# li-kunyi/dns-slam

Hardware: AMD Instinct MI355X
Metric: ray-samples/s (higher is better)
Workload: dtype f32 (MLP products as 3 x f16 split-operand MFMA / 6 x bf16 for weight gradients, f32 accumulate: error <= fp32 fma chain)

## Files before the change

dns_slam_amd/_lib.py:

```python
from __future__ import annotations

import ctypes as C
import os

_HERE = os.path.dirname(os.path.abspath(__file__))
LIB_PATH = os.environ.get("DNS_HIP_LIB") or os.path.join(_HERE, "libdns_hip.so")
DNS_MAX_LEVELS = 32
ABI_VERSION = 13


class DnsGridMeta(C.Structure):
    _fields_ = [
        ("n_levels", C.c_uint32), ("n_features", C.c_uint32), ("log2_hashmap_size", C.c_uint32),
        ("base_resolution", C.c_uint32), ("total_rows", C.c_uint32), ("per_level_scale", C.c_float),
        ("scale", C.c_float * DNS_MAX_LEVELS), ("resolution", C.c_uint32 * DNS_MAX_LEVELS),
        ("size", C.c_uint32 * DNS_MAX_LEVELS), ("offset", C.c_uint32 * DNS_MAX_LEVELS),
        ("hashed", C.c_uint32 * DNS_MAX_LEVELS),
    ]


class DnsSplitRows(C.Structure):
    _fields_ = [("rows", C.c_void_p), ("exps", C.c_void_p), ("ld", C.c_uint32), ("lo_off", C.c_uint32)]


class DnsAdamTensor(C.Structure):
    _fields_ = [("p", C.c_void_p), ("g", C.c_void_p), ("m", C.c_void_p), ("v", C.c_void_p), ("n", C.c_uint64),
                ("lr", C.c_float)]


_P = C.c_void_p
_U = C.c_uint32
_I = C.c_int


class DnsTrackFused(C.Structure):
    _fields_ = [("color", _P), ("depth", _P), ("label", _P),
                ("H", C.c_int32), ("W", C.c_int32), ("H0", C.c_int32), ("H1", C.c_int32), ("W0", C.c_int32), ("W1", C.c_int32),
                ("cam", _P), ("bound", _P),
                ("pix", _P), ("t_uniform", _P), ("t_surf", _P), ("t_zero", _P), ("dmax", _P), ("iter", _P), ("n_iters", _U),
                ("n_uniform", _U), ("n_surface", _U), ("n_rays", _U),
                ("quat", _P), ("trans", _P),
                ("table", _P), ("meta", C.POINTER(DnsGridMeta)), ("n_bins", _U),
                ("w_coarse", _P), ("w_color", _P), ("w_logit", _P),
                ("n_neurons", _U), ("n_hidden_layers", _U), ("hidden", _U), ("n_feat", _U), ("n_class", _U),
                ("code", _P), ("code_dim", _U),
                ("lambda_p", C.c_float), ("lambda_d", C.c_float), ("lambda_l", C.c_float),
                ("ws", _P), ("adam_m", _P), ("adam_v", _P), ("adam_state", _P),
                ("lr_quat", C.c_float), ("lr_trans", C.c_float), ("beta1", C.c_float), ("beta2", C.c_float), ("eps", C.c_float),
                ("best_loss", _P), ("best_cam", _P), ("out", _P), ("g_quat", _P), ("g_trans", _P)]

SIGNATURES = {
    "dns_abi_version": (C.c_int, []),
    "dns_last_error": (C.c_char_p, []),
    "dns_init": (C.c_int, []),
    "dns_kernel_timing": (C.c_int, [C.c_int]),
    "dns_kernel_timing_count": (C.c_int, []),
    "dns_kernel_timing_get": (C.c_int, [C.c_int, C.c_char_p, C.c_int, C.POINTER(C.c_float)]),
    "dns_grid_meta_init": (C.c_int, [C.POINTER(DnsGridMeta), _U, _U, _U, _U, C.c_double]),
    "dns_raygen_sample": (C.c_int, [_P, _P, _P, _P, _P, _P, _P, _P, _I, _I, _I, _I, _I, _I, _I, _I, _P, _P, _P, _I, _I, _I,
                                    _P, _I, _P, _P, _P, _P, _P, _P, _P, _P, _P]),
    "dns_rays_from_pixels": (C.c_int, [_P, _P, _I, _P, _P, _P, _I, _I, _I, _I, _I, _I, _I, _P, _P, _P, _P, _P]),
    "dns_sample_along_rays": (C.c_int, [_P, _P, _I, _P, _P, _P, _I, _I, _P, _P, _P]),
    "dns_raygen_bwd": (C.c_int, [_P, _P, _P, _I, _I, _I, _I, _I, _I, _I, _P, _P, _P, _P, _P, _P, _P, _P]),
    "dns_raygen_bwd_ws_floats": (C.c_uint64, [_I, _I]),
    "dns_encode_fwd": (C.c_int, [_P, _P, _U, _U, _P, C.POINTER(DnsGridMeta), _P, _P, _U, _P, _U, _P, _P]),
    "dns_encode_bwd": (C.c_int, [_P, _P, _U, _U, _P, C.POINTER(DnsGridMeta), _P, _U, _P, _U, _P, _P, _P, _P, _U, _U, _P]),
    "dns_encode_bwd_ws_floats": (C.c_uint64, [_U, C.POINTER(DnsGridMeta), _U, _U]),
    "dns_hashgrid_indices": (C.c_int, [_P, _U, C.POINTER(DnsGridMeta), _P, _P]),
    "dns_mlp_fwd": (C.c_int, [_P, _U, _P, _U, _U, _P, _U, _U, _U, _U, _P, _U, _U, _P, _P, _U, _P, _U, _P]),
    "dns_mlp_bwd": (C.c_int, [_P, _U, _P, _U, _U, _P, _U, _P, _U, _U, _U, _U, _P, _U, _P, _U, _P, _P, _U, _P, _P, _U, _P, _I, _P]),
    "dns_mlp_bwd_ws_floats": (C.c_uint64, [_U, _U, _U]),
    "dns_mlp_dwin": (C.c_int, [_P, _U, _P, _U, _U, _U, _U, _U, _P, _P, _U, _P, _P, _U, _U, _P]),
    "dns_mlp_prepared_floats": (C.c_uint64, [_U, _U, _U, _U]),
    "dns_mlp_prepare": (C.c_int, [_P, _U, _U, _U, _U, _U, _U, _P, _U, _P]),
    "dns_encode_fwd_split": (C.c_int, [_P, _P, _U, _U, _P, C.POINTER(DnsGridMeta), _P, _P, _U, _P, _U, _P, _U, _P, _P]),
    "dns_mlp_fwd_split": (C.c_int, [C.POINTER(DnsSplitRows), C.POINTER(DnsSplitRows), _U, _P, _U, _U, _U, _U, _P, _U, _U, _P, _P, _U,
                                    _U, _P]),
    "dns_mlp_bwd_split": (C.c_int, [C.POINTER(DnsSplitRows), C.POINTER(DnsSplitRows), _U, _P, _U, _P, _U, _U, _U, _U, _P, _U, _P, _U,
                                    _P, _P, _U, _P, _P, _U, _I, _P]),
    "dns_mlp_fwd_half": (C.c_int, [_P, _U, _P, _U, _U, _P, _U, _U, _U, _U, _P, _U, _U, _P, _P, _U, _U, _P]),
    "dns_mlp_bwd_half": (C.c_int, [_P, _U, _P, _U, _U, _P, _U, _P, _U, _U, _U, _U, _P, _U, _P, _U, _P, _U, _P, _P, _U, _I, C.c_float, _P]),
    "dns_feature_block_split": (C.c_int, [_P, _U, _U, _P, _U, _U, _U, _P, _P, _U, _U, _P, _U, _P, _U, _P, _U, _P, _P]),
    "dns_loss_sums": (C.c_int, [_P, _U, _U, _U, _U, _I, _P, _P, _P, _P, _P, _P, _P, _P, _P, _P, _P, _P, _P]),
    "dns_loss_rays": (C.c_int, [_P, _U, _U, _U, _U, _I] + [_P] * 19),
    "dns_loss_finalize_bwd": (C.c_int, [_P, _U, _U, _U, _U, _I] + [_P] * 16),
    "dns_loss_finalize": (C.c_int, [_P, _U, _U, _U, _U, _I, _P, _P, _P]),
    "dns_loss_bwd": (C.c_int, [_P, _U, _U, _U, _U, _I, _P, _P, _P, _P, _P, _P, _P, _P, _P, _P, _P, _P, _P, _P, _P, _P, _P,
                                _P, _P, _U, _P]),
    "dns_loss_bwd_points": (C.c_int, [_P, _U, _U, _U, _U, _P, _P, _P, _P, _P, _P, _P, _P, _P, _U, _P, _U, _P]),
    "dns_composite_fwd_ex": (C.c_int, [_P, _P, _P, _U, _U, _U, _P, _P, _P, _P, _P, _U, _P]),
    "dns_composite_bwd_ex": (C.c_int, [_P, _P, _P, _U, _U, _U, _P, _P, _P, _P, _P, _P, _P, _U, _P]),
    "dns_class_slots": (C.c_int, [_P, _U, _U, _I, _P, _U, _P, _P]),
    "dns_feature_block": (C.c_int, [_P, _U, _U, _P, _U, _P, _P, _U, _U, _P, _U, _P, _P]),
    "dns_rgb_sigmoid": (C.c_int, [_P, _U, _P]),
    "dns_raw_bwd": (C.c_int, [_P, _P, _U, _P, _P, _U, _I, _P]),
    "dns_lattice_points": (C.c_int, [_P, _P, _U, _P, _U, _P, _P]),
    "dns_draw_finish": (C.c_int, [_P, _P, _P, _P, _P, _P, _P, _P, _U, _U, _U, _U, _P, _P, _P, _P]),
    "dns_track_mask": (C.c_int, [_P, _P, _U, C.c_float, _P, _P]),
    "dns_keep_best": (C.c_int, [_P, _P, _P, _P, _P, _P]),
    "dns_force_half": (C.c_int, [_P, _U, _U, _P]),
    "dns_track_fused_ws_floats": (C.c_uint64, [C.POINTER(DnsTrackFused)]),
    "dns_track_fused_begin": (C.c_int, [_P, _U, _U, _P, _I, _I, _I, _I, _P, _U, _P, _P]),
    "dns_track_fused_iter": (C.c_int, [C.POINTER(DnsTrackFused), _P]),
    "dns_feature_gather": (C.c_int, [_P, _P, _P, _P, _U, _U, _U, _I, _I, _I, _I, _P, _P, _P]),
    "dns_feature_gather_frames": (C.c_int, [_P, _P, _P, _P, _P, _U, _U, _U, _U, _I, _I, _I, _I, _P, _U, _P, _P]),
    "dns_refer_poses": (C.c_int, [_P, _P, _P, _P, _U, _P, _P, _P]),
    "dns_merge_dy": (C.c_int, [_P, _U, _U, _U, _U, _P, _P, _U, _U, _P, _P]),
    "dns_add_ref_sum": (C.c_int, [_P, _U, _U, _U, _P, _P]),
    "dns_tv_fwd": (C.c_int, [_P, _U, _U, _U, _I, _U, _P, _P]),
    "dns_tv_bwd": (C.c_int, [_P, _U, _U, _U, _I, _U, _P, _P, _P]),
    "dns_group_slots": (C.c_int, [_P, _U, _U, _U, _U, _P, _P, _P, _P]),
    "dns_group_scatter": (C.c_int, [_P, _U, _U, _P, _U, _P, _P]),
    "dns_device_error": (C.c_int, [C.c_int]),
    "dns_adam_step": (C.c_int, [C.POINTER(DnsAdamTensor), _U, C.c_float, C.c_float, C.c_float, _P, _P]),
    "dns_composite_fwd": (C.c_int, [_P, _P, _P, _U, _U, _U, _P, _P, _P, _P, _P, _P]),
    "dns_composite_bwd": (C.c_int, [_P, _P, _P, _U, _U, _U, _P, _P, _P, _P, _P, _P, _P, _P]),
    "dns_mc_ws_bytes": (C.c_uint64, [_U, _U, _U]),
    "dns_mc_count": (C.c_int, [_P, _U, _U, _U, C.c_float, _P, _P, _P]),
    "dns_mc_emit": (C.c_int, [_P, _U, _U, _U, C.c_float, C.POINTER(C.c_double), C.POINTER(C.c_double), _P, _P, C.c_uint64, _P,
                              C.c_uint64, _P]),
    "dns_keyframe_project": (C.c_int, [_P, _U, _P, _U, _P, _P, _I, _I, C.POINTER(C.c_float), _P, _P, _P]),
}


def _load():
    if not os.path.exists(LIB_PATH):
        raise ImportError(
            f"{LIB_PATH} is missing: the HIP hot-path library has not been built. Run "
            "`python -c 'import __graft_entry__ as g; g.build()'` (or `make -C dns_slam_amd/csrc`). "
            "dns_slam_amd has no CPU fallback.")
    import torch
    lib = C.CDLL(LIB_PATH)
    for name, (res, args) in SIGNATURES.items():
        fn = getattr(lib, name)
        fn.restype = res
        fn.argtypes = args
    v = lib.dns_abi_version()
    if v != ABI_VERSION:
        raise ImportError(f"libdns_hip.so ABI version {v} != expected {ABI_VERSION}; rebuild it")
    return lib


lib = _load()


_ready_devices = set()


def ensure_init() -> None:
    import torch
    d = torch.cuda.current_device()
    if d not in _ready_devices:
        if torch.cuda.is_current_stream_capturing():
            raise RuntimeError("dns_slam_amd: first use on this device inside a hipGraph capture; run one op (or "
                               "dns_slam_amd._lib.ensure_init()) before capturing")
        check(lib.dns_init(), "dns_init")
        _ready_devices.add(d)


def check(rc: int, what: str = "") -> None:
    if rc == 0:
        return
    msg = lib.dns_last_error().decode("utf-8", "replace")
    if rc == -1:
        raise ValueError(f"{what}: {msg}")
    if rc == -2:
        word = lib.dns_device_error(1)
        if word:
            raise RuntimeError(f"{what}: {msg} (code {rc}; device error word {word:#x} was set by an EARLIER kernel -- bit 0: "
                               f"dns_group_slots / dns_group_scatter cursor past n_slots -- and has been cleared)")
    raise RuntimeError(f"{what}: {msg} (code {rc})")


def ptr(t):
    return None if t is None else C.c_void_p(t.data_ptr())


def stream_ptr():
    import torch
    ensure_init()
    return C.c_void_p(torch.cuda.current_stream().cuda_stream)


def require_cuda(*tensors):
    import torch
    for t in tensors:
        if t is None:
            continue
        if not isinstance(t, torch.Tensor) or not t.is_cuda:
            raise ValueError("dns_slam_amd ops run on the GPU only (got a non-CUDA tensor); there is no CPU fallback")
        if not t.is_contiguous():
            raise ValueError("dns_slam_amd ops need contiguous tensors")
```

dns_slam_amd/csrc/composite.hip:

```cpp
#include "common.hpp"
#include "dev_composite.hpp"

namespace dns {

template <int E>
__global__ __launch_bounds__(256) void composite_fwd_kernel(const float* __restrict__ raw, const float* __restrict__ zv,
                                                            const float* __restrict__ logits, uint32_t N, uint32_t S,
                                                            uint32_t C, float* __restrict__ depth, float* __restrict__ var,
                                                            float* __restrict__ rgb, float* __restrict__ weights,
                                                            float* __restrict__ sem, uint32_t rgbl) {
  extern __shared__ float lds[];
  const uint32_t lane = threadIdx.x & 63u, wave = threadIdx.x >> 6;
  const uint32_t n = blockIdx.x * 4 + wave;
  if (n >= N) return;
  float* wl = lds + wave * (64 * E);
  RayState<E> st;
  ray_forward<E>(raw, zv, n, S, lane, st);
  float sv = 0.f, sc[3] = {0.f, 0.f, 0.f};
#pragma unroll
  for (int e = 0; e < E; ++e) {
    const uint32_t s = lane * E + e;
    const float t = st.z[e] - st.depth;
    sv += st.w[e] * t * t;
    if (s < S) {
      const float* r = raw + ((size_t)n * S + s) * 4;
      const float c0 = rgbl ? sigmoid1c(r[0]) : r[0], c1 = rgbl ? sigmoid1c(r[1]) : r[1], c2 = rgbl ? sigmoid1c(r[2]) : r[2];
      sc[0] += st.w[e] * c0;
      sc[1] += st.w[e] * c1;
      sc[2] += st.w[e] * c2;
      if (weights) weights[(size_t)n * S + s] = st.w[e];
    }
    wl[s] = st.w[e];
  }
  sv = wave_sum(sv);
  sc[0] = wave_sum(sc[0]);
  sc[1] = wave_sum(sc[1]);
  sc[2] = wave_sum(sc[2]);
  if (lane == 0) {
    depth[n] = st.depth;
    var[n] = sv;
    rgb[(size_t)n * 3 + 0] = sc[0];
    rgb[(size_t)n * 3 + 1] = sc[1];
    rgb[(size_t)n * 3 + 2] = sc[2];
  }
  if (C) {
    for (uint32_t c = lane; c < C; c += 64) {
      float acc = 0.f;
      const float* lp = logits + (size_t)n * S * C + c;
      for (uint32_t s = 0; s < S; ++s) acc += wl[s] * lp[(size_t)s * C];
      sem[(size_t)n * C + c] = acc;
    }
  }
}

template <int E>
__global__ __launch_bounds__(256) void composite_bwd_kernel(const float* __restrict__ raw, const float* __restrict__ zv,
                                                            const float* __restrict__ logits, uint32_t N, uint32_t S,
                                                            uint32_t C, const float* __restrict__ d_depth,
                                                            const float* __restrict__ d_var, const float* __restrict__ d_rgb,
                                                            const float* __restrict__ d_weights,
                                                            const float* __restrict__ d_sem, float* __restrict__ d_raw,
                                                            float* __restrict__ d_logits, uint32_t rgbl) {
  extern __shared__ float lds[];
  const uint32_t lane = threadIdx.x & 63u, wave = threadIdx.x >> 6;
  const uint32_t n = blockIdx.x * 4 + wave;
  if (n >= N) return;
  float* wl = lds + wave * (64 * E);
  RayState<E> st;
  ray_forward<E>(raw, zv, n, S, lane, st);
  const float gD = d_depth ? d_depth[n] : 0.f;
  const float gV = d_var ? d_var[n] : 0.f;
  float gc[3] = {0.f, 0.f, 0.f};
  if (d_rgb) {
    gc[0] = d_rgb[(size_t)n * 3];
    gc[1] = d_rgb[(size_t)n * 3 + 1];
    gc[2] = d_rgb[(size_t)n * 3 + 2];
  }
  float g[E];
  float col[E][3];
  float gbar = 0.f;
#pragma unroll
  for (int e = 0; e < E; ++e) {
    const uint32_t s = lane * E + e;
    g[e] = 0.f;
    col[e][0] = col[e][1] = col[e][2] = 0.f;
    if (s < S) {
      const float* r = raw + ((size_t)n * S + s) * 4;
      const float t = st.z[e] - st.depth;
      col[e][0] = rgbl ? sigmoid1c(r[0]) : r[0];
      col[e][1] = rgbl ? sigmoid1c(r[1]) : r[1];
      col[e][2] = rgbl ? sigmoid1c(r[2]) : r[2];
      float v = gc[0] * col[e][0] + gc[1] * col[e][1] + gc[2] * col[e][2] + gD * st.z[e] + gV * t * t;
      if (d_weights) v += d_weights[(size_t)n * S + s];
      if (C && d_sem) {
        const float* lp = logits + ((size_t)n * S + s) * C;
        const float* gs = d_sem + (size_t)n * C;
        float dot = 0.f;
        for (uint32_t c = 0; c < C; ++c) dot += gs[c] * lp[c];
        v += dot;
      }
      g[e] = v;
    }
    gbar += st.w[e] * g[e];
    wl[s] = st.w[e];
  }
  gbar = wave_sum(gbar);
  float du[E], lsum = 0.f;
#pragma unroll
  for (int e = 0; e < E; ++e) {
    du[e] = (g[e] - gbar) / st.sumu;
    lsum += du[e] * st.u[e];
  }
  const float after = wave_suffix_excl_sum(lsum, lane);
  float tail = after;
#pragma unroll
  for (int e = E - 1; e >= 0; --e) {
    const uint32_t s = lane * E + e;
    const float dalpha = du[e] * st.T[e] - tail / st.om[e];
    tail += du[e] * st.u[e];
    if (s < S) {
      float* o = d_raw + ((size_t)n * S + s) * 4;
      float o0 = st.w[e] * gc[0], o1 = st.w[e] * gc[1], o2 = st.w[e] * gc[2];
      if (rgbl) {
        o0 = o0 * (1.f - col[e][0]) * col[e][0];
        o1 = o1 * (1.f - col[e][1]) * col[e][1];
        o2 = o2 * (1.f - col[e][2]) * col[e][2];
      }
      o[0] = o0;
      o[1] = o1;
      o[2] = o2;
      o[3] = 10.0f * st.alpha[e] * (1.0f - st.alpha[e]) * dalpha;
    }
  }
  if (C && d_logits) {
    for (uint32_t c = lane; c < C; c += 64) {
      const float gs = d_sem ? d_sem[(size_t)n * C + c] : 0.f;
      float* lp = d_logits + (size_t)n * S * C + c;
      for (uint32_t s = 0; s < S; ++s) lp[(size_t)s * C] = wl[s] * gs;
    }
  }
}

}

using namespace dns;

static int composite_fwd_impl(const char* who, const float* raw, const float* z, const float* logits, uint32_t N, uint32_t S,
                              uint32_t C, float* depth, float* var, float* rgb, float* weights, float* sem, uint32_t rgbl,
                              void* stream) {
  if (N == 0) return DNS_OK;
  DNS_REQUIRE(raw && z && depth && var && rgb, "%s: NULL argument", who);
  DNS_REQUIRE(S >= 1 && S <= 256, "%s: S=%u out of range [1,256]", who, S);
  DNS_REQUIRE(C == 0 || (logits && sem), "%s: C>0 needs logits and sem", who);
  const uint32_t blocks = (N + 3) / 4;
  hipStream_t st = (hipStream_t)stream;
  const uint32_t E = S <= 64 ? 1 : (S <= 128 ? 2 : 4);
  const size_t ldsb = 4 * 64 * E * sizeof(float);
  if (E == 1) DNS_LAUNCH(composite_fwd_kernel<1>, dim3(blocks), dim3(256), ldsb, st, raw, z, logits, N, S, C, depth, var, rgb, weights, sem, rgbl);
  else if (E == 2) DNS_LAUNCH(composite_fwd_kernel<2>, dim3(blocks), dim3(256), ldsb, st, raw, z, logits, N, S, C, depth, var, rgb, weights, sem, rgbl);
  else DNS_LAUNCH(composite_fwd_kernel<4>, dim3(blocks), dim3(256), ldsb, st, raw, z, logits, N, S, C, depth, var, rgb, weights, sem, rgbl);
  return check_launch(who);
}

static int composite_bwd_impl(const char* who, const float* raw, const float* z, const float* logits, uint32_t N, uint32_t S,
                              uint32_t C, const float* d_depth, const float* d_var, const float* d_rgb, const float* d_weights,
                              const float* d_sem, float* d_raw, float* d_logits, uint32_t rgbl, void* stream) {
  if (N == 0) return DNS_OK;
  DNS_REQUIRE(raw && z && d_raw, "%s: NULL argument", who);
  DNS_REQUIRE(S >= 1 && S <= 256, "%s: S=%u out of range [1,256]", who, S);
  DNS_REQUIRE(C == 0 || logits, "%s: C>0 needs logits", who);
  const uint32_t blocks = (N + 3) / 4;
  hipStream_t st = (hipStream_t)stream;
  const uint32_t E = S <= 64 ? 1 : (S <= 128 ? 2 : 4);
  const size_t ldsb = 4 * 64 * E * sizeof(float);
  if (E == 1) DNS_LAUNCH(composite_bwd_kernel<1>, dim3(blocks), dim3(256), ldsb, st, raw, z, logits, N, S, C, d_depth, d_var, d_rgb, d_weights, d_sem, d_raw, d_logits, rgbl);
  else if (E == 2) DNS_LAUNCH(composite_bwd_kernel<2>, dim3(blocks), dim3(256), ldsb, st, raw, z, logits, N, S, C, d_depth, d_var, d_rgb, d_weights, d_sem, d_raw, d_logits, rgbl);
  else DNS_LAUNCH(composite_bwd_kernel<4>, dim3(blocks), dim3(256), ldsb, st, raw, z, logits, N, S, C, d_depth, d_var, d_rgb, d_weights, d_sem, d_raw, d_logits, rgbl);
  return check_launch(who);
}

extern "C" int dns_composite_fwd(const float* raw, const float* z, const float* logits, uint32_t N, uint32_t S,
                                 uint32_t C, float* depth, float* var, float* rgb, float* weights, float* sem,
                                 void* stream) {
  return composite_fwd_impl("dns_composite_fwd", raw, z, logits, N, S, C, depth, var, rgb, weights, sem, 0u, stream);
}

extern "C" int dns_composite_bwd(const float* raw, const float* z, const float* logits, uint32_t N, uint32_t S,
                                 uint32_t C, const float* d_depth, const float* d_var, const float* d_rgb,
                                 const float* d_weights, const float* d_sem, float* d_raw, float* d_logits,
                                 void* stream) {
  return composite_bwd_impl("dns_composite_bwd", raw, z, logits, N, S, C, d_depth, d_var, d_rgb, d_weights, d_sem, d_raw, d_logits, 0u,
                            stream);
}

extern "C" int dns_composite_fwd_ex(const float* raw, const float* z, const float* logits, uint32_t N, uint32_t S, uint32_t C,
                                    float* depth, float* var, float* rgb, float* weights, float* sem, uint32_t flags, void* stream) {
  DNS_REQUIRE((flags & ~DNS_COMPOSITE_RGB_LOGITS) == 0, "dns_composite_fwd_ex: unknown flags 0x%x", flags);
  return composite_fwd_impl("dns_composite_fwd_ex", raw, z, logits, N, S, C, depth, var, rgb, weights, sem, flags & DNS_COMPOSITE_RGB_LOGITS,
                            stream);
}

extern "C" int dns_composite_bwd_ex(const float* raw, const float* z, const float* logits, uint32_t N, uint32_t S, uint32_t C,
                                    const float* d_depth, const float* d_var, const float* d_rgb, const float* d_weights,
                                    const float* d_sem, float* d_raw, float* d_logits, uint32_t flags, void* stream) {
  DNS_REQUIRE((flags & ~DNS_COMPOSITE_RGB_LOGITS) == 0, "dns_composite_bwd_ex: unknown flags 0x%x", flags);
  return composite_bwd_impl("dns_composite_bwd_ex", raw, z, logits, N, S, C, d_depth, d_var, d_rgb, d_weights, d_sem, d_raw, d_logits,
                            flags & DNS_COMPOSITE_RGB_LOGITS, stream);
}
```

dns_slam_amd/csrc/dev_composite.hpp:

```cpp
#pragma once
#include "common.hpp"

namespace dns {

__device__ __forceinline__ float wave_sum(float v) {
#pragma unroll
  for (int o = 32; o >= 1; o >>= 1) v += __shfl_xor(v, o);
  return v;
}

__device__ __forceinline__ float wave_excl_prod(float v, uint32_t lane) {
  float inc = v;
#pragma unroll
  for (int o = 1; o < 64; o <<= 1) {
    const float t = __shfl_up(inc, o);
    if (lane >= (uint32_t)o) inc *= t;
  }
  const float ex = __shfl_up(inc, 1);
  return lane == 0 ? 1.0f : ex;
}

__device__ __forceinline__ float wave_suffix_excl_sum(float v, uint32_t lane) {
  float inc = v;
#pragma unroll
  for (int o = 1; o < 64; o <<= 1) {
    const float t = __shfl_down(inc, o);
    if (lane + o < 64u) inc += t;
  }
  const float ex = __shfl_down(inc, 1);
  return lane == 63 ? 0.0f : ex;
}

__device__ __forceinline__ float sigmoid10(float occ) { return 1.0f / (1.0f + expf(-10.0f * occ)); }
__device__ __forceinline__ float sigmoid1c(float x) { return 1.0f / (1.0f + expf(-x)); }

template <int E>
struct RayState {
  float alpha[E], om[E], T[E], u[E], w[E], z[E];
  float sumu, depth;
};

template <int E>
__device__ __forceinline__ void ray_forward(const float* __restrict__ raw, const float* __restrict__ zv, uint32_t n,
                                            uint32_t S, uint32_t lane, RayState<E>& st) {
  float lp = 1.0f;
#pragma unroll
  for (int e = 0; e < E; ++e) {
    const uint32_t s = lane * E + e;
    const bool ok = s < S;
    const float occ = ok ? raw[((size_t)n * S + s) * 4 + 3] : 0.f;
    st.z[e] = ok ? zv[(size_t)n * S + s] : 0.f;
    st.alpha[e] = ok ? sigmoid10(occ) : 0.f;
    st.om[e] = ok ? (1.0f - st.alpha[e]) + 1e-10f : 1.0f;
    st.T[e] = lp;
    lp *= st.om[e];
  }
  const float pre = wave_excl_prod(lp, lane);
  float su = 0.f;
#pragma unroll
  for (int e = 0; e < E; ++e) {
    st.T[e] *= pre;
    st.u[e] = st.alpha[e] * st.T[e];
    su += st.u[e];
  }
  st.sumu = wave_sum(su);
  float sd = 0.f;
#pragma unroll
  for (int e = 0; e < E; ++e) {
    st.w[e] = st.u[e] / st.sumu;
    sd += st.w[e] * st.z[e];
  }
  st.depth = wave_sum(sd);
}

}
```

dns_slam_amd/csrc/losses.hip:

```cpp
#include <stdlib.h>
#include "common.hpp"

namespace dns {

enum { S_P = 0, S_D, S_L, S_LT, S_FS, S_OP, S_NV, S_ND, S_NFRONT, S_NOMASK, S_COUNT = 16,
       S_PARTIALS = 32, S_MAX_BLOCKS = 1024 };
constexpr uint32_t LOSS_POINT_BLOCKS = 1024;
enum { O_P = 0, O_D, O_L, O_LT, O_FS, O_OP, O_TOTAL, O_CP = 8, O_CD, O_CL, O_CLT, O_CFS, O_COP };

struct LossCfg {
  float lambda_p, lambda_d, lambda_l, lambda_lt, lambda_fs, lambda_op;
  float truncation, sigma;
  uint32_t N, S, C, L;
  int tracker;
};

__device__ __forceinline__ float block_sum(float v, float* sh) {
#pragma unroll
  for (int o = 32; o >= 1; o >>= 1) v += __shfl_xor(v, o);
  const uint32_t lane = threadIdx.x & 63u, wave = threadIdx.x >> 6;
  __syncthreads();
  if (lane == 0) sh[wave] = v;
  __syncthreads();
  float t = 0.f;
  if (threadIdx.x == 0)
    for (uint32_t w = 0; w < (blockDim.x >> 6); ++w) t += sh[w];
  return t;
}

__device__ __forceinline__ bool ray_valid(const uint8_t* valid, uint32_t n) { return valid ? valid[n] != 0 : true; }

struct RayTerms {
  float sp, sd, sl, nv, nd;
};
__device__ __forceinline__ RayTerms ray_terms(const LossCfg& c, uint32_t n, const float* __restrict__ pred_color,
                                              const float* __restrict__ pred_depth, const float* __restrict__ pred_var,
                                              const float* __restrict__ logits, const float* __restrict__ gt_color,
                                              const float* __restrict__ gt_depth, const int64_t* __restrict__ gt_label,
                                              const uint8_t* __restrict__ valid) {
  RayTerms r = {0.f, 0.f, 0.f, 0.f, 0.f};
  if (n < c.N && ray_valid(valid, n)) {
    r.nv = 1.f;
#pragma unroll
    for (int k = 0; k < 3; ++k) {
      const float e = gt_color[(size_t)n * 3 + k] - pred_color[(size_t)n * 3 + k];
      r.sp += e * e;
    }
    const float gd = gt_depth[n];
    if (c.tracker) {
      r.sd = fabsf(gd - pred_depth[n]) / sqrtf(pred_var[n] + 1e-10f);
      r.nd = 1.f;
    } else if (gd > 0.f) {
      r.sd = fabsf(gd - pred_depth[n]);
      r.nd = 1.f;
    }
    if (c.C) {
      const float* lg = logits + (size_t)n * c.C;
      float mx = -INFINITY;
      for (uint32_t k = 0; k < c.C; ++k) mx = fmaxf(mx, lg[k]);
      float se = 0.f;
      for (uint32_t k = 0; k < c.C; ++k) se += expf(lg[k] - mx);
      const int64_t lab = gt_label[n];
      const float ll = (lab >= 0 && lab < (int64_t)c.C) ? lg[lab] : 0.f;
      r.sl = (mx + logf(se)) - ll;
    }
  }
  return r;
}

__global__ __launch_bounds__(256) void loss_ray_sums_kernel(LossCfg c, const float* __restrict__ pred_color,
                                                            const float* __restrict__ pred_depth,
                                                            const float* __restrict__ pred_var,
                                                            const float* __restrict__ logits,
                                                            const float* __restrict__ gt_color,
                                                            const float* __restrict__ gt_depth,
                                                            const int64_t* __restrict__ gt_label,
                                                            const uint8_t* __restrict__ valid, float* __restrict__ sums,
                                                            uint32_t n_partials) {
  __shared__ float sh[16];
  const uint32_t n = blockIdx.x * blockDim.x + threadIdx.x;
  const RayTerms rt = ray_terms(c, n, pred_color, pred_depth, pred_var, logits, gt_color, gt_depth, gt_label, valid);
  const float sp = rt.sp, sd = rt.sd, sl = rt.sl, nv = rt.nv, nd = rt.nd;
  float t;
  t = block_sum(sp, sh); if (threadIdx.x == 0 && t != 0.f) atomicAdd(sums + S_P, t);
  t = block_sum(sd, sh); if (threadIdx.x == 0 && t != 0.f) atomicAdd(sums + S_D, t);
  t = block_sum(sl, sh); if (threadIdx.x == 0 && t != 0.f) atomicAdd(sums + S_L, t);
  t = block_sum(nv, sh); if (threadIdx.x == 0 && t != 0.f) atomicAdd(sums + S_NV, t);
  t = block_sum(nd, sh); if (threadIdx.x == 0 && t != 0.f) atomicAdd(sums + S_ND, t);
  if (blockIdx.x == 0 && n_partials) {
    const float* partial = sums + S_PARTIALS;
    const int dst[5] = {S_LT, S_FS, S_OP, S_NFRONT, S_NOMASK};
#pragma unroll
    for (int i = 0; i < 5; ++i) {
      float v = 0.f;
      for (uint32_t b = threadIdx.x; b < n_partials; b += blockDim.x) v += partial[b * 5u + i];
      const float tt = block_sum(v, sh);
      if (threadIdx.x == 0) sums[dst[i]] = tt;
    }
  }
}

__device__ __forceinline__ float sigmoid10f(float x) { return 1.0f / (1.0f + expf(-10.0f * x)); }

struct PointAcc {
  float slt, sfs, sop, nfr, nom;
};

__device__ __forceinline__ void loss_point_elem(const LossCfg& c, float f, float co, uint32_t p, uint32_t k, uint32_t n,
                                                const float* __restrict__ z, const float* __restrict__ gt_depth,
                                                const uint8_t* __restrict__ valid, PointAcc& a) {
  if (!ray_valid(valid, n)) return;
  const float d0 = co - f;
  a.slt += d0 * d0;
  if (k + 1 == c.L) {
    const float d = gt_depth[n], zz = z[p];
    const float occ = sigmoid10f(f);
    const float front = zz < (d - c.truncation) ? 1.f : 0.f;
    const float back = zz > (d + c.truncation) ? 1.f : 0.f;
    const float dm = d > 0.f ? 1.f : 0.f;
    const float om = (1.f - front) * (1.f - back) * dm;
    const float a1 = occ * front * dm;
    a.sfs += a1 * a1;
    const float r = (zz - d) / c.sigma;
    const float pseudo = 0.5f * expf(-0.5f * r * r);
    const float a2 = occ * om - pseudo * om;
    a.sop += a2 * a2;
    a.nfr += front;
    a.nom += om;
  }
}

__device__ __forceinline__ void loss_point_quad(const LossCfg& c, uint32_t e0, const float4& f4, const float4& c4,
                                                const float* __restrict__ z, const float* __restrict__ gt_depth,
                                                const uint8_t* __restrict__ valid, PointAcc& a) {
  const uint32_t p0 = e0 / c.L, k0 = e0 - p0 * c.L;
  const uint32_t n0 = p0 / c.S;
  const uint32_t p1 = p0 + (k0 + 3u >= c.L ? 1u : 0u);
  const uint32_t n1 = (p1 != p0 && p1 - n0 * c.S == c.S) ? n0 + 1u : n0;
  const bool v0 = ray_valid(valid, n0), v1 = ray_valid(valid, n1);
  const uint32_t jl = c.L - 1u - k0;
  const bool has_last = jl < 4u;
  const float zz = z[p0], d = gt_depth[n0];
  const float fv[4] = {f4.x, f4.y, f4.z, f4.w}, cv[4] = {c4.x, c4.y, c4.z, c4.w};
#pragma unroll
  for (int j = 0; j < 4; ++j) {
    const bool second = k0 + (uint32_t)j >= c.L;
    const bool ok = second ? v1 : v0;
    const float d0 = cv[j] - fv[j];
    a.slt += ok ? d0 * d0 : 0.f;
  }
  if (has_last && v0) {
    const float f = jl == 0 ? fv[0] : jl == 1 ? fv[1] : jl == 2 ? fv[2] : fv[3];
    const float occ = sigmoid10f(f);
    const float front = zz < (d - c.truncation) ? 1.f : 0.f;
    const float back = zz > (d + c.truncation) ? 1.f : 0.f;
    const float dm = d > 0.f ? 1.f : 0.f;
    const float om = (1.f - front) * (1.f - back) * dm;
    const float a1 = occ * front * dm;
    a.sfs += a1 * a1;
    const float r = (zz - d) / c.sigma;
    const float pseudo = 0.5f * expf(-0.5f * r * r);
    const float a2 = occ * om - pseudo * om;
    a.sop += a2 * a2;
    a.nfr += front;
    a.nom += om;
  }
}

__global__ __launch_bounds__(256) void loss_point_sums_kernel(LossCfg c, const float* __restrict__ fine,
                                                              const float* __restrict__ coarse,
                                                              const float* __restrict__ z,
                                                              const float* __restrict__ gt_depth,
                                                              const uint8_t* __restrict__ valid,
                                                              float* __restrict__ sums) {
  __shared__ float sh[4];
  if (blockIdx.x == 0 && threadIdx.x < S_COUNT) sums[threadIdx.x] = 0.f;
  const uint32_t E = c.N * c.S * c.L;
  PointAcc a = {0.f, 0.f, 0.f, 0.f, 0.f};
  const uint32_t gtid = blockIdx.x * blockDim.x + threadIdx.x, gstride = gridDim.x * blockDim.x;
  const bool vec = ((((uintptr_t)fine) | ((uintptr_t)coarse)) & 15u) == 0;
  const uint32_t Q = vec ? E / 4u : 0u;
  const float4* __restrict__ f4p = reinterpret_cast<const float4*>(fine);
  const float4* __restrict__ c4p = reinterpret_cast<const float4*>(coarse);
  for (uint32_t q = gtid; q < Q; q += 4u * gstride) {
    uint32_t qq[4];
    float4 fv[4], cv[4];
#pragma unroll
    for (int u = 0; u < 4; ++u) {
      qq[u] = q + (uint32_t)u * gstride;
      const uint32_t qc = qq[u] < Q ? qq[u] : q;
      fv[u] = f4p[qc];
      cv[u] = c4p[qc];
    }
#pragma unroll
    for (int u = 0; u < 4; ++u)
      if (qq[u] < Q) loss_point_quad(c, 4u * qq[u], fv[u], cv[u], z, gt_depth, valid, a);
  }
  for (uint32_t e = 4u * Q + gtid; e < E; e += gstride) {
    const uint32_t p = e / c.L, k = e - p * c.L;
    loss_point_elem(c, fine[e], coarse[e], p, k, p / c.S, z, gt_depth, valid, a);
  }
  float* partial = sums + S_PARTIALS;
  const float vals[5] = {a.slt, a.sfs, a.sop, a.nfr, a.nom};
#pragma unroll
  for (int i = 0; i < 5; ++i) {
    const float t = block_sum(vals[i], sh);
    if (threadIdx.x == 0) partial[blockIdx.x * 5u + i] = t;
  }
}

__device__ __forceinline__ void finalize_terms(const LossCfg& c, const float* sums, float* out) {
  const float nv = sums[S_NV], nd = sums[S_ND];
  const float np = nv * (float)c.S;
  const float p = sums[S_P] / (3.f * nv);
  const float d = sums[S_D] / nd;
  const float l = c.C ? sums[S_L] / nv : 0.f;
  float lt = 0.f, fs = 0.f, op = 0.f, flag = 0.f;
  if (!c.tracker) {
    lt = sums[S_LT] / (np * (float)c.L);
    flag = (sums[S_NFRONT] > 0.f && sums[S_NOMASK] > 0.f) ? 1.f : 0.f;
    fs = flag * sums[S_FS] / np;
    op = flag * sums[S_OP] / np;
  }
  out[O_P] = p; out[O_D] = d; out[O_L] = l; out[O_LT] = lt; out[O_FS] = fs; out[O_OP] = op;
  out[O_TOTAL] = c.lambda_p * p + c.lambda_d * d + c.lambda_l * l + c.lambda_lt * lt + c.lambda_fs * fs + c.lambda_op * op;
  out[O_CP] = c.lambda_p * 2.f / (3.f * nv);
  out[O_CD] = c.lambda_d / nd;
  out[O_CL] = c.lambda_l / nv;
  out[O_CLT] = c.tracker ? 0.f : c.lambda_lt * 2.f / (np * (float)c.L);
  out[O_CFS] = c.tracker ? 0.f : flag * c.lambda_fs * 2.f / np;
  out[O_COP] = c.tracker ? 0.f : flag * c.lambda_op * 2.f / np;
}

__global__ void loss_finalize_kernel(LossCfg c, const float* __restrict__ sums, float* __restrict__ out) {
  if (threadIdx.x != 0 || blockIdx.x != 0) return;
  finalize_terms(c, sums, out);
}

__device__ __forceinline__ void ray_bwd_one(const LossCfg& c, const float* out, float g, uint32_t n,
                                            const float* __restrict__ pred_color, const float* __restrict__ pred_depth,
                                            const float* __restrict__ pred_var, const float* __restrict__ logits,
                                            const float* __restrict__ gt_color, const float* __restrict__ gt_depth,
                                            const int64_t* __restrict__ gt_label, const uint8_t* __restrict__ valid,
                                            float* __restrict__ d_color, float* __restrict__ d_depth, float* __restrict__ d_var,
                                            float* __restrict__ d_logits) {
  const bool ok = ray_valid(valid, n);
#pragma unroll
  for (int k = 0; k < 3; ++k)
    d_color[(size_t)n * 3 + k] = ok ? -g * out[O_CP] * (gt_color[(size_t)n * 3 + k] - pred_color[(size_t)n * 3 + k]) : 0.f;
  const float gd = gt_depth[n];
  float dd = 0.f, dv = 0.f;
  if (ok) {
    const float e = gd - pred_depth[n];
    const float sg = e > 0.f ? -1.f : (e < 0.f ? 1.f : 0.f);
    if (c.tracker) {
      const float sv = sqrtf(pred_var[n] + 1e-10f);
      dd = g * out[O_CD] * sg / sv;
      dv = g * out[O_CD] * fabsf(e) * (-0.5f) / (sv * sv * sv);
    } else if (gd > 0.f) {
      dd = g * out[O_CD] * sg;
    }
  }
  d_depth[n] = dd;
  if (d_var) d_var[n] = dv;
  if (c.C) {
    const float* lg = logits + (size_t)n * c.C;
    float* dl = d_logits + (size_t)n * c.C;
    if (!ok) {
      for (uint32_t k = 0; k < c.C; ++k) dl[k] = 0.f;
    } else {
      float mx = -INFINITY;
      for (uint32_t k = 0; k < c.C; ++k) mx = fmaxf(mx, lg[k]);
      float se = 0.f;
      for (uint32_t k = 0; k < c.C; ++k) se += expf(lg[k] - mx);
      const int64_t lab = gt_label[n];
      const float cl = g * out[O_CL];
      for (uint32_t k = 0; k < c.C; ++k) dl[k] = cl * (expf(lg[k] - mx) / se - ((int64_t)k == lab ? 1.f : 0.f));
    }
  }
}

__global__ __launch_bounds__(256) void loss_ray_bwd_kernel(LossCfg c, const float* __restrict__ out,
                                                           const float* __restrict__ g_total,
                                                           const float* __restrict__ pred_color,
                                                           const float* __restrict__ pred_depth,
                                                           const float* __restrict__ pred_var,
                                                           const float* __restrict__ logits,
                                                           const float* __restrict__ gt_color,
                                                           const float* __restrict__ gt_depth,
                                                           const int64_t* __restrict__ gt_label,
                                                           const uint8_t* __restrict__ valid, float* __restrict__ d_color,
                                                           float* __restrict__ d_depth, float* __restrict__ d_var,
                                                           float* __restrict__ d_logits, const float* __restrict__ sums,
                                                           float* __restrict__ out_w) {
  __shared__ float s_out[16];
  if (sums) {
    if (threadIdx.x == 0) {
      finalize_terms(c, sums, s_out);
      s_out[7] = 0.f; s_out[14] = 0.f; s_out[15] = 0.f;
    }
    __syncthreads();
    if (blockIdx.x == 0 && threadIdx.x < 16) out_w[threadIdx.x] = s_out[threadIdx.x];
    out = s_out;
  }
  const uint32_t n = blockIdx.x * blockDim.x + threadIdx.x;
  if (n >= c.N) return;
  ray_bwd_one(c, out, g_total[0], n, pred_color, pred_depth, pred_var, logits, gt_color, gt_depth, gt_label, valid, d_color, d_depth,
              d_var, d_logits);
}

__global__ __launch_bounds__(1024) void loss_rays_fused_kernel(LossCfg c, const float* __restrict__ pred_color,
                                                               const float* __restrict__ pred_depth,
                                                               const float* __restrict__ pred_var,
                                                               const float* __restrict__ logits,
                                                               const float* __restrict__ gt_color,
                                                               const float* __restrict__ gt_depth,
                                                               const int64_t* __restrict__ gt_label,
                                                               const uint8_t* __restrict__ valid, float* __restrict__ sums,
                                                               uint32_t n_partials, float* __restrict__ out,
                                                               const float* __restrict__ g_total, float* __restrict__ d_color,
                                                               float* __restrict__ d_depth, float* __restrict__ d_var,
                                                               float* __restrict__ d_logits) {
  __shared__ float sh[16];
  __shared__ float s_sums[S_COUNT], s_out[16];
  RayTerms a = {0.f, 0.f, 0.f, 0.f, 0.f};
  for (uint32_t n = threadIdx.x; n < c.N; n += blockDim.x) {
    const RayTerms r = ray_terms(c, n, pred_color, pred_depth, pred_var, logits, gt_color, gt_depth, gt_label, valid);
    a.sp += r.sp; a.sd += r.sd; a.sl += r.sl; a.nv += r.nv; a.nd += r.nd;
  }
  if (threadIdx.x < S_COUNT) s_sums[threadIdx.x] = 0.f;
  const float rv[5] = {a.sp, a.sd, a.sl, a.nv, a.nd};
  const int rd[5] = {S_P, S_D, S_L, S_NV, S_ND};
#pragma unroll
  for (int i = 0; i < 5; ++i) {
    const float t = block_sum(rv[i], sh);
    if (threadIdx.x == 0) s_sums[rd[i]] = t;
  }
  if (n_partials) {
    const float* partial = sums + S_PARTIALS;
    const int dst[5] = {S_LT, S_FS, S_OP, S_NFRONT, S_NOMASK};
#pragma unroll
    for (int i = 0; i < 5; ++i) {
      float v = 0.f;
      for (uint32_t b = threadIdx.x; b < n_partials; b += blockDim.x) v += partial[b * 5u + i];
      const float t = block_sum(v, sh);
      if (threadIdx.x == 0) s_sums[dst[i]] = t;
    }
  }
  if (threadIdx.x == 0) {
    finalize_terms(c, s_sums, s_out);
    s_out[7] = 0.f; s_out[14] = 0.f; s_out[15] = 0.f;
  }
  __syncthreads();
  if (threadIdx.x < S_COUNT) {
    sums[threadIdx.x] = s_sums[threadIdx.x];
    out[threadIdx.x] = s_out[threadIdx.x];
  }
  const float g = g_total[0];
  for (uint32_t n = threadIdx.x; n < c.N; n += blockDim.x)
    ray_bwd_one(c, s_out, g, n, pred_color, pred_depth, pred_var, logits, gt_color, gt_depth, gt_label, valid, d_color, d_depth, d_var,
                d_logits);
}

__global__ __launch_bounds__(256) void loss_point_bwd_kernel(LossCfg c, const float* __restrict__ out,
                                                             const float* __restrict__ g_total,
                                                             const float* __restrict__ fine,
                                                             const float* __restrict__ coarse,
                                                             const float* __restrict__ z,
                                                             const float* __restrict__ gt_depth,
                                                             const uint8_t* __restrict__ valid, float* __restrict__ d_fine,
                                                             float* __restrict__ d_coarse, uint32_t ldd_fine,
                                                             const float* __restrict__ d_occ, uint32_t ld_occ) {
  const uint32_t E = c.N * c.S * c.L;
  const float g = g_total[0];
  const float clt = g * out[O_CLT], cfs = g * out[O_CFS], cop = g * out[O_COP];
  auto elem = [&](uint32_t p, uint32_t k, uint32_t n, bool ok, float f, float co, float& df, float& dc) {
    df = (k == 0 && d_occ) ? d_occ[(size_t)p * ld_occ] : 0.f;
    dc = 0.f;
    if (!ok) return;
    const float d0 = co - f;
    dc = clt * d0;
    df -= clt * d0;
    if (k + 1 == c.L) {
      const float d = gt_depth[n], zz = z[p];
      const float occ = sigmoid10f(f);
      const float front = zz < (d - c.truncation) ? 1.f : 0.f;
      const float back = zz > (d + c.truncation) ? 1.f : 0.f;
      const float dm = d > 0.f ? 1.f : 0.f;
      const float om = (1.f - front) * (1.f - back) * dm;
      const float r = (zz - d) / c.sigma;
      const float pseudo = 0.5f * expf(-0.5f * r * r);
      const float docc = cfs * (occ * front * dm) * (front * dm) + cop * (occ * om - pseudo * om) * om;
      df += docc * 10.f * occ * (1.f - occ);
    }
  };
  const uint32_t gtid = blockIdx.x * blockDim.x + threadIdx.x, stride = gridDim.x * blockDim.x;
  const bool vec = ((((uintptr_t)fine) | ((uintptr_t)coarse) | ((uintptr_t)d_coarse)) & 15u) == 0;
  const uint32_t Q = vec ? E / 4u : 0u;
  const float4* __restrict__ f4p = reinterpret_cast<const float4*>(fine);
  const float4* __restrict__ c4p = reinterpret_cast<const float4*>(coarse);
  for (uint32_t q0 = gtid; q0 < Q; q0 += 2u * stride) {
    const uint32_t q1 = q0 + stride;
    const bool two = q1 < Q;
    const uint32_t qq[2] = {q0, two ? q1 : q0};
    const float4 fa[2] = {f4p[qq[0]], f4p[qq[1]]}, ca[2] = {c4p[qq[0]], c4p[qq[1]]};
#pragma unroll
    for (int u = 0; u < 2; ++u) {
      if (u == 1 && !two) break;
      const uint32_t e0 = 4u * qq[u];
      uint32_t p = e0 / c.L, k = e0 - p * c.L;
      uint32_t n = p / c.S, sidx = p - n * c.S;
      bool ok = ray_valid(valid, n);
      const float fv[4] = {fa[u].x, fa[u].y, fa[u].z, fa[u].w}, cv[4] = {ca[u].x, ca[u].y, ca[u].z, ca[u].w};
      float dcv[4];
#pragma unroll
      for (int j = 0; j < 4; ++j) {
        float df;
        elem(p, k, n, ok, fv[j], cv[j], df, dcv[j]);
        d_fine[(size_t)p * ldd_fine + k] = df;
        if (++k == c.L) {
          k = 0;
          ++p;
          if (++sidx == c.S) {
            sidx = 0;
            ++n;
            ok = n < c.N ? ray_valid(valid, n) : false;
          }
        }
      }
      *reinterpret_cast<float4*>(d_coarse + e0) = make_float4(dcv[0], dcv[1], dcv[2], dcv[3]);
    }
  }
  for (uint32_t e = 4u * Q + gtid; e < E; e += stride) {
    const uint32_t p = e / c.L, k = e - p * c.L;
    const uint32_t n = p / c.S;
    float df, dc;
    elem(p, k, n, ray_valid(valid, n), fine[e], coarse[e], df, dc);
    d_fine[(size_t)p * ldd_fine + k] = df;
    d_coarse[e] = dc;
  }
}

}

using namespace dns;

static LossCfg make_cfg(const float* lambdas, uint32_t N, uint32_t S, uint32_t C, uint32_t L, int tracker) {
  LossCfg c;
  c.lambda_p = lambdas[0]; c.lambda_d = lambdas[1]; c.lambda_l = lambdas[2];
  c.lambda_lt = lambdas[3]; c.lambda_fs = lambdas[4]; c.lambda_op = lambdas[5];
  c.truncation = lambdas[6]; c.sigma = lambdas[7];
  c.N = N; c.S = S; c.C = C; c.L = L; c.tracker = tracker;
  return c;
}

extern "C" int dns_loss_sums(const float* lambdas, uint32_t N, uint32_t S, uint32_t C, uint32_t L, int tracker,
                             const float* pred_color, const float* pred_depth, const float* pred_var,
                             const float* pred_logits, const float* gt_color, const float* gt_depth,
                             const int64_t* gt_label, const uint8_t* valid, const float* fine, const float* coarse,
                             const float* z, float* sums, void* stream) {
  DNS_REQUIRE(lambdas && sums, "dns_loss_sums: NULL argument");
  hipStream_t st = (hipStream_t)stream;
  if (tracker || N == 0) {
    const int rc = fill_words(sums, 0u, S_COUNT, st, "dns_loss_sums");
    if (rc != DNS_OK) return rc;
  }
  if (N == 0) return DNS_OK;
  DNS_REQUIRE(pred_color && pred_depth && gt_color && gt_depth, "dns_loss_sums: NULL ray tensor");
  DNS_REQUIRE(C == 0 || (pred_logits && gt_label), "dns_loss_sums: C > 0 needs logits and labels");
  DNS_REQUIRE(!tracker || pred_var, "dns_loss_sums: tracker mode needs pred_var");
  DNS_REQUIRE(tracker || (fine && coarse && z && L >= 1 && S >= 1), "dns_loss_sums: mapper mode needs fine, coarse, z");
  DNS_REQUIRE(tracker || (uint64_t)N * S * L < (1ull << 32) - (1ull << 22), "dns_loss_sums: N*S*L must stay below 2^32");
  const LossCfg c = make_cfg(lambdas, N, S, C, L, tracker);
  uint32_t blocks = 0;
  if (!tracker) {
    const uint64_t E = (uint64_t)N * S * L;
    static const uint32_t cap_env = [] { const char* e = getenv("DNS_LOSS_BLOCKS"); const long n = e ? atol(e) : 0; return (uint32_t)(n >= 1 && n <= (long)S_MAX_BLOCKS ? n : 0); }();
    const uint32_t cap = cap_env ? cap_env : LOSS_POINT_BLOCKS;
    blocks = (uint32_t)((E + 255) / 256 < cap ? (E + 255) / 256 : cap);
    DNS_LAUNCH(loss_point_sums_kernel, dim3(blocks), dim3(256), 0, st, c, fine, coarse, z, gt_depth, valid, sums);
  }
  DNS_LAUNCH(loss_ray_sums_kernel, dim3((N + 255) / 256), dim3(256), 0, st, c, pred_color, pred_depth, pred_var,
                     pred_logits, gt_color, gt_depth, gt_label, valid, sums, blocks);
  return check_launch("dns_loss_sums");
}

extern "C" int dns_loss_rays(const float* lambdas, uint32_t N, uint32_t S, uint32_t C, uint32_t L, int tracker,
                             const float* pred_color, const float* pred_depth, const float* pred_var, const float* pred_logits,
                             const float* gt_color, const float* gt_depth, const int64_t* gt_label, const uint8_t* valid,
                             const float* fine, const float* coarse, const float* z, float* sums, float* out, const float* g_total,
                             float* d_color, float* d_depth, float* d_var, float* d_logits, void* stream) {
  DNS_REQUIRE(lambdas && sums && out && g_total, "dns_loss_rays: NULL argument");
  DNS_REQUIRE(N >= 1 && N <= (1u << 20), "dns_loss_rays: N %u outside [1, 2^20] (use dns_loss_sums / _finalize / _bwd)", N);
  DNS_REQUIRE(pred_color && pred_depth && gt_color && gt_depth && d_color && d_depth, "dns_loss_rays: NULL ray tensor");
  DNS_REQUIRE(C == 0 || (pred_logits && gt_label && d_logits), "dns_loss_rays: C > 0 needs logits, labels and d_logits");
  DNS_REQUIRE(!tracker || pred_var, "dns_loss_rays: tracker mode needs pred_var");
  DNS_REQUIRE(tracker || (fine && coarse && z && L >= 1 && S >= 1), "dns_loss_rays: mapper mode needs fine, coarse, z");
  DNS_REQUIRE(tracker || (uint64_t)N * S * L < (1ull << 32) - (1ull << 22), "dns_loss_rays: N*S*L must stay below 2^32");
  const LossCfg c = make_cfg(lambdas, N, S, C, L, tracker);
  hipStream_t st = (hipStream_t)stream;
  uint32_t blocks = 0;
  if (!tracker) {
    const uint64_t E = (uint64_t)N * S * L;
    const uint32_t cap = LOSS_POINT_BLOCKS;
    blocks = (uint32_t)((E + 255) / 256 < cap ? (E + 255) / 256 : cap);
    DNS_LAUNCH(loss_point_sums_kernel, dim3(blocks), dim3(256), 0, st, c, fine, coarse, z, gt_depth, valid, sums);
  }
  DNS_LAUNCH(loss_rays_fused_kernel, dim3(1), dim3(1024), 0, st, c, pred_color, pred_depth, pred_var, pred_logits, gt_color, gt_depth,
             gt_label, valid, sums, blocks, out, g_total, d_color, d_depth, d_var, d_logits);
  return check_launch("dns_loss_rays");
}

extern "C" int dns_loss_finalize(const float* lambdas, uint32_t N, uint32_t S, uint32_t C, uint32_t L, int tracker,
                                 const float* sums, float* out, void* stream) {
  DNS_REQUIRE(lambdas && sums && out, "dns_loss_finalize: NULL argument");
  const LossCfg c = make_cfg(lambdas, N, S, C, L, tracker);
  DNS_LAUNCH(loss_finalize_kernel, dim3(1), dim3(64), 0, (hipStream_t)stream, c, sums, out);
  return check_launch("dns_loss_finalize");
}

extern "C" int dns_loss_bwd(const float* lambdas, uint32_t N, uint32_t S, uint32_t C, uint32_t L, int tracker,
                            const float* out, const float* g_total, const float* pred_color, const float* pred_depth,
                            const float* pred_var, const float* pred_logits, const float* gt_color,
                            const float* gt_depth, const int64_t* gt_label, const uint8_t* valid, const float* fine,
                            const float* coarse, const float* z, float* d_color, float* d_depth, float* d_var,
                            float* d_logits, float* d_fine, float* d_coarse, uint32_t ldd_fine, void* stream) {
  if (N == 0) return DNS_OK;
  DNS_REQUIRE(ldd_fine == 0 || ldd_fine >= L, "dns_loss_bwd: ldd_fine %u < L %u", ldd_fine, L);
  DNS_REQUIRE(lambdas && out && g_total && d_color && d_depth, "dns_loss_bwd: NULL argument");
  DNS_REQUIRE(C == 0 || d_logits, "dns_loss_bwd: C > 0 needs d_logits");
  DNS_REQUIRE(tracker || (d_fine != nullptr) == (d_coarse != nullptr), "dns_loss_bwd: d_fine and d_coarse come together (both NULL: "
              "the ray part only, the point part follows with dns_loss_bwd_points)");
  const LossCfg c = make_cfg(lambdas, N, S, C, L, tracker);
  hipStream_t st = (hipStream_t)stream;
  DNS_LAUNCH(loss_ray_bwd_kernel, dim3((N + 255) / 256), dim3(256), 0, st, c, out, g_total, pred_color, pred_depth,
                     pred_var, pred_logits, gt_color, gt_depth, gt_label, valid, d_color, d_depth, d_var, d_logits, (const float*)nullptr,
                     (float*)nullptr);
  if (!tracker && d_fine) {
    const uint64_t E = (uint64_t)N * S * L;
    const uint32_t blocks = (uint32_t)((E + 255) / 256 < 4096 ? (E + 255) / 256 : 4096);
    DNS_LAUNCH(loss_point_bwd_kernel, dim3(blocks), dim3(256), 0, st, c, out, g_total, fine, coarse, z, gt_depth,
                       valid, d_fine, d_coarse, ldd_fine ? ldd_fine : L, nullptr, 0u);
  }
  return check_launch("dns_loss_bwd");
}

extern "C" int dns_loss_finalize_bwd(const float* lambdas, uint32_t N, uint32_t S, uint32_t C, uint32_t L, int tracker,
                                     const float* sums, float* out, const float* g_total, const float* pred_color,
                                     const float* pred_depth, const float* pred_var, const float* pred_logits, const float* gt_color,
                                     const float* gt_depth, const int64_t* gt_label, const uint8_t* valid, float* d_color,
                                     float* d_depth, float* d_var, float* d_logits, void* stream) {
  DNS_REQUIRE(N >= 1, "dns_loss_finalize_bwd: N must be >= 1 (dns_loss_finalize handles the empty batch)");
  DNS_REQUIRE(lambdas && sums && out && g_total && d_color && d_depth, "dns_loss_finalize_bwd: NULL argument");
  DNS_REQUIRE(C == 0 || d_logits, "dns_loss_finalize_bwd: C > 0 needs d_logits");
  const LossCfg c = make_cfg(lambdas, N, S, C, L, tracker);
  DNS_LAUNCH(loss_ray_bwd_kernel, dim3((N + 255) / 256), dim3(256), 0, (hipStream_t)stream, c, (const float*)nullptr, g_total,
             pred_color, pred_depth, pred_var, pred_logits, gt_color, gt_depth, gt_label, valid, d_color, d_depth, d_var, d_logits, sums,
             out);
  return check_launch("dns_loss_finalize_bwd");
}

extern "C" int dns_loss_bwd_points(const float* lambdas, uint32_t N, uint32_t S, uint32_t C, uint32_t L, const float* out,
                                   const float* g_total, const float* gt_depth, const uint8_t* valid, const float* fine,
                                   const float* coarse, const float* z, float* d_fine, float* d_coarse, uint32_t ldd_fine,
                                   const float* d_occ, uint32_t ld_occ, void* stream) {
  if (N == 0) return DNS_OK;
  DNS_REQUIRE(lambdas && out && g_total && gt_depth && fine && coarse && z && d_fine && d_coarse, "dns_loss_bwd_points: NULL argument");
  DNS_REQUIRE(ldd_fine == 0 || ldd_fine >= L, "dns_loss_bwd_points: ldd_fine %u < L %u", ldd_fine, L);
  DNS_REQUIRE(!d_occ || ld_occ >= 1, "dns_loss_bwd_points: ld_occ");
  DNS_REQUIRE((uint64_t)N * S * L < (1ull << 32) - (1ull << 22), "dns_loss_bwd_points: N*S*L must stay below 2^32");
  const LossCfg c = make_cfg(lambdas, N, S, C, L, 0);
  const uint64_t E = (uint64_t)N * S * L;
  const uint32_t blocks = (uint32_t)((E + 255) / 256 < 4096 ? (E + 255) / 256 : 4096);
  DNS_LAUNCH(loss_point_bwd_kernel, dim3(blocks), dim3(256), 0, (hipStream_t)stream, c, out, g_total, fine, coarse, z, gt_depth, valid,
             d_fine, d_coarse, ldd_fine ? ldd_fine : L, d_occ, ld_occ);
  return check_launch("dns_loss_bwd_points");
}
```

dns_slam_amd/fused_step.py:

```python
from __future__ import annotations

import ctypes as C
import os

import torch

from . import ops
from ._lib import DnsAdamTensor, DnsSplitRows, DnsTrackFused, check, ptr
from .common import get_quad_from_c2w, get_rotation_from_quad

_V = C.c_void_p


def _morton2(row, col):
    def spread(v):
        v = v & 0xffff
        v = (v | (v << 8)) & 0x00ff00ff
        v = (v | (v << 4)) & 0x0f0f0f0f
        v = (v | (v << 2)) & 0x33333333
        return (v | (v << 1)) & 0x55555555
    return spread(col) | (spread(row) << 1)


class _Set:
    pass


class MapStep:
    def __init__(self, mapper, target_frames, quad_list=None, T_list=None, prep=None, features=None, lambda_lt=10.0,
                 smooth=True, betas=(0.9, 0.999), eps=1e-8, keep_hidden=False, split_rows=None, refer_frames=None):
        m = self.m = mapper
        dev = self.dev = torch.device(m.device)
        if dev.type != "cuda":
            raise ValueError("dns_slam_amd ops run on the GPU only; there is no CPU fallback")
        if not (m.static_shapes and m.fused_losses):
            raise ValueError("MapStep needs mapper.static_shapes and mapper.fused_losses (the sync-free iteration)")
        self.stem = features is not None and features.dim() == 5
        if features is not None and features.dim() not in (3, 5):
            raise ValueError("MapStep: features is the per-sample code [N, S, C] or the stem feature maps [K, R, C, h, w]")
        if self.stem and refer_frames is None:
            raise ValueError("MapStep: stem feature maps need refer_frames (kf_idx, est_c2w)")
        self.dist_on = m.dist is not None and m.dist.enabled
        self.world = m.dist.world_size if self.dist_on else 1
        self.union = self.dist_on and m.dist.union
        self.frames = target_frames
        self.prep = prep if prep is not None else m.prepare_frames(target_frames)
        self.npf_g = self.prep["n1"] + self.prep["n2"]
        self.ray_a, self.ray_b = m.dist.shard(self.npf_g) if self.union else (0, self.npf_g)
        self.features = None if (features is None or self.stem) else features.to(dev).float().contiguous()
        if self.features is not None and self.union:
            K_ = m.n_target_frame
            fs = self.features
            self.features = fs.reshape(K_, self.npf_g, *fs.shape[1:])[:, self.ray_a:self.ray_b].reshape(-1, *fs.shape[1:]).contiguous()
        self.lambda_lt, self.smooth = float(lambda_lt), bool(smooth)
        self.morton = (bool(getattr(m, "morton_draws", os.environ.get("DNS_MORTON_DRAWS", "0") == "1")) and m.label_layout == "per_ray")
        self.betas, self.eps = betas, eps
        K = self.K = m.n_target_frame
        dec, pool = m.decoder, m.fine_decoders
        self.pe_dim, self.grid_dim, self.hid = m.pe_dim, m.grid_dim, m.hidden_dim
        nets = (dec.coarse_fn.decoder, dec.out_fn.color_decoder, dec.out_fn.logit_decoder)
        if any(getattr(n, "fp16", False) != getattr(nets[0], "fp16", False) for n in nets):
            raise ValueError("MapStep: the networks must share one operand precision")
        self.fp16 = ops.MLP_FP16_FLAG if getattr(nets[0], "fp16", False) else 0
        shp = lambda n: (n.n_input_dims, n.n_output_dims, n.n_neurons, n.n_hidden_layers)
        self.shp_c, self.shp_col, self.shp_log = (shp(n) for n in nets)
        self.shp_f = (self.pe_dim + self.grid_dim, self.hid + 1, pool.nn_, pool.nl)
        code_dim = self.hid if self.stem else (0 if features is None else self.features.shape[-1])
        n_feat_full = self.shp_col[0] - self.pe_dim
        self.n_feat = self.hid + code_dim
        if not (self.pe_dim % 4 == 0 and self.pe_dim <= 64 and n_feat_full <= 64 and self.n_feat % 4 == 0
                and (self.n_feat == n_feat_full or code_dim == 0) and self.shp_log[0] == self.shp_col[0]):
            raise ValueError("MapStep: network shapes outside the two-segment input form (ops.render_nets has the same limits)")
        self.live = ops.MLP_LIVE_IN(self.pe_dim + self.n_feat) if self.n_feat < n_feat_full else 0
        if self.live and keep_hidden:
            self.n_feat, self.live = n_feat_full, 0
        self.n_class = self.shp_log[1]

        if quad_list is None:
            quad_list = [get_quad_from_c2w(target_frames["est_c2w"][k]).to(dev) for k in range(K)]
            T_list = [target_frames["est_c2w"][k][:3, 3].detach().clone().to(dev) for k in range(K)]
        self.quad_list, self.T_list = quad_list, T_list
        self.Q = torch.stack([q.detach().float() for q in quad_list]).contiguous()
        self.T = torch.stack([t.detach().float() for t in T_list]).contiguous()
        self.is_BA = bool(m.is_BA)
        self.pose_row0 = 0 if K == 1 else 1

        self.p_table = dec.pe_fn.grid_fn.params
        self.meta = dec.pe_fn.grid_fn.meta
        self.n_bins = dec.pe_fn.pe_fn.n_bins
        self.p_coarse, self.p_color, self.p_logit = (n.params for n in nets)
        self.p_pool = pool.pool
        names = ["color", "logit", "pool"] + (["merge"] if self.stem else []) + ["table", "coarse", "quat", "trans"]
        if self.stem:
            mg = dec.merge.decoder
            self.shp_m = shp(mg)
            self.p_merge = mg.params
        byname = {"color": self.p_color, "logit": self.p_logit, "pool": self.p_pool, "table": self.p_table, "coarse": self.p_coarse,
                  "quat": self.Q, "trans": self.T}
        if self.stem:
            byname["merge"] = self.p_merge
        plist = [byname[n] for n in names]
        for p in plist:
            if not (p.is_cuda and p.is_contiguous() and p.dtype == torch.float32):
                raise ValueError("MapStep: parameters must be contiguous fp32 CUDA tensors")
        sizes = [(p.numel() + 3) // 4 * 4 for p in plist]
        offs = [sum(sizes[:i]) for i in range(len(sizes))]
        off_of = dict(zip(names, offs))
        n_G = sum(sizes)
        self.M, self.V = torch.zeros(n_G, device=dev), torch.zeros(n_G, device=dev)
        self.adam_state = torch.zeros(3, device=dev)
        lr_pose = float(m.BA_cam_lr) * float(self.is_BA)
        items = [(byname[n], off_of[n], byname[n].numel(), float(m.lr)) for n in names if n not in ("quat", "trans")]
        if self.is_BA:
            a4, a3 = 4 * self.pose_row0, 3 * self.pose_row0
            items.append((self.Q.view(-1)[a4:], off_of["quat"] + a4, self.Q.numel() - a4, lr_pose))
            items.append((self.T.view(-1)[a3:], off_of["trans"] + a3, self.T.numel() - a3, lr_pose))
        items = [it for it in items if it[2] > 0]
        self.n_adam = len(items)

        def adam_items(G):
            arr = (DnsAdamTensor * len(items))()
            for k, (p, o, n, lr) in enumerate(items):
                it = arr[k]
                it.p, it.g = p.data_ptr(), G.data_ptr() + 4 * o
                it.m, it.v = self.M.data_ptr() + 4 * o, self.V.data_ptr() + 4 * o
                it.n, it.lr = n, lr
            return arr

        npf = self.npf = self.ray_b - self.ray_a
        nu = 0 if m.t_uniform is None else m.t_uniform.numel()
        ns = m.n_surface_ray
        N, S = K * npf, nu + ns
        P = N * S
        self.N, self.S, self.P, self.nu, self.ns = N, S, P, nu, ns
        f = lambda *s: torch.empty(*s, device=dev, dtype=torch.float32)
        self.rays_o, self.rays_d, self.gt_color, self.gt_depth = f(N, 3), f(N, 3), f(N, 3), f(N)
        self.gt_label = torch.empty(N, device=dev, dtype=torch.int64)
        self.inside = torch.empty(N, device=dev, dtype=torch.uint8)
        self.z, self.pts = f(N, S), f(N, S, 3)
        ld = self.ld = self.pe_dim + self.grid_dim
        self.x3, self.buf = f(P, 3), f(P, ld)
        self.dydx = f(self.meta.n_levels * 3 * P * 2) if self.is_BA else None
        if split_rows is None:
            split_rows = os.environ.get("DNS_SPLIT_ROWS", "0") == "1"
        self.sr = bool(split_rows) and ld % 16 == 0 and self.pe_dim % 16 == 0 and self.n_feat % 16 == 0 and not keep_hidden
        if self.sr and self.live:
            self.n_feat, self.live = self.shp_col[0] - self.pe_dim, 0
        self.half = (bool(self.fp16) and bool(getattr(m, "half_rows", os.environ.get("DNS_HALF_ROWS", "1") != "0")) and not self.stem
                     and not keep_hidden and not self.sr and ld % 16 == 0 and self.pe_dim % 8 == 0 and self.n_feat % 8 == 0
                     and (self.pe_dim + self.n_feat) % 16 == 0)
        self.loss_scale = float(getattr(m, "loss_scale", ops.HALF_LOSS_SCALE))
        if self.half:
            self.xh = torch.empty(P, ld, device=dev, dtype=torch.float16)
            self.feath = torch.empty(P, self.n_feat, device=dev, dtype=torch.float16)
        self.use_prep = (bool(getattr(m, "prepared_images", os.environ.get("DNS_PREPARED_IMAGES", "1") != "0")) and not self.sr
                         and not self.half)
        self._blobs, self._prep_jobs = {}, []
        if self.use_prep:
            raw_lib = ops.lib._raw
            G = int(self.p_pool.shape[0]) if self.p_pool.dim() == 2 else 1
            live_n = (self.live >> 16) & 0xff
            jobs = [(self.p_coarse, self.shp_c, self.shp_c[1], 1, 0, 0),
                    (self.p_coarse, self.shp_c, 1, 1, 0, 0),
                    (self.p_pool, self.shp_f, self.shp_f[1], G, int(self.p_pool.shape[-1]), 0),
                    (self.p_color, self.shp_col, self.shp_col[1], 1, 0, self.live),
                    (self.p_logit, self.shp_log, self.shp_log[1], 1, 0, self.live)]
            for prm, shp_, n_out, n_sets, stride, lv in jobs:
                n_in_eff = live_n if lv else shp_[0]
                nfl = int(raw_lib.dns_mlp_prepared_floats(n_in_eff, n_out, shp_[2], shp_[3]))
                blob = torch.empty(nfl * n_sets + 64, device=dev)
                off = (-blob.data_ptr() // 4) % 4
                view = blob[off:off + nfl * n_sets]
                self._blobs[(prm.data_ptr(), n_out)] = view
                self._prep_jobs.append((prm, shp_[0], n_out, shp_[2], shp_[3], n_sets, stride, view, lv, blob))
        self.sr_planes = 1 if self.fp16 else 2
        self.sr_flags = 1 if self.fp16 else 0
        if self.sr:
            np_ = self.sr_planes
            h16 = lambda *s_: torch.empty(*s_, device=dev, dtype=torch.float16)
            i32 = lambda n_: torch.empty(n_, device=dev, dtype=torch.int32)
            self.xs, self.xexp = h16(P, np_ * ld), i32(P)
            self.fxs, self.fexp = h16(P, np_ * self.n_feat), i32(P)
            self.rows_x = DnsSplitRows(self.xs.data_ptr(), self.xexp.data_ptr(), np_ * ld, ld if np_ == 2 else 0)
            self.rows_f = DnsSplitRows(self.fxs.data_ptr(), self.fexp.data_ptr(), np_ * self.n_feat, self.n_feat if np_ == 2 else 0)
        nf = self.hid + 1
        self.coarse = f(P, nf)
        n_groups = self.n_groups = max(len(pool), 1)
        self.n_slots = (P + 127) // 128 * 128 + 128 * n_groups
        self.group_ws = torch.empty(512, device=dev, dtype=torch.int32)
        self.feat = f(P, self.n_feat)
        self.slot = torch.empty(P, device=dev, dtype=torch.int64)
        self.sets = []
        for _ in range(2):
            st_ = _Set()
            o_G = (P * nf + 3) // 4 * 4
            st_.zb = torch.zeros(o_G + n_G, device=dev)
            st_.fine, st_.G = st_.zb[:P * nf].view(P, nf), st_.zb[o_G:]
            for n_ in names:
                setattr(st_, "g_" + n_, st_.G[off_of[n_]:off_of[n_] + byname[n_].numel()])
            st_.G_early, st_.G_late = st_.G[:off_of["table"]], st_.G[off_of["table"]:]
            st_.adam_items = adam_items(st_.G)
            st_.row_index = torch.empty(self.n_slots, device=dev, dtype=torch.int32)
            st_.tile_group = torch.empty(self.n_slots // 128, device=dev, dtype=torch.int32)
            st_.ev, st_.draws, st_.dmax = None, None, None
            self.sets.append(st_)
        self.cur = self.sets[0]
        self.raw, self.logit = f(P, 4), f(P, self.n_class)
        self.depth, self.var, self.rgb, self.weights, self.sem = f(N), f(N), f(N, 3), f(N, S), f(N, self.n_class)
        self.sums_ws, self.out = f(ops.LOSS_SUMS_FLOATS), f(16)
        self.one = torch.ones(1, device=dev)
        self.d_color, self.d_depth, self.d_sem = f(N, 3), f(N), f(N, self.n_class)
        self.d_coarse = f(P, nf)
        self.d_raw, self.d_logit, self.d_col = f(P, 4), f(P, self.n_class), f(P, 4)
        self.d_buf = f(P, ld)
        self.d_featx = torch.zeros(P, 4 + self.n_feat, device=dev)
        self.d_x3 = f(P, 3)
        raw_lib = ops.lib._raw
        if self.stem:
            Kf, R, Cs, fh, fw = features.shape
            if Kf != K:
                raise ValueError("MapStep: stem feature maps must have one set of reference views per target frame")
            self.R, self.Cs, self.fh, self.fw = int(R), int(Cs), int(fh), int(fw)
            self.feat_maps = features.detach().to(dev).float().permute(0, 1, 3, 4, 2).contiguous().reshape(K * R, fh, fw, Cs)
            mrg = dec.merge
            self.n_bins_m = mrg.pe_fn.n_bins
            self.pe_m = 3 * self.n_bins_m
            n_in_m, n_out_m = self.shp_m[0], self.shp_m[1]
            if not (n_in_m == self.pe_m + Cs and n_out_m == self.hid and self.pe_m % 4 == 0):
                raise ValueError("MapStep: Decoder.merge's network does not match the stem features / hidden width")
            self.b6m = ops._bound6(mrg.bound)
            target_idx = list(target_frames["kf_idx"])
            src, fixed = [], []
            for i in range(K):
                ridx = list(refer_frames["kf_idx"][i])
                if len(ridx) != R:
                    raise ValueError("MapStep: refer_frames['kf_idx'] must list n_refer views per target frame")
                for r, rid in enumerate(ridx):
                    k = i if rid == -1 else (target_idx.index(rid) if rid in target_idx else -1)
                    src.append(k)
                    fixed.append(refer_frames["est_c2w"][i][ridx.index(rid)].detach().to(dev).float().reshape(16))
            self.ref_src = torch.tensor(src, dtype=torch.int32, device=dev)
            self.ref_fixed = torch.stack(fixed).contiguous()
            self.w2c, self.origin = f(K * R, 16), f(K * R, 3)
            Mr = self.Mr = R * P
            self.Pf = npf * S
            self.mbuf, self.rel, self.xm = f(Mr, n_in_m), f(Mr, 3), f(Mr, 3)
            self.mlat, self.mdy = f(Mr, n_out_m), f(Mr, n_out_m)
            self.d_mpe, self.d_rel = (f(Mr, self.pe_m), f(Mr, 3)) if self.is_BA else (None, None)
            self.ws_m = f(max(int(raw_lib.dns_mlp_bwd_ws_floats(Mr, self.shp_m[2], self.shp_m[3])), 4))
            self.K9 = (C.c_float * 9)(float(m.fx), 0.0, float(m.cx), 0.0, float(m.fy), float(m.cy), 0.0, 0.0, 1.0)
        self.ray_ws = f(max(int(raw_lib.dns_raygen_bwd_ws_floats(K, npf)), 1))
        mlp_ws = lambda n_slots, s: f(max(int(raw_lib.dns_mlp_bwd_ws_floats(n_slots, s[2], s[3])), 4))
        self.ws_mlp = max((mlp_ws(self.n_slots, s) for s in (self.shp_f, self.shp_c, self.shp_col, self.shp_log)),
                          key=lambda t: t.numel())
        self.ws_mlp4 = [self.ws_mlp] + [torch.empty_like(self.ws_mlp) for _ in range(3)]
        self.keep_h = self.keep_h_lat = bool(keep_hidden)
        hbuf = lambda n_slots, s: f(s[3] * n_slots * s[2]) if self.keep_h else None
        self.h_c, self.h_f, self.h_col, self.h_log = hbuf(P, self.shp_c), hbuf(self.n_slots, self.shp_f), hbuf(P, self.shp_col), hbuf(P, self.shp_log)
        self.scatter_form, self.scatter_cap = ops.SCATTER_FORM
        enc_ws = lambda n: f(max(int(raw_lib.dns_encode_bwd_ws_floats(n, C.byref(self.meta.c), self.scatter_form, self.scatter_cap)), 4))
        self.ws_enc = enc_ws(P)
        tr = m.cfg["training"]
        self.lam = (C.c_float * 8)(m.lambda_p, m.lambda_d, m.lambda_l, self.lambda_lt, m.lambda_fs, m.lambda_opacity,
                                   tr["opacity_sigma"], 0.05)
        self.camv = (C.c_double * 4)(float(m.fx), float(m.fy), float(m.cx), float(m.cy))
        self.b6 = ops._bound6(m.bound)

        if self.smooth:
            sp = self.sp = tr["smooth_pts"]
            m._ensure_lattice(sp, 0.1, 0.05)
            n = self.n_lat = sp - 1
            la, lb = m.dist.shard(n) if self.union else (0, n)
            lhi = min(lb + 1, n)
            self.lat_nx, self.lat_halo = lhi - la, 1 if lhi > lb else 0
            Pl = self.Pl = self.lat_nx * n * n
            self.bufl, self.occ, self.d_occ, self.d_bufl = f(Pl, ld), f(Pl, 1), f(Pl, 1), f(Pl, ld)
            if self.half:
                self.xhl = torch.empty(Pl, ld, device=dev, dtype=torch.float16)
            if self.sr:
                np_ = self.sr_planes
                self.xsl, self.xexpl = torch.empty(Pl, np_ * ld, device=dev, dtype=torch.float16), torch.empty(Pl, device=dev, dtype=torch.int32)
                self.rows_l = DnsSplitRows(self.xsl.data_ptr(), self.xexpl.data_ptr(), np_ * ld, ld if np_ == 2 else 0)
            self.pts_l = f(Pl, 3)
            ar = torch.arange(n, device=dev)
            ii, jj, kk = torch.meshgrid(ar[la:lhi], ar, ar, indexing="ij")
            elem = (ii * (n * n) + jj * n + kk).reshape(-1)

            def spread(v):
                v = v & 0x3ff
                v = (v | (v << 16)) & 0x30000ff
                v = (v | (v << 8)) & 0x300f00f
                v = (v | (v << 4)) & 0x30c30c3
                return (v | (v << 2)) & 0x9249249

            code = spread(ii.reshape(-1)) | (spread(jj.reshape(-1)) << 1) | (spread(kk.reshape(-1)) << 2)
            self.lat_order_l = torch.argsort(code).contiguous()
            self.lat_order = elem[self.lat_order_l].to(torch.int32).contiguous()
            self.lat_slot = torch.empty_like(self.lat_order_l)
            self.lat_slot[self.lat_order_l] = torch.arange(Pl, device=dev)
            self.occ_x, self.d_occ_x = f(Pl, 1), f(Pl, 1)
            _, c_vox, c_off, c_mar = m._lattice_consts
            self.lat_consts = (C.c_double * 9)(*[float(v) for t in (c_vox, c_off, c_mar) for v in t.cpu().tolist()])
            self.tv = f(1)
            self.w_sm = torch.full((1,), m.lambda_sm if self.union else m.lambda_sm / self.world, device=dev)
            self.ws_mlp_l = mlp_ws(Pl, self.shp_c)
            self.h_l = f(self.shp_c[3] * Pl * self.shp_c[2]) if self.keep_h_lat else None
            self.ws_enc_l = enc_ws(Pl)
        if getattr(m, "_side_stream", None) is None:
            m._side_stream = torch.cuda.Stream(device=dev)
        self.side = m._side_stream
        self.steps = 0

    def _prepare_weights(self, st):
        for prm, n_in, n_out, nn, nl, n_sets, stride, view, lv, _ in self._prep_jobs:
            check(ops.lib.dns_mlp_prepare(ptr(prm), n_in, n_out, nn, nl, n_sets, stride, ptr(view), lv, st), "dns_mlp_prepare")

    def _w(self, params, n_out):
        blob = self._blobs.get((params.data_ptr(), n_out)) if self.use_prep else None
        if blob is None:
            return ptr(params), 0
        return ptr(blob), ops.MLP_PREPARED_FLAG

    def _lattice_branch(self, cur, st):
        lib = ops.lib
        Pl, ld, pe = self.Pl, self.ld, self.pe_dim
        pts = self.pts_l
        check(lib.dns_lattice_points(ptr(cur.draws["r6"]), self.lat_consts, self.n_lat, ptr(self.lat_order), Pl, ptr(pts), st),
              "dns_lattice_points")
        meta = C.byref(self.meta.c)
        grid_l = _V(self.bufl.data_ptr() + 4 * pe)
        n_in, _, nn, nl = self.shp_c
        if self.half:
            check(lib.dns_encode_fwd_split(ptr(pts), None, Pl, self.n_bins, ptr(self.p_table), meta, None, None, 0, ptr(self.xhl), ld,
                                           None, ops.SPLIT_PLAIN, None, st), "dns_encode_fwd_split")
            check(lib.dns_mlp_fwd_half(ptr(self.xhl), ld, None, 0, 0, ptr(self.p_coarse), n_in, 1, nn, nl, ptr(self.occ), 1, Pl,
                                       None, None, 0, 0, st), "dns_mlp_fwd_half")
        elif self.sr:
            check(lib.dns_encode_fwd_split(ptr(pts), None, Pl, self.n_bins, ptr(self.p_table), meta, None, ptr(self.bufl), ld,
                                           ptr(self.xsl), self.sr_planes * ld, ptr(self.xexpl), self.sr_flags, None, st), "dns_encode_fwd_split")
            check(lib.dns_mlp_fwd_split(C.byref(self.rows_l), None, 0, ptr(self.p_coarse), n_in, 1, nn, nl, ptr(self.occ), 1, Pl,
                                        None, None, 0, self.fp16, st), "dns_mlp_fwd_split")
        else:
            check(lib.dns_encode_fwd(ptr(pts), None, Pl, self.n_bins, ptr(self.p_table), meta, None, ptr(self.bufl), ld,
                                     grid_l, ld, None, st), "dns_encode_fwd")
            wl, wflag = self._w(self.p_coarse, 1)
            check(lib.dns_mlp_fwd(ptr(self.bufl), ld, None, 0, 0, wl, n_in, 1, nn, nl, ptr(self.occ), 1, Pl,
                                  None, None, 0, ptr(self.h_l), self.fp16 | wflag, st), "dns_mlp_fwd")
        torch.index_select(self.occ, 0, self.lat_slot, out=self.occ_x)
        check(lib.dns_tv_fwd(ptr(self.occ_x), 1, self.lat_nx, self.n_lat, self.lat_halo, self.sp, ptr(self.tv), st), "dns_tv_fwd")
        check(lib.dns_tv_bwd(ptr(self.occ_x), 1, self.lat_nx, self.n_lat, self.lat_halo, self.sp, ptr(self.w_sm), ptr(self.d_occ_x), st),
              "dns_tv_bwd")
        torch.index_select(self.d_occ_x, 0, self.lat_order_l, out=self.d_occ)
        if self.half:
            check(lib.dns_mlp_bwd_half(ptr(self.xhl), ld, None, 0, 0, ptr(self.d_occ), 1, ptr(self.p_coarse), n_in, 1, nn, nl,
                                       ptr(self.d_bufl), ld, None, 0, ptr(cur.g_coarse), Pl, None, None, 0, ops.MLP_DX_FROM(pe),
                                       self.loss_scale, st), "dns_mlp_bwd_half")
        elif self.sr:
            check(lib.dns_mlp_bwd_split(C.byref(self.rows_l), None, 0, ptr(self.d_occ), 1, ptr(self.p_coarse), n_in, 1, nn, nl,
                                        ptr(self.d_bufl), ld, None, 0, ptr(cur.g_coarse), ptr(self.ws_mlp_l), Pl, None, None, 0,
                                        self.fp16, st), "dns_mlp_bwd_split")
            check(lib.dns_mlp_dwin(ptr(self.bufl), ld, None, 0, 0, n_in, nn, nl, ptr(cur.g_coarse), ptr(self.ws_mlp_l), Pl, None, None,
                                   0, self.fp16, st), "dns_mlp_dwin")
        else:
            wl, wflag = self._w(self.p_coarse, 1)
            check(lib.dns_mlp_bwd(ptr(self.bufl), ld, None, 0, 0, ptr(self.d_occ), 1, wl, n_in, 1, nn, nl,
                                  ptr(self.d_bufl), ld, None, 0, ptr(cur.g_coarse), ptr(self.ws_mlp_l), Pl, None, None, 0, ptr(self.h_l),
                                  self.fp16 | wflag | (0 if self.h_l is not None else ops.MLP_DX_FROM(pe)), st), "dns_mlp_bwd")
        d_grid_l = _V(self.d_bufl.data_ptr() + 4 * pe)
        check(lib.dns_encode_bwd(ptr(pts), None, Pl, self.n_bins, ptr(self.p_table), meta, None, ld, d_grid_l, ld,
                                 ptr(cur.g_table), None, None, ptr(self.ws_enc_l), self.scatter_form, self.scatter_cap, st),
              "dns_encode_bwd")

    def _prepare(self, st_, stream, draws):
        m, lib = self.m, ops.lib
        K, npf, N, S, P = self.K, self.npf, self.N, self.S, self.P
        npf_g = self.npf_g
        prep = self.prep
        if draws is None:
            n1, n2 = prep["n1"], prep["n2"]
            i1 = torch.randint(prep["HW"], (K, n1), device=self.dev)
            u = torch.rand(K, n2, device=self.dev, dtype=torch.float64)
            pix = torch.empty(K * npf_g, device=self.dev, dtype=torch.int64)
            labels = torch.empty(K * npf_g, device=self.dev, dtype=torch.int64)
            dmax = torch.empty(K, device=self.dev, dtype=torch.int32)
            check(lib.dns_draw_finish(ptr(i1), ptr(u), ptr(prep["counts_f64"]), ptr(prep["counts_m1"]), ptr(prep["starts_flat"]),
                                      ptr(prep["sorted_flat"]), ptr(prep["depth"]), ptr(prep["label"]), K, n1, n2, prep["HW"],
                                      ptr(pix), ptr(labels), ptr(dmax), stream), "dns_draw_finish")
            if self.morton:
                p2 = pix.view(K, npf_g)
                code = _morton2(torch.div(p2, m.W, rounding_mode="floor"), p2 % m.W)
                order = torch.argsort(code, dim=1)
                pix = torch.gather(p2, 1, order).reshape(-1).contiguous()
                labels = torch.gather(labels.view(K, npf_g), 1, order).reshape(-1).contiguous()
            d = {"pix": pix, "jitter": m.draw_jitter(), "r6": torch.rand(6, device=self.dev) if self.smooth else None}
        else:
            d = dict(draws)
            pix2 = d["pix"].reshape(K, npf_g)
            dmax = torch.gather(prep["depth"].reshape(K, -1), 1, pix2).amax(dim=1).clamp_min(0.0).float().contiguous().view(torch.int32)
            labels = torch.gather(prep["label"].reshape(K, -1), 1, pix2).reshape(-1).long()
        tiled = m.label_layout == "reference_tiled"
        n_lab, s_lab = N, S
        if self.union:
            m._check_same_draws(d["pix"].reshape(K, npf_g))
            a, b = self.ray_a, self.ray_b
            d["pix"] = d["pix"].reshape(K, npf_g)[:, a:b].reshape(-1).contiguous()
            if tiled:
                from .dist import union_point_labels
                labels, n_lab, s_lab, tiled = union_point_labels(labels, K, npf_g, a, b, S).contiguous(), P, 1, False
            else:
                labels = labels.reshape(K, npf_g)[:, a:b].reshape(-1).contiguous()
        st_.draws = d
        if self.dist_on and not self.union:
            fmax = dmax.view(torch.float32)
            m.dist.allreduce_max(fmax)
        st_.dmax = dmax
        lut = m.fine_decoders.lut(0)
        check(lib.dns_class_slots(ptr(labels), n_lab, s_lab, 1 if tiled else 0, ptr(lut), lut.numel(),
                                  ptr(self.slot), stream), "dns_class_slots")
        check(lib.dns_group_slots(ptr(self.slot), P, self.n_groups, 2, self.n_slots, ptr(self.group_ws), ptr(st_.row_index),
                                  ptr(st_.tile_group), stream), "dns_group_slots")
        st_.zb.zero_()

    @torch.no_grad()
    def step(self, draws=None, last=False):
        m, lib = self.m, ops.lib
        if torch.cuda.is_current_stream_capturing():
            self._captured = True
        main = torch.cuda.current_stream()
        st = _V(main.cuda_stream)
        K, npf, N, S, P, ld, pe = self.K, self.npf, self.N, self.S, self.P, self.ld, self.pe_dim
        prefetch = getattr(m, "prefetch_draws", False) and draws is None
        cur = self.sets[self.steps % 2]
        if not prefetch or cur.ev is None:
            self._prepare(cur, st, draws)
        else:
            main.wait_event(cur.ev)
        cur.ev = None
        self.cur = cur
        pix, (t_surf, t_zero) = cur.draws["pix"], cur.draws["jitter"]
        on_side = self.smooth and getattr(m, "overlap_smooth", False)
        if on_side or prefetch:
            self.side.wait_stream(main)
        prep_ev = None
        if self.use_prep:
            if on_side or prefetch:
                with torch.cuda.stream(self.side):
                    self._prepare_weights(_V(self.side.cuda_stream))
                    prep_ev = torch.cuda.Event()
                    prep_ev.record(self.side)
            else:
                self._prepare_weights(st)
        if on_side:
            with torch.cuda.stream(self.side):
                self._lattice_branch(cur, _V(self.side.cuda_stream))
        elif self.smooth:
            self._lattice_branch(cur, st)
        if prefetch and not last:
            nxt = self.sets[(self.steps + 1) % 2]
            with torch.cuda.stream(self.side):
                self._prepare(nxt, _V(self.side.cuda_stream), None)
                nxt.ev = torch.cuda.Event()
                nxt.ev.record(self.side)
            for t in (nxt.draws["pix"], nxt.draws["jitter"][0], nxt.draws["jitter"][1], nxt.dmax):
                t.record_stream(main)

        jstride = self.ns if t_surf.dim() == 2 else 0
        prep = self.prep
        H, W = m.H, m.W
        check(lib.dns_raygen_sample(ptr(pix), ptr(prep["color"]), ptr(prep["depth"]), ptr(prep["label"]), ptr(self.Q),
                                    ptr(self.T), self.camv, self.b6, H, W, 0, H, 0, W, K, npf, ptr(m.t_uniform), ptr(t_surf),
                                    ptr(t_zero), self.nu, self.ns, jstride, ptr(cur.dmax), 1, ptr(self.rays_o), ptr(self.rays_d),
                                    ptr(self.gt_color), ptr(self.gt_depth), ptr(self.gt_label), ptr(self.inside), ptr(self.z),
                                    ptr(self.pts), st), "dns_raygen_sample")
        meta = C.byref(self.meta.c)
        grid = _V(self.buf.data_ptr() + 4 * pe)
        sr = self.sr
        half = self.half
        if half:
            check(lib.dns_encode_fwd_split(ptr(self.pts), self.b6, P, self.n_bins, ptr(self.p_table), meta, ptr(self.x3), None, 0,
                                           ptr(self.xh), ld, None, ops.SPLIT_PLAIN, ptr(self.dydx), st), "dns_encode_fwd_split")
        elif sr:
            check(lib.dns_encode_fwd_split(ptr(self.pts), self.b6, P, self.n_bins, ptr(self.p_table), meta, ptr(self.x3), ptr(self.buf),
                                           ld, ptr(self.xs), self.sr_planes * ld, ptr(self.xexp), self.sr_flags, ptr(self.dydx), st),
                  "dns_encode_fwd_split")
        else:
            check(lib.dns_encode_fwd(ptr(self.pts), self.b6, P, self.n_bins, ptr(self.p_table), meta, ptr(self.x3), ptr(self.buf),
                                     ld, grid, ld, ptr(self.dydx), st), "dns_encode_fwd")
        if self.stem:
            R, Pf = self.R, self.Pf
            n_in_m, n_out_m, nn_m, nl_m = self.shp_m
            check(lib.dns_refer_poses(ptr(self.Q), ptr(self.T), ptr(self.ref_src), ptr(self.ref_fixed), K * R, ptr(self.w2c),
                                      ptr(self.origin), st), "dns_refer_poses")
            check(lib.dns_feature_gather_frames(ptr(self.pts), ptr(self.w2c), ptr(self.origin), self.K9, ptr(self.feat_maps), K, R, Pf,
                                                self.Cs, self.fh, self.fw, H, W, _V(self.mbuf.data_ptr() + 4 * self.pe_m), n_in_m,
                                                ptr(self.rel), st), "dns_feature_gather_frames")
            check(lib.dns_encode_fwd(ptr(self.rel), self.b6m, self.Mr, self.n_bins_m, None, None, ptr(self.xm), ptr(self.mbuf), n_in_m,
                                     None, 0, None, st), "dns_encode_fwd")
            check(lib.dns_mlp_fwd(ptr(self.mbuf), n_in_m, None, 0, 0, ptr(self.p_merge), n_in_m, n_out_m, nn_m, nl_m, ptr(self.mlat),
                                  n_out_m, self.Mr, None, None, 0, None, self.fp16, st), "dns_mlp_fwd")
        fp16 = self.fp16
        rows_x = C.byref(self.rows_x) if sr else None
        rows_f = C.byref(self.rows_f) if sr else None

        def fwd(x2, n_in1, params, shape, y, ri, tg, n_slots, stride, hs):
            n_in, n_out, nn, nl = shape
            if half:
                check(lib.dns_mlp_fwd_half(ptr(self.xh), ld, None if x2 is None else ptr(self.feath), self.n_feat, n_in1, ptr(params),
                                           n_in, n_out, nn, nl, ptr(y), y.stride(0), n_slots, ptr(ri), ptr(tg), stride,
                                           0 if x2 is None else self.live, st), "dns_mlp_fwd_half")
                return
            if sr:
                check(lib.dns_mlp_fwd_split(rows_x, None if x2 is None else rows_f, n_in1, ptr(params), n_in, n_out, nn, nl, ptr(y),
                                            y.stride(0), n_slots, ptr(ri), ptr(tg), stride, fp16, st), "dns_mlp_fwd_split")
                return
            wp, wflag = self._w(params, n_out)
            check(lib.dns_mlp_fwd(ptr(self.buf), ld, ptr(x2), 0 if x2 is None else x2.stride(0), n_in1, wp, n_in, n_out,
                                  nn, nl, ptr(y), y.stride(0), n_slots, ptr(ri), ptr(tg), stride, ptr(hs),
                                  fp16 | wflag | (0 if x2 is None else self.live), st), "dns_mlp_fwd")

        if prep_ev is not None:
            main.wait_event(prep_ev)
        fwd(None, 0, self.p_coarse, self.shp_c, self.coarse, None, None, P, 0, self.h_c)
        fine, row_index, tile_group = cur.fine, cur.row_index, cur.tile_group
        fwd(None, 0, self.p_pool, self.shp_f, fine, row_index, tile_group, self.n_slots, self.p_pool.shape[-1], self.h_f)
        if half:
            check(lib.dns_feature_block_split(ptr(fine), self.hid + 1, self.hid, ptr(self.features), self.n_feat - self.hid, 1, 0,
                                              ptr(self.z), ptr(self.gt_depth), N, S, None, 0, ptr(self.feath), self.n_feat, None,
                                              ops.SPLIT_PLAIN, ptr(self.raw), st), "dns_feature_block_split")
        elif sr or self.stem:
            code, n_ref, Pf_ = (self.mlat, self.R, self.Pf) if self.stem else (self.features, 1, 0)
            check(lib.dns_feature_block_split(ptr(fine), self.hid + 1, self.hid, ptr(code), self.n_feat - self.hid, n_ref, Pf_,
                                              ptr(self.z), ptr(self.gt_depth), N, S, ptr(self.feat), self.n_feat,
                                              ptr(self.fxs) if sr else None, self.sr_planes * self.n_feat,
                                              ptr(self.fexp) if sr else None, self.sr_flags, ptr(self.raw), st),
                  "dns_feature_block_split")
        else:
            check(lib.dns_feature_block(ptr(fine), self.hid + 1, self.hid, ptr(self.features), self.n_feat - self.hid, ptr(self.z),
                                        ptr(self.gt_depth), N, S, ptr(self.feat), self.n_feat, ptr(self.raw), st), "dns_feature_block")
        fwd(self.feat, pe, self.p_color, self.shp_col, self.raw, None, None, P, 0, self.h_col)
        fwd(self.feat, pe, self.p_logit, self.shp_log, self.logit, None, None, P, 0, self.h_log)
        Cn, L = self.n_class, self.hid + 1
        check(lib.dns_composite_fwd_ex(ptr(self.raw), ptr(self.z), ptr(self.logit), N, S, Cn, ptr(self.depth), ptr(self.var),
                                       ptr(self.rgb), ptr(self.weights), ptr(self.sem), 1, st), "dns_composite_fwd_ex")
        lam = self.lam
        check(lib.dns_loss_sums(lam, N, S, Cn, L, 0, ptr(self.rgb), ptr(self.depth), None, ptr(self.sem), ptr(self.gt_color),
                                ptr(self.gt_depth), ptr(self.gt_label), ptr(self.inside), ptr(fine), ptr(self.coarse),
                                ptr(self.z), ptr(self.sums_ws), st), "dns_loss_sums")
        if self.dist_on:
            m.dist.allreduce_sums(self.sums_ws[:16])

        ldf = 4 + self.n_feat
        d_fine_dst = _V(self.d_featx.data_ptr() + 4 * 3)
        check(lib.dns_loss_finalize_bwd(lam, N, S, Cn, L, 0, ptr(self.sums_ws), ptr(self.out), ptr(self.one), ptr(self.rgb),
                                        ptr(self.depth), None, ptr(self.sem), ptr(self.gt_color), ptr(self.gt_depth),
                                        ptr(self.gt_label), ptr(self.inside), ptr(self.d_color), ptr(self.d_depth), None,
                                        ptr(self.d_sem), st), "dns_loss_finalize_bwd")
        check(lib.dns_composite_bwd_ex(ptr(self.raw), ptr(self.z), ptr(self.logit), N, S, Cn, ptr(self.d_depth), None,
                                       ptr(self.d_color), None, ptr(self.d_sem), ptr(self.d_raw), ptr(self.d_logit), 1, st),
              "dns_composite_bwd_ex")
        check(lib.dns_loss_bwd_points(lam, N, S, Cn, L, ptr(self.out), ptr(self.one), ptr(self.gt_depth), ptr(self.inside), ptr(fine),
                                      ptr(self.coarse), ptr(self.z), d_fine_dst, ptr(self.d_coarse), ldf,
                                      _V(self.d_raw.data_ptr() + 12), 4, st), "dns_loss_bwd_points")

        fork_dwin = on_side and not half
        side_st = _V(self.side.cuda_stream)
        nws = [0]

        def bwd(x2, n_in1, dy, params, shape, d_x2, d_p, ri, tg, n_slots, stride, acc, hs):
            n_in, n_out, nn, nl = shape
            live = 0 if x2 is None else self.live
            ws = self.ws_mlp4[nws[0]] if fork_dwin else self.ws_mlp
            nws[0] += 1
            if half:
                check(lib.dns_mlp_bwd_half(ptr(self.xh), ld, None if x2 is None else ptr(self.feath), self.n_feat, n_in1, ptr(dy),
                                           dy.stride(0), ptr(params), n_in, n_out, nn, nl, ptr(self.d_buf), ld, ptr(d_x2),
                                           0 if d_x2 is None else d_x2.stride(0), ptr(d_p), n_slots, ptr(ri), ptr(tg), stride,
                                           acc | live, self.loss_scale, st), "dns_mlp_bwd_half")
                return
            if sr:
                check(lib.dns_mlp_bwd_split(rows_x, None if x2 is None else rows_f, n_in1, ptr(dy), dy.stride(0), ptr(params), n_in,
                                            n_out, nn, nl, ptr(self.d_buf), ld, ptr(d_x2), 0 if d_x2 is None else d_x2.stride(0),
                                            ptr(d_p), ptr(ws), n_slots, ptr(ri), ptr(tg), stride, acc | fp16, st), "dns_mlp_bwd_split")
                if not fork_dwin:
                    check(lib.dns_mlp_dwin(ptr(self.buf), ld, ptr(x2), 0 if x2 is None else x2.stride(0), n_in1, n_in, nn, nl, ptr(d_p),
                                           ptr(ws), n_slots, ptr(ri), ptr(tg), stride, fp16 | live, st), "dns_mlp_dwin")
            else:
                wp, wflag = self._w(params, n_out)
                check(lib.dns_mlp_bwd(ptr(self.buf), ld, ptr(x2), 0 if x2 is None else x2.stride(0), n_in1, ptr(dy), dy.stride(0),
                                      wp, n_in, n_out, nn, nl, ptr(self.d_buf), ld, ptr(d_x2),
                                      0 if d_x2 is None else d_x2.stride(0), ptr(d_p), ptr(ws), n_slots, ptr(ri), ptr(tg),
                                      stride, ptr(hs), acc | fp16 | wflag | live | (ops.MLP_NO_DWIN_FLAG if fork_dwin else 0), st), "dns_mlp_bwd")
            if fork_dwin:
                ev = torch.cuda.Event()
                ev.record(main)
                self.side.wait_event(ev)
                with torch.cuda.stream(self.side):
                    check(lib.dns_mlp_dwin(ptr(self.buf), ld, ptr(x2), 0 if x2 is None else x2.stride(0), n_in1, n_in, nn, nl, ptr(d_p),
                                           ptr(ws), n_slots, ptr(ri), ptr(tg), stride, fp16 | live, side_st), "dns_mlp_dwin")

        d_feat = self.d_featx[:, 4:]
        bwd(None, 0, self.d_coarse, self.p_coarse, self.shp_c, None, cur.g_coarse, None, None, P, 0, 0, self.h_c)
        bwd(self.feat, pe, self.d_raw, self.p_color, self.shp_col, d_feat, cur.g_color, None, None, P, 0, 3, self.h_col)
        bwd(self.feat, pe, self.d_logit, self.p_logit, self.shp_log, d_feat, cur.g_logit, None, None, P, 0, 3, self.h_log)
        if self.stem:
            n_in_m, n_out_m, nn_m, nl_m = self.shp_m
            pe_m = self.pe_m
            check(lib.dns_merge_dy(_V(self.d_featx.data_ptr() + 4 * (4 + self.hid)), ldf, n_out_m, self.R, self.Pf, ptr(self.z),
                                   ptr(self.gt_depth), N, S, ptr(self.mdy), st), "dns_merge_dy")
            check(lib.dns_mlp_bwd(ptr(self.mbuf), n_in_m, _V(self.mbuf.data_ptr() + 4 * pe_m), n_in_m, pe_m, ptr(self.mdy), n_out_m,
                                  ptr(self.p_merge), n_in_m, n_out_m, nn_m, nl_m, ptr(self.d_mpe), pe_m, None, 0, ptr(cur.g_merge),
                                  ptr(self.ws_m), self.Mr, None, None, 0, None,
                                  ops.MLP_DX_FIRST_FLAG | fp16 | (ops.MLP_NO_DWIN_FLAG if fork_dwin else 0), st), "dns_mlp_bwd")
            if fork_dwin:
                ev = torch.cuda.Event()
                ev.record(main)
                self.side.wait_event(ev)
                with torch.cuda.stream(self.side):
                    check(lib.dns_mlp_dwin(ptr(self.mbuf), n_in_m, None, 0, 0, n_in_m, nn_m, nl_m, ptr(cur.g_merge), ptr(self.ws_m),
                                           self.Mr, None, None, 0, fp16, side_st), "dns_mlp_dwin")
            if self.is_BA:
                check(lib.dns_encode_bwd(ptr(self.xm), self.b6m, self.Mr, self.n_bins_m, None, None, ptr(self.d_mpe), pe_m, None, 0,
                                         None, ptr(self.d_rel), None, None, 0, 0, st), "dns_encode_bwd")
        bwd(None, 0, self.d_featx[:, 3:3 + L], self.p_pool, self.shp_f, None, cur.g_pool, row_index, tile_group,
            self.n_slots, self.p_pool.shape[-1], 1, self.h_f)
        work = None
        if self.dist_on:
            import torch.distributed as dist
            if fork_dwin:
                with torch.cuda.stream(self.side):
                    work = dist.all_reduce(cur.G_early, op=dist.ReduceOp.SUM, group=m.dist.group, async_op=True)
            else:
                work = dist.all_reduce(cur.G_early, op=dist.ReduceOp.SUM, group=m.dist.group, async_op=True)
        d_grid = _V(self.d_buf.data_ptr() + 4 * pe)
        fork_pose = self.is_BA and on_side
        if fork_pose:
            self.side.wait_stream(main)
            with torch.cuda.stream(self.side):
                st2 = _V(self.side.cuda_stream)
                check(lib.dns_encode_bwd(ptr(self.x3), self.b6, P, self.n_bins, ptr(self.p_table), meta, ptr(self.d_buf), ld, d_grid,
                                         ld, None, ptr(self.d_x3), ptr(self.dydx), None, 0, 0, st2), "dns_encode_bwd")
                if self.stem:
                    check(lib.dns_add_ref_sum(ptr(self.d_rel), self.R, self.Pf, P, ptr(self.d_x3), st2), "dns_add_ref_sum")
                check(lib.dns_raygen_bwd(ptr(pix), ptr(self.Q), self.camv, 0, H, 0, W, K, npf, S, ptr(self.z), ptr(self.d_x3), None,
                                         None, ptr(self.ray_ws), ptr(cur.g_quat), ptr(cur.g_trans), st2), "dns_raygen_bwd")
        check(lib.dns_encode_bwd(ptr(self.x3), self.b6, P, self.n_bins, ptr(self.p_table), meta, ptr(self.d_buf), ld, d_grid, ld,
                                 ptr(cur.g_table), ptr(self.d_x3) if (self.is_BA and not fork_pose) else None, ptr(self.dydx),
                                 ptr(self.ws_enc), self.scatter_form, self.scatter_cap, st), "dns_encode_bwd")
        if self.is_BA and not fork_pose:
            if self.stem:
                check(lib.dns_add_ref_sum(ptr(self.d_rel), self.R, self.Pf, P, ptr(self.d_x3), st), "dns_add_ref_sum")
            check(lib.dns_raygen_bwd(ptr(pix), ptr(self.Q), self.camv, 0, H, 0, W, K, npf, S, ptr(self.z), ptr(self.d_x3), None,
                                     None, ptr(self.ray_ws), ptr(cur.g_quat), ptr(cur.g_trans), st), "dns_raygen_bwd")
        if on_side:
            main.wait_stream(self.side)
        if self.dist_on:
            import torch.distributed as dist
            work2 = dist.all_reduce(cur.G_late, op=dist.ReduceOp.SUM, group=m.dist.group, async_op=True)
            work.wait()
            work2.wait()
        check(lib.dns_adam_step(cur.adam_items, self.n_adam, self.betas[0], self.betas[1], self.eps, ptr(self.adam_state), st),
              "dns_adam_step")
        self.steps += 1

    def set_lambda_lt(self, value):
        if getattr(self, "_captured", False) and float(value) != float(self.lam[3]):
            raise RuntimeError("MapStep.set_lambda_lt: the step has been captured into a hipGraph -- the loss weights are kernel "
                               "arguments frozen at capture time; capture one graph per weight schedule phase")
        self.lam[3] = float(value)

    g_table = property(lambda self: self.cur.g_table)
    g_coarse = property(lambda self: self.cur.g_coarse)
    g_color = property(lambda self: self.cur.g_color)
    g_logit = property(lambda self: self.cur.g_logit)
    g_pool = property(lambda self: self.cur.g_pool)
    g_merge = property(lambda self: self.cur.g_merge)
    g_quat = property(lambda self: self.cur.g_quat)
    g_trans = property(lambda self: self.cur.g_trans)

    def losses(self):
        t = self.out
        terms = {"p_loss": t[0], "d_loss": t[1], "l_loss": t[2], "lt_loss": t[3], "fs_loss": t[4], "opacity_loss": t[5]}
        total = t[6]
        if self.smooth:
            terms["smooth_loss"] = self.tv[0]
            total = total + self.w_sm[0] * self.tv[0]
        return total, terms

    @torch.no_grad()
    def write_back(self):
        for k in range(self.K):
            self.quad_list[k].data.copy_(self.Q[k])
            self.T_list[k].data.copy_(self.T[k])

    def pose(self, k):
        bottom = torch.tensor([[0.0, 0.0, 0.0, 1.0]], device=self.dev)
        return torch.cat([torch.cat((get_rotation_from_quad(self.Q[k]), self.T[k][:, None]), -1), bottom], dim=0)


class TrackStep:

    def __init__(self, tracker, cur_frames, est_c2w, features=None, betas=(0.9, 0.999), eps=1e-8, refer_frames=None):
        t = self.t = tracker
        dev = self.dev = torch.device(t.device)
        if dev.type != "cuda":
            raise ValueError("dns_slam_amd ops run on the GPU only; there is no CPU fallback")
        self.stem = features is not None and features.dim() == 5
        if features is not None and features.dim() not in (3, 5):
            raise ValueError("TrackStep: features is the per-sample code [N, S, C] or the stem feature maps [1, R, C, h, w]")
        if self.stem and refer_frames is None:
            raise ValueError("TrackStep: stem feature maps need refer_frames['est_w2c']")
        dec = t.decoder
        self.prep = t.prepare_frame(cur_frames)
        self.features = None if (features is None or self.stem) else features.to(dev).float().contiguous()
        self.betas, self.eps = betas, eps
        self.pe_dim, self.grid_dim, self.hid = dec.pe_dim, dec.grid_dim, dec.hidden_dim
        nets = (dec.coarse_fn.decoder, dec.out_fn.color_decoder, dec.out_fn.logit_decoder)
        self.fp16 = ops.MLP_FP16_FLAG if getattr(nets[0], "fp16", False) else 0
        shp = lambda n: (n.n_input_dims, n.n_output_dims, n.n_neurons, n.n_hidden_layers)
        self.shp_c, self.shp_col, self.shp_log = (shp(n) for n in nets)
        self.p_coarse, self.p_color, self.p_logit = (n.params for n in nets)
        self.p_table, self.meta, self.n_bins = dec.pe_fn.grid_fn.params, dec.pe_fn.grid_fn.meta, dec.pe_fn.pe_fn.n_bins
        self.n_feat = self.hid + (self.hid if (features is None or self.stem) else self.features.shape[-1])
        if not (self.pe_dim % 4 == 0 and self.pe_dim <= 64 and self.n_feat <= 64 and self.n_feat % 4 == 0
                and self.shp_col[0] == self.pe_dim + self.n_feat and self.shp_c[1] == self.hid + 1):
            raise ValueError("TrackStep: network shapes outside the two-segment input form")
        self.n_class = self.shp_log[1]
        N = self.N = int(t.n_pixels)
        nu = self.nu = 0 if t.t_uniform is None else t.t_uniform.numel()
        ns = self.ns = t.n_surface_ray
        S = self.S = nu + ns
        P = self.P = N * S
        ld = self.ld = self.pe_dim + self.grid_dim
        f = lambda *s: torch.empty(*s, device=dev, dtype=torch.float32)
        self.Q = get_quad_from_c2w(est_c2w).detach().to(dev).float().reshape(1, 4).contiguous()
        self.T = est_c2w[:3, 3].detach().clone().to(dev).float().reshape(1, 3).contiguous()
        self.zbuf = torch.zeros(P * ld + 8, device=dev)
        self.d_buf = self.zbuf[:P * ld].view(P, ld)
        self.g_quat, self.g_trans = self.zbuf[P * ld:P * ld + 4], self.zbuf[P * ld + 4:P * ld + 7]
        self.M, self.V, self.adam_state = torch.zeros(8, device=dev), torch.zeros(8, device=dev), torch.zeros(3, device=dev)
        lr = float(t.cam_lr)
        lrT = lr * 0.2 if t.seperate_LR else lr
        self.adam_items = (DnsAdamTensor * 2)()
        for k, (p, g, o, n, l) in enumerate(((self.T, self.g_trans, 4, 3, lrT), (self.Q, self.g_quat, 0, 4, lr))):
            it = self.adam_items[k]
            it.p, it.g, it.m, it.v, it.n, it.lr = p.data_ptr(), g.data_ptr(), self.M.data_ptr() + 4 * o, self.V.data_ptr() + 4 * o, n, l
        self.best_loss = torch.full((1,), float("inf"), device=dev)
        self.best_cam = torch.cat((self.Q.reshape(-1), self.T.reshape(-1))).clone()
        self.rays_o, self.rays_d, self.gt_color, self.gt_depth = f(N, 3), f(N, 3), f(N, 3), f(N)
        self.gt_label = torch.empty(N, device=dev, dtype=torch.int64)
        self.inside, self.valid = torch.empty(N, device=dev, dtype=torch.uint8), torch.empty(N, device=dev, dtype=torch.uint8)
        self.z, self.pts = f(N, S), f(N, S, 3)
        self.dmax_ws = torch.empty(1, device=dev, dtype=torch.int32)
        self.x3, self.buf = f(P, 3), f(P, ld)
        self.dydx = f(self.meta.n_levels * 3 * P * 2)
        nf = self.hid + 1
        self.lat, self.feat = f(P, nf), f(P, self.n_feat)
        self.raw, self.logit = f(P, 4), f(P, self.n_class)
        self.depth, self.var, self.rgb, self.weights, self.sem = f(N), f(N), f(N, 3), f(N, S), f(N, self.n_class)
        self.sums_ws, self.out, self.one = f(ops.LOSS_SUMS_FLOATS), f(16), torch.ones(1, device=dev)
        self.d_color, self.d_depth, self.d_var, self.d_sem = f(N, 3), f(N), f(N), f(N, self.n_class)
        self.d_raw, self.d_logit, self.d_col = f(P, 4), f(P, self.n_class), f(P, 4)
        self.d_featx = torch.zeros(P, 4 + self.n_feat, device=dev)
        self.d_x3 = f(P, 3)
        raw_lib = ops.lib._raw
        if self.stem:
            _, R, Cs, fh, fw = features.shape
            self.R, self.Cs, self.fh, self.fw = int(R), int(Cs), int(fh), int(fw)
            self.feat_maps = features.detach().to(dev).float()[0].permute(0, 2, 3, 1).contiguous()
            mg = dec.merge.decoder
            self.shp_m, self.p_merge = shp(mg), mg.params
            self.n_bins_m = dec.merge.pe_fn.n_bins
            self.pe_m = 3 * self.n_bins_m
            if not (self.shp_m[0] == self.pe_m + Cs and self.shp_m[1] == self.hid and self.pe_m % 4 == 0):
                raise ValueError("TrackStep: Decoder.merge's network does not match the stem features / hidden width")
            self.b6m = ops._bound6(dec.merge.bound)
            w2c = refer_frames["est_w2c"].clone().detach().to(dev).float()
            self.w2c = w2c.reshape(R, 16).contiguous()
            self.origin = torch.inverse(w2c)[:, :3, 3].contiguous()
            Mr = self.Mr = R * P
            self.mbuf, self.rel, self.xm = f(Mr, self.shp_m[0]), f(Mr, 3), f(Mr, 3)
            self.mlat, self.mdy = f(Mr, self.hid), f(Mr, self.hid)
            self.d_mpe, self.d_rel = f(Mr, self.pe_m), f(Mr, 3)
            self.K9 = (C.c_float * 9)(float(t.fx), 0.0, float(t.cx), 0.0, float(t.fy), float(t.cy), 0.0, 0.0, 1.0)
        self.ray_ws = f(max(int(raw_lib.dns_raygen_bwd_ws_floats(1, N)), 1))
        self.PREP = ops.MLP_PREPARED_FLAG
        nets_w = [(self.p_coarse, self.shp_c), (self.p_color, self.shp_col), (self.p_logit, self.shp_log)]
        if self.stem:
            nets_w.append((self.p_merge, self.shp_m))
        self._nets_w = nets_w
        self.w = [f(int(raw_lib.dns_mlp_prepared_floats(*shp_))) for _, shp_ in nets_w]
        self._prepare_weights()
        self.g = None
        self.w_coarse, self.w_color, self.w_logit = self.w[:3]
        self.w_merge = self.w[3] if self.stem else None
        self.lam = (C.c_float * 8)(t.lambda_p, t.lambda_d, t.lambda_l, 0.0, 0.0, 0.0, 0.0, 1.0)
        self.camv = (C.c_double * 4)(float(t.fx), float(t.fy), float(t.cx), float(t.cy))
        self.b6 = ops._bound6(t.bound)
        self.steps = 0

    @torch.no_grad()
    def step(self, draws=None):
        t, lib = self.t, ops.lib
        st = _V(torch.cuda.current_stream().cuda_stream)
        N, S, P, ld, pe, b = self.N, self.S, self.P, self.ld, self.pe_dim, t.border
        H, W = t.H, t.W
        if draws is None:
            pix = torch.randint((H - 2 * b) * (W - 2 * b), (N,), device=self.dev)
            t_surf = torch.rand(self.ns, device=self.dev)
            check(lib.dns_force_half(ptr(t_surf), self.ns, self.ns // 2 + 1, st), "dns_force_half")
            t_zero = torch.rand(self.ns, device=self.dev)
        else:
            pix, t_surf, t_zero = draws
        self._keep = (pix, t_surf, t_zero)
        self.zbuf.zero_()
        prep = self.prep
        check(lib.dns_raygen_sample(ptr(pix), ptr(prep["color"]), ptr(prep["depth"]), ptr(prep["label"]), ptr(self.Q), ptr(self.T),
                                    self.camv, self.b6, H, W, b, H - b, b, W - b, 1, N, ptr(t.t_uniform), ptr(t_surf), ptr(t_zero),
                                    self.nu, self.ns, 0, ptr(self.dmax_ws), 0, ptr(self.rays_o), ptr(self.rays_d),
                                    ptr(self.gt_color), ptr(self.gt_depth), ptr(self.gt_label), ptr(self.inside), ptr(self.z),
                                    ptr(self.pts), st), "dns_raygen_sample")
        check(lib.dns_track_mask(ptr(self.gt_depth), ptr(self.inside), N, 0.01, ptr(self.valid), st), "dns_track_mask")
        meta = C.byref(self.meta.c)
        check(lib.dns_encode_fwd(ptr(self.pts), self.b6, P, self.n_bins, ptr(self.p_table), meta, ptr(self.x3), ptr(self.buf), ld,
                                 _V(self.buf.data_ptr() + 4 * pe), ld, ptr(self.dydx), st), "dns_encode_fwd")
        fp16 = self.fp16 | self.PREP

        def fwd(x2, n_in1, params, shape, y):
            n_in, n_out, nn, nl = shape
            check(lib.dns_mlp_fwd(ptr(self.buf), ld, ptr(x2), 0 if x2 is None else x2.stride(0), n_in1, ptr(params), n_in, n_out,
                                  nn, nl, ptr(y), y.stride(0), P, None, None, 0, None, fp16, st), "dns_mlp_fwd")

        fwd(None, 0, self.w_coarse, self.shp_c, self.lat)
        if self.stem:
            n_in_m, n_out_m, nn_m, nl_m = self.shp_m
            check(lib.dns_feature_gather_frames(ptr(self.pts), ptr(self.w2c), ptr(self.origin), self.K9, ptr(self.feat_maps), 1, self.R,
                                                P, self.Cs, self.fh, self.fw, H, W, _V(self.mbuf.data_ptr() + 4 * self.pe_m), n_in_m,
                                                ptr(self.rel), st), "dns_feature_gather_frames")
            check(lib.dns_encode_fwd(ptr(self.rel), self.b6m, self.Mr, self.n_bins_m, None, None, ptr(self.xm), ptr(self.mbuf), n_in_m,
                                     None, 0, None, st), "dns_encode_fwd")
            check(lib.dns_mlp_fwd(ptr(self.mbuf), n_in_m, None, 0, 0, ptr(self.w_merge), n_in_m, n_out_m, nn_m, nl_m, ptr(self.mlat),
                                  n_out_m, self.Mr, None, None, 0, None, fp16, st), "dns_mlp_fwd")
            check(lib.dns_feature_block_split(ptr(self.lat), self.hid + 1, self.hid, ptr(self.mlat), self.hid, self.R, P, ptr(self.z),
                                              ptr(self.gt_depth), N, S, ptr(self.feat), self.n_feat, None, 0, None, 0, ptr(self.raw), st),
                  "dns_feature_block_split")
        else:
            check(lib.dns_feature_block(ptr(self.lat), self.hid + 1, self.hid, ptr(self.features), self.n_feat - self.hid, ptr(self.z),
                                        ptr(self.gt_depth), N, S, ptr(self.feat), self.n_feat, ptr(self.raw), st), "dns_feature_block")
        fwd(self.feat, pe, self.w_color, self.shp_col, self.raw)
        fwd(self.feat, pe, self.w_logit, self.shp_log, self.logit)
        check(lib.dns_rgb_sigmoid(ptr(self.raw), P, st), "dns_rgb_sigmoid")
        Cn = self.n_class
        check(lib.dns_composite_fwd(ptr(self.raw), ptr(self.z), ptr(self.logit), N, S, Cn, ptr(self.depth), ptr(self.var),
                                    ptr(self.rgb), ptr(self.weights), ptr(self.sem), st), "dns_composite_fwd")
        lam = self.lam
        check(lib.dns_loss_rays(lam, N, 1, Cn, 1, 1, ptr(self.rgb), ptr(self.depth), ptr(self.var), ptr(self.sem), ptr(self.gt_color),
                                ptr(self.gt_depth), ptr(self.gt_label), ptr(self.valid), None, None, None, ptr(self.sums_ws),
                                ptr(self.out), ptr(self.one), ptr(self.d_color), ptr(self.d_depth), ptr(self.d_var), ptr(self.d_sem),
                                st), "dns_loss_rays")
        check(lib.dns_keep_best(_V(self.out.data_ptr() + 4 * 6), ptr(self.Q), ptr(self.T), ptr(self.best_loss), ptr(self.best_cam),
                                st), "dns_keep_best")
        check(lib.dns_composite_bwd(ptr(self.raw), ptr(self.z), ptr(self.logit), N, S, Cn, ptr(self.d_depth), ptr(self.d_var),
                                    ptr(self.d_color), None, ptr(self.d_sem), ptr(self.d_raw), ptr(self.d_logit), st),
              "dns_composite_bwd")
        ldf = 4 + self.n_feat
        check(lib.dns_raw_bwd(ptr(self.d_raw), ptr(self.raw), P, ptr(self.d_col), _V(self.d_featx.data_ptr() + 12), ldf, 0, st),
              "dns_raw_bwd")

        def bwd(x2, n_in1, dy, params, shape, d_x2, acc):
            n_in, n_out, nn, nl = shape
            check(lib.dns_mlp_bwd(ptr(self.buf), ld, ptr(x2), 0 if x2 is None else x2.stride(0), n_in1, ptr(dy), dy.stride(0),
                                  ptr(params), n_in, n_out, nn, nl, ptr(self.d_buf), ld, ptr(d_x2),
                                  0 if d_x2 is None else d_x2.stride(0), None, None, P, None, None, 0, None, acc | fp16, st),
                  "dns_mlp_bwd")

        d_feat = self.d_featx[:, 4:]
        bwd(self.feat, pe, self.d_col, self.w_color, self.shp_col, d_feat, 1)
        bwd(self.feat, pe, self.d_logit, self.w_logit, self.shp_log, d_feat, 3)
        if self.stem:
            n_in_m, n_out_m, nn_m, nl_m = self.shp_m
            pe_m = self.pe_m
            check(lib.dns_merge_dy(_V(self.d_featx.data_ptr() + 4 * (4 + self.hid)), ldf, n_out_m, self.R, P, ptr(self.z),
                                   ptr(self.gt_depth), N, S, ptr(self.mdy), st), "dns_merge_dy")
            check(lib.dns_mlp_bwd(ptr(self.mbuf), n_in_m, _V(self.mbuf.data_ptr() + 4 * pe_m), n_in_m, pe_m, ptr(self.mdy), n_out_m,
                                  ptr(self.w_merge), n_in_m, n_out_m, nn_m, nl_m, ptr(self.d_mpe), pe_m, None, 0, None, None, self.Mr,
                                  None, None, 0, None, ops.MLP_DX_FIRST_FLAG | fp16, st), "dns_mlp_bwd")
            check(lib.dns_encode_bwd(ptr(self.xm), self.b6m, self.Mr, self.n_bins_m, None, None, ptr(self.d_mpe), pe_m, None, 0, None,
                                     ptr(self.d_rel), None, None, 0, 0, st), "dns_encode_bwd")
        bwd(None, 0, self.d_featx[:, 3:3 + self.hid + 1], self.w_coarse, self.shp_c, None, 1)
        check(lib.dns_encode_bwd(ptr(self.x3), self.b6, P, self.n_bins, ptr(self.p_table), meta, ptr(self.d_buf), ld,
                                 _V(self.d_buf.data_ptr() + 4 * pe), ld, None, ptr(self.d_x3), ptr(self.dydx), None, 0, 0, st),
              "dns_encode_bwd")
        if self.stem:
            check(lib.dns_add_ref_sum(ptr(self.d_rel), self.R, P, P, ptr(self.d_x3), st), "dns_add_ref_sum")
        check(lib.dns_raygen_bwd(ptr(pix), ptr(self.Q), self.camv, b, H - b, b, W - b, 1, N, S, ptr(self.z), ptr(self.d_x3), None,
                                 None, ptr(self.ray_ws), ptr(self.g_quat), ptr(self.g_trans), st), "dns_raygen_bwd")
        check(lib.dns_adam_step(self.adam_items, 2, self.betas[0], self.betas[1], self.eps, ptr(self.adam_state), st),
              "dns_adam_step")
        self.steps += 1

    @staticmethod
    def signature(tracker, features, refer_frames):
        t, dec = tracker, tracker.decoder
        nets = [dec.pe_fn.grid_fn.params, dec.coarse_fn.decoder.params, dec.out_fn.color_decoder.params, dec.out_fn.logit_decoder.params]
        fs = None if features is None else tuple(features.shape)
        if features is not None and features.dim() == 5:
            nets.append(dec.merge.decoder.params)
            fs = fs + (tuple(refer_frames["est_w2c"].shape),)
        grid = dec.pe_fn.grid_fn
        meta = getattr(grid, "meta", None)
        meta_key = None
        meta = getattr(meta, "c", meta)
        if meta is not None:
            n_lv = int(meta.n_levels)
            meta_key = (n_lv,) + tuple((float(meta.scale[l]), int(meta.resolution[l]), int(meta.size[l]), int(meta.offset[l]),
                                        int(meta.hashed[l])) for l in range(n_lv))
        extra = (bool(getattr(dec.coarse_fn.decoder, "fp16", False)), str(torch.device(t.device)), meta_key,
                 int(dec.pe_fn.pe_fn.n_bins), 0 if t.t_uniform is None else t.t_uniform.data_ptr())
        if features is not None and features.dim() == 5:
            mb = getattr(dec.merge, "bound", None)
            extra = extra + (None if mb is None else tuple(float(v) for v in torch.as_tensor(mb).reshape(-1)),
                             int(getattr(getattr(dec.merge, "pe_fn", None), "n_bins", 0) or 0))
        return extra + (int(t.n_pixels), 0 if t.t_uniform is None else t.t_uniform.numel(), t.n_surface_ray, t.H, t.W, t.border, fs,
                float(t.lambda_p), float(t.lambda_d), float(t.lambda_l), float(t.cam_lr), bool(t.seperate_LR),
                float(t.fx), float(t.fy), float(t.cx), float(t.cy), tuple(float(v) for v in torch.as_tensor(t.bound).reshape(-1)),
                tuple((p.data_ptr(), p.numel()) for p in nets))

    @torch.no_grad()
    def reset(self, cur_frames, est_c2w, features=None, refer_frames=None):
        t, dev = self.t, self.dev
        for k, v in (("color", cur_frames["gt_color"]), ("depth", cur_frames["gt_depth"]), ("label", cur_frames["gt_label"])):
            self.prep[k].copy_(v.to(dev).float()[None])
        if self.stem:
            self.feat_maps.copy_(features.detach().to(dev).float()[0].permute(0, 2, 3, 1))
            w2c = refer_frames["est_w2c"].clone().detach().to(dev).float()
            self.w2c.copy_(w2c.reshape(self.R, 16))
            self.origin.copy_(torch.inverse(w2c)[:, :3, 3])
        elif self.features is not None:
            self.features.copy_(features.to(dev).float())
        self.Q.copy_(get_quad_from_c2w(est_c2w).detach().to(dev).float().reshape(1, 4))
        self.T.copy_(est_c2w[:3, 3].detach().to(dev).float().reshape(1, 3))
        self.M.zero_()
        self.V.zero_()
        self.adam_state.zero_()
        self.best_loss.fill_(float("inf"))
        self.best_cam.copy_(torch.cat((self.Q.reshape(-1), self.T.reshape(-1))))
        self._prepare_weights()
        self.steps = 0

    def _prepare_weights(self):
        st = _V(torch.cuda.current_stream().cuda_stream)
        for (p_, shp_), w in zip(self._nets_w, self.w):
            check(ops.lib.dns_mlp_prepare(ptr(p_), shp_[0], shp_[1], shp_[2], shp_[3], 1, 0, ptr(w), 0, st), "dns_mlp_prepare")
        if self.features is None and not self.stem:
            live = ops.MLP_LIVE_IN(self.pe_dim + self.hid)
            if getattr(self, "w_live", None) is None:
# ... 115 lines not shown
```

dns_slam_amd/ops.py:

```python
from __future__ import annotations

import ctypes as C
from typing import Optional

import os

import numpy as np
import torch

from ._lib import DnsGridMeta, check, lib as _rawlib, ptr, require_cuda, stream_ptr


class _TimedLib:

    def __init__(self, raw):
        self._raw = raw
        self.records = None
        self.kernels = False

    def __getattr__(self, name):
        fn = getattr(self._raw, name)
        if self.records is None or name in ("dns_grid_meta_init", "dns_mlp_bwd_ws_floats", "dns_mlp_prepared_floats", "dns_encode_bwd_ws_floats", "dns_raygen_bwd_ws_floats", "dns_last_error",
                                            "dns_abi_version", "dns_init") or name.startswith("dns_kernel_timing"):
            return fn

        ui = self._UNITS_ARG.get(name)
        info_of = self._INFO.get(name)

        def timed(*a):
            k0 = self._raw.dns_kernel_timing_count() if self.kernels else 0
            e0 = torch.cuda.Event(enable_timing=True)
            e1 = torch.cuda.Event(enable_timing=True)
            e0.record()
            rc = fn(*a)
            e1.record()
            k1 = self._raw.dns_kernel_timing_count() if self.kernels else 0
            units = 0 if ui is None else (a[ui] if not isinstance(ui, tuple) else a[ui[0]] * a[ui[1]])
            self.records.append((name, e0, e1, int(units), info_of(a) if info_of else None, (k0, k1)))
            return rc
        return timed

    _live = staticmethod(lambda n_in, flags: ((int(flags) >> 16) & 0xff) or n_in)
    @staticmethod
    def _grid_info(meta_ref):
        m = getattr(meta_ref, "_obj", None)
        if m is None:
            return None
        L = int(m.n_levels)
        in_lists = lambda l: 8192 < m.size[l] <= (1 << 20) and (m.hashed[l] or (m.size[l] + 8191) // 8192 >= 6)
        return {"n_levels": L, "list_levels": sum(1 for l in range(L) if in_lists(l))}

    _INFO = {"dns_encode_bwd": lambda a: _TimedLib._grid_info(a[5]),
             "dns_mlp_fwd": lambda a: {"n_in": _TimedLib._live(a[6], a[17]), "n_out": a[7], "nn": a[8], "nl": a[9]},
             "dns_mlp_dwin": lambda a: {"n_in": _TimedLib._live(a[5], a[14]), "n_out": 0, "nn": a[6], "nl": a[7]},
             "dns_mlp_bwd": lambda a: {"n_in": _TimedLib._live(a[8], a[23]), "n_out": a[9], "nn": a[10], "nl": a[11], "dx": bool(a[12]),
                                       "dw": bool(a[16])},
             "dns_mlp_fwd_half": lambda a: {"n_in": _TimedLib._live(a[6], a[16]), "n_out": a[7], "nn": a[8], "nl": a[9]},
             "dns_mlp_bwd_half": lambda a: {"n_in": _TimedLib._live(a[8], a[21]), "n_out": a[9], "nn": a[10], "nl": a[11], "dx": bool(a[12]),
                                            "dw": bool(a[16]), "dx_from": (int(a[21]) >> 24) & 0x7f, "acc": int(a[21]) & 3},
             "dns_mlp_fwd_split": lambda a: {"n_in": a[4], "n_out": a[5], "nn": a[6], "nl": a[7]},
             "dns_mlp_bwd_split": lambda a: {"n_in": a[6], "n_out": a[7], "nn": a[8], "nl": a[9], "dx": bool(a[10]), "dw": bool(a[14])}}

    _UNITS_ARG = {"dns_encode_fwd": 2, "dns_encode_bwd": 2, "dns_mlp_fwd": 12, "dns_mlp_bwd": 18,
                  "dns_composite_fwd": 3, "dns_composite_bwd": 3, "dns_raygen_sample": (14, 15), "dns_raygen_bwd": (7, 8),
                  "dns_rays_from_pixels": 12, "dns_mlp_dwin": 10, "dns_feature_block": (7, 8), "dns_loss_sums": (1, 2),
                  "dns_loss_bwd": (1, 2), "dns_loss_rays": (1, 2), "dns_loss_finalize_bwd": (1, 2), "dns_raw_bwd": 2, "dns_rgb_sigmoid": 1, "dns_class_slots": (1, 2),
                  "dns_hashgrid_indices": 1, "dns_sample_along_rays": 2, "dns_feature_gather": (4, 5),
                  "dns_encode_fwd_split": 2, "dns_mlp_fwd_half": 12, "dns_mlp_bwd_half": 17, "dns_mlp_fwd_split": 10, "dns_mlp_bwd_split": 16, "dns_feature_block_split": (9, 10),
                  "dns_composite_fwd_ex": 3, "dns_composite_bwd_ex": 3, "dns_loss_bwd_points": (1, 2)}

    def arm(self, kernels=False):
        self.kernels = bool(kernels)
        if self.kernels:
            check(self._raw.dns_kernel_timing(1), "dns_kernel_timing")
        self.records = []

    def disarm(self):
        recs, self.records = self.records or [], None
        out = {}
        spans = []
        if self.kernels:
            check(self._raw.dns_kernel_timing(0), "dns_kernel_timing")
            buf, ms = C.create_string_buffer(160), C.c_float()
        for name, e0, e1, units, info, (k0, k1) in recs:
            c, t, u = out.get(name, (0, 0.0, 0))
            out[name] = (c + 1, t + e0.elapsed_time(e1), u + units)
            for k in range(k0, k1):
                check(self._raw.dns_kernel_timing_get(k, buf, 160, C.byref(ms)), "dns_kernel_timing_get")
                spans.append((name, buf.value.decode().strip("()"), float(ms.value), units, info))
        self.kernel_spans, self.kernels = spans, False
        return out


lib = _TimedLib(_rawlib)
timer = lib


class GridMeta:

    def __init__(self, log2_hashmap_size: int, desired_resolution: int, n_levels: int = 16,
                 n_features: int = 2, base_resolution: int = 16, per_level_scale: Optional[float] = None):
        if per_level_scale is None:
            per_level_scale = float(np.exp2(np.log2(desired_resolution / base_resolution) / (n_levels - 1)))
        self.c = DnsGridMeta()
        check(lib.dns_grid_meta_init(C.byref(self.c), n_levels, n_features, log2_hashmap_size, base_resolution,
                                     per_level_scale), "dns_grid_meta_init")
        self.n_levels = n_levels
        self.n_features = n_features
        self.total_rows = int(self.c.total_rows)
        self.out_dim = n_levels * n_features
        self._args = (log2_hashmap_size, desired_resolution, n_levels, n_features, base_resolution, per_level_scale)

    def levels(self):
        c = self.c
        return [dict(scale=np.float32(c.scale[l]), resolution=int(c.resolution[l]), size=int(c.size[l]),
                     offset=int(c.offset[l]), hashed=bool(c.hashed[l])) for l in range(self.n_levels)]

    def __getstate__(self):
        return {"args": self._args}

    def __setstate__(self, st):
        a = st["args"]
        self.__init__(a[0], a[1], a[2], a[3], a[4], a[5])


def _bound6(bound) -> Optional[C.Array]:
    if bound is None:
        return None
    if isinstance(bound, C.Array):
        return bound
    cached = getattr(bound, "_dns_b6", None) if isinstance(bound, torch.Tensor) else None
    if cached is not None:
        return cached
    b = torch.as_tensor(bound, dtype=torch.float64).detach().cpu().reshape(3, 2)
    b6 = (C.c_double * 6)(*[float(v) for v in b.reshape(-1)])
    if isinstance(bound, torch.Tensor):
        try:
            bound._dns_b6 = b6
        except Exception:
            pass
    return b6


SCATTER_AUTO, SCATTER_ATOMIC, SCATTER_BINNED, SCATTER_QUEUES = 0, 1, 2, 3
SCATTER_REPLAY = 0x10
SCATTER_LISTS = 0x20
SCATTER_FORM = (SCATTER_AUTO | (SCATTER_REPLAY if os.environ.get("DNS_SCATTER_REPLAY", "0") == "1" else 0)
                | (SCATTER_LISTS if os.environ.get("DNS_SCATTER_LISTS", "0") == "1" else 0), 0)
SAVE_DY_DX = True


class _EncodeFn(torch.autograd.Function):
    @staticmethod
    def forward(ctx, pts, table, meta: Optional[GridMeta], bound, n_bins: int, want_pe: bool, want_grid: bool):
        require_cuda(pts, table)
        P = pts.shape[0]
        pts = pts.contiguous().float()
        pe_dim = 3 * n_bins if want_pe else 0
        g_dim = meta.out_dim if want_grid else 0
        ld = pe_dim + g_dim
        out = torch.empty(P, ld, device=pts.device, dtype=torch.float32)
        b6 = _bound6(bound)
        x = torch.empty(P, 3, device=pts.device, dtype=torch.float32) if b6 is not None else pts
        pe_ptr = ptr(out) if want_pe else None
        grid_ptr = C.c_void_p(out.data_ptr() + 4 * pe_dim) if want_grid else None
        dydx = torch.empty(meta.n_levels * 3 * P * 2, device=pts.device, dtype=torch.float32) \
            if (want_grid and pts.requires_grad and SAVE_DY_DX) else None
        check(lib.dns_encode_fwd(ptr(pts), b6, P, n_bins, ptr(table) if want_grid else None,
                                 C.byref(meta.c) if want_grid else None,
                                 ptr(x) if b6 is not None else None, pe_ptr, ld, grid_ptr, ld, ptr(dydx), stream_ptr()),
              "dns_encode_fwd")
        ctx.save_for_backward(x, table if want_grid else None, dydx)
        ctx.meta, ctx.b6, ctx.n_bins, ctx.pe_dim, ctx.g_dim = meta, b6, n_bins, pe_dim, g_dim
        ctx.need_x = pts.requires_grad
        return out

    @staticmethod
    def backward(ctx, d_out):
        x, table, dydx = ctx.saved_tensors
        P = x.shape[0]
        d_out = d_out.contiguous()
        ld = ctx.pe_dim + ctx.g_dim
        need_x = ctx.needs_input_grad[0]
        need_t = ctx.g_dim > 0 and ctx.needs_input_grad[1]
        d_x = torch.empty(P, 3, device=x.device, dtype=torch.float32) if need_x else None
        d_table = torch.zeros_like(table) if need_t else None
        d_pe = ptr(d_out) if ctx.pe_dim else None
        d_grid = C.c_void_p(d_out.data_ptr() + 4 * ctx.pe_dim) if ctx.g_dim else None
        form, cap = SCATTER_FORM
        ws = torch.empty(int(lib.dns_encode_bwd_ws_floats(P, C.byref(ctx.meta.c), form, cap)), device=x.device,
                         dtype=torch.float32) if need_t else None
        check(lib.dns_encode_bwd(ptr(x), ctx.b6, P, ctx.n_bins, ptr(table) if ctx.g_dim else None,
                                 C.byref(ctx.meta.c) if ctx.g_dim else None, d_pe, ld, d_grid, ld,
                                 ptr(d_table), ptr(d_x), ptr(dydx) if need_x else None, ptr(ws), form, cap, stream_ptr()),
              "dns_encode_bwd")
        return d_x, d_table, None, None, None, None, None


def encode(pts: torch.Tensor, table: Optional[torch.Tensor], meta: Optional[GridMeta], bound=None, n_bins: int = 16,
           want_pe: bool = True, want_grid: bool = True) -> torch.Tensor:
    if table is None:
        table = pts.new_zeros(1)
    return _EncodeFn.apply(pts, table, meta, bound, n_bins, want_pe, want_grid)


def hashgrid_rows(x: torch.Tensor, meta: GridMeta) -> torch.Tensor:
    require_cuda(x)
    x = x.contiguous().float()
    rows = torch.empty(x.shape[0], meta.n_levels, 8, device=x.device, dtype=torch.int32)
    check(lib.dns_hashgrid_indices(ptr(x), x.shape[0], C.byref(meta.c), ptr(rows), stream_ptr()), "dns_hashgrid_indices")
    return rows.to(torch.int64) & 0xFFFFFFFF


def mlp_out_padded(n_out: int) -> int:
    return (n_out + 15) // 16 * 16


def mlp_param_count(n_in: int, n_out: int, n_neurons: int, n_hidden_layers: int) -> int:
    return n_neurons * n_in + (n_hidden_layers - 1) * n_neurons * n_neurons + mlp_out_padded(n_out) * n_neurons


def _row_major_2d(x: torch.Tensor) -> torch.Tensor:
    if x.dim() != 2 or x.stride(1) != 1 or x.stride(0) % 4 != 0 or x.data_ptr() % 16 != 0:
        x = x.contiguous()
        if x.data_ptr() % 16 != 0:
            x = x.clone()
    return x


LOSS_SUMS_FLOATS = 32 + 5 * 1024
MLP_SAVE_HIDDEN = False
MLP_FP16_FLAG = 0x100
MLP_PREPARED_FLAG = 0x200
MLP_NO_DWIN_FLAG = 0x400
MLP_DX_FIRST_FLAG = 0x800
MLP_DX_FROM = lambda c: int(c) << 24
MLP_LIVE_IN = lambda n: int(n) << 16


class _MlpFn(torch.autograd.Function):

    @staticmethod
    def forward(ctx, x, params, shape, row_index, tile_group, n_slots):
        n_in, n_out, nn, nl = shape[:4]
        fp16 = MLP_FP16_FLAG if (len(shape) > 4 and shape[4]) else 0
        require_cuda(params, row_index, tile_group)
        if not x.is_cuda:
            raise ValueError("dns_slam_amd ops run on the GPU only (got a non-CUDA tensor); there is no CPU fallback")
        x = _row_major_2d(x.float())
        P = x.shape[0]
        if row_index is None:
            y = torch.empty(P, n_out, device=x.device, dtype=torch.float32)
            n_slots = P
        else:
            y = torch.zeros(P, n_out, device=x.device, dtype=torch.float32)
        stride = params.shape[-1] if params.dim() == 2 else 0
        keep = MLP_SAVE_HIDDEN and (ctx.needs_input_grad[0] or ctx.needs_input_grad[1])
        h_save = torch.empty(nl * n_slots * nn, device=x.device, dtype=torch.float32) if keep else None
        check(lib.dns_mlp_fwd(ptr(x), x.stride(0), None, 0, 0, ptr(params), n_in, n_out, nn, nl, ptr(y), n_out, n_slots,
                              ptr(row_index), ptr(tile_group), stride, ptr(h_save), fp16, stream_ptr()), "dns_mlp_fwd")
        ctx.save_for_backward(x, params, row_index, tile_group, h_save)
        ctx.shape, ctx.n_slots, ctx.stride, ctx.fp16 = shape[:4], n_slots, stride, fp16
        return y

    @staticmethod
    def backward(ctx, dy):
        x, params, row_index, tile_group, h_save = ctx.saved_tensors
        n_in, n_out, nn, nl = ctx.shape
        dy = dy.contiguous()
        P = x.shape[0]
        need_x, need_p = ctx.needs_input_grad[0], ctx.needs_input_grad[1]
        if row_index is None:
            d_x = torch.empty(P, n_in, device=x.device, dtype=torch.float32) if need_x else None
        else:
            d_x = torch.zeros(P, n_in, device=x.device, dtype=torch.float32) if need_x else None
        d_p = torch.zeros_like(params) if need_p else None
        ws = torch.empty(int(lib.dns_mlp_bwd_ws_floats(ctx.n_slots, nn, nl)), device=x.device, dtype=torch.float32)
        check(lib.dns_mlp_bwd(ptr(x), x.stride(0), None, 0, 0, ptr(dy), n_out, ptr(params), n_in, n_out, nn, nl,
                              ptr(d_x), n_in, None, 0, ptr(d_p), ptr(ws), ctx.n_slots, ptr(row_index), ptr(tile_group),
                              ctx.stride, ptr(h_save), ctx.fp16, stream_ptr()), "dns_mlp_bwd")
        return d_x, d_p, None, None, None, None


class _MlpCatFn(torch.autograd.Function):

    @staticmethod
    def forward(ctx, x1, x2, params, shape):
        n_in, n_out, nn, nl = shape[:4]
        fp16 = MLP_FP16_FLAG if (len(shape) > 4 and shape[4]) else 0
        require_cuda(params)
        if not (x1.is_cuda and x2.is_cuda):
            raise ValueError("dns_slam_amd ops run on the GPU only (got a non-CUDA tensor); there is no CPU fallback")
        x1, x2 = _row_major_2d(x1.float()), _row_major_2d(x2.float())
        P, n1 = x1.shape
        y = torch.empty(P, n_out, device=x1.device, dtype=torch.float32)
        h_save = torch.empty(nl * P * nn, device=x1.device, dtype=torch.float32) if MLP_SAVE_HIDDEN else None
        check(lib.dns_mlp_fwd(ptr(x1), x1.stride(0), ptr(x2), x2.stride(0), n1, ptr(params), n_in, n_out, nn, nl, ptr(y),
                              n_out, P, None, None, 0, ptr(h_save), fp16, stream_ptr()), "dns_mlp_fwd")
        ctx.save_for_backward(x1, x2, params, h_save)
        ctx.shape, ctx.fp16 = shape[:4], fp16
        return y

    @staticmethod
    def backward(ctx, dy):
        x1, x2, params, h_save = ctx.saved_tensors
        n_in, n_out, nn, nl = ctx.shape
        dy = dy.contiguous()
        P, n1 = x1.shape
        need_x = ctx.needs_input_grad[0] or ctx.needs_input_grad[1]
        d1 = torch.empty(P, n1, device=x1.device, dtype=torch.float32) if need_x else None
        d2 = torch.empty(P, n_in - n1, device=x1.device, dtype=torch.float32) if need_x else None
        d_p = torch.zeros_like(params) if ctx.needs_input_grad[2] else None
        ws = torch.empty(int(lib.dns_mlp_bwd_ws_floats(P, nn, nl)), device=x1.device, dtype=torch.float32)
        check(lib.dns_mlp_bwd(ptr(x1), x1.stride(0), ptr(x2), x2.stride(0), n1, ptr(dy), n_out, ptr(params), n_in, n_out, nn, nl,
                              ptr(d1), n1, ptr(d2), n_in - n1, ptr(d_p), ptr(ws), P, None, None, 0, ptr(h_save), ctx.fp16,
                              stream_ptr()), "dns_mlp_bwd")
        return (d1 if ctx.needs_input_grad[0] else None), (d2 if ctx.needs_input_grad[1] else None), d_p, None


def mlp_cat(x1: torch.Tensor, x2: torch.Tensor, params: torch.Tensor, n_out: int, n_neurons: int = 32,
            n_hidden_layers: int = 1, fp16: bool = False) -> torch.Tensor:
    n1, n2 = x1.shape[-1], x2.shape[-1]
    ok = (n1 % 4 == 0 and n2 % 4 == 0 and 0 < n1 <= 64 and 0 < n2 <= 64 and x1.dim() == 2 and x2.dim() == 2
          and x1.stride(-1) == 1 and x2.stride(-1) == 1 and x1.stride(0) % 4 == 0 and x2.stride(0) % 4 == 0
          and x1.data_ptr() % 16 == 0 and x2.data_ptr() % 16 == 0 and x1.dtype == torch.float32 and x2.dtype == torch.float32)
    if not ok:
        return mlp(torch.cat((x1, x2), -1), params, n1 + n2, n_out, n_neurons, n_hidden_layers, fp16)
    return _MlpCatFn.apply(x1, x2, params, (n1 + n2, n_out, n_neurons, n_hidden_layers, bool(fp16)))


def mlp(x: torch.Tensor, params: torch.Tensor, n_in: int, n_out: int, n_neurons: int = 32,
        n_hidden_layers: int = 1, fp16: bool = False) -> torch.Tensor:
    return _MlpFn.apply(x, params, (n_in, n_out, n_neurons, n_hidden_layers, bool(fp16)), None, None, 0)


HALF_LOSS_SCALE = 128.0
SPLIT_PLAIN = 2


def _cuda_rows(*tensors):
    for t in tensors:
        if t is None:
            continue
        if not isinstance(t, torch.Tensor) or not t.is_cuda:
            raise ValueError("dns_slam_amd ops run on the GPU only (got a non-CUDA tensor); there is no CPU fallback")
        if t.dim() == 2 and t.stride(1) != 1:
            raise ValueError("dns_slam_amd ops need unit column stride")


def _half_rows_ok(t):
    return t is None or (t.is_cuda and t.dtype == torch.float16 and t.dim() == 2 and t.stride(1) == 1)


def mlp_fwd_half(x, params, n_in, n_out, n_neurons, n_hidden_layers, x2=None, row_index=None, tile_group=None, n_slots=None,
                 param_stride=0, live_in=0, out=None):
    _cuda_rows(x, x2, out)
    require_cuda(params)
    if not (_half_rows_ok(x) and _half_rows_ok(x2)):
        raise ValueError("mlp_fwd_half: x / x2 must be 2-D float16 CUDA tensors with unit column stride")
    rows = x.shape[0]
    n_slots = rows if n_slots is None else n_slots
    y = out if out is not None else torch.zeros(rows, n_out, device=x.device, dtype=torch.float32)
    n_in1 = x.shape[1] if x2 is not None else 0
    check(lib.dns_mlp_fwd_half(ptr(x), x.stride(0), ptr(x2), 0 if x2 is None else x2.stride(0), n_in1, ptr(params), n_in, n_out,
                               n_neurons, n_hidden_layers, ptr(y), y.stride(0), n_slots, ptr(row_index), ptr(tile_group), param_stride,
                               MLP_LIVE_IN(live_in) if live_in else 0, stream_ptr()), "dns_mlp_fwd_half")
    return y


def mlp_bwd_half(x, dy, params, n_in, n_out, n_neurons, n_hidden_layers, x2=None, d_x=None, d_x2=None, d_params=None, row_index=None,
                 tile_group=None, n_slots=None, param_stride=0, accumulate=0, loss_scale=HALF_LOSS_SCALE):
    _cuda_rows(x, x2, dy, d_x, d_x2)
# ... 464 lines not shown
```

include/dns_hip.h:

```cpp
#ifndef DNS_HIP_H
#define DNS_HIP_H

#include <stdint.h>

#ifdef __cplusplus
extern "C" {
#endif

#define DNS_ABI_VERSION 13
#define DNS_MAX_LEVELS 32

#define DNS_OK 0
#define DNS_E_ARG (-1)
#define DNS_E_LAUNCH (-2)
#define DNS_E_STATE (-3)

typedef struct DnsGridMeta {
  uint32_t n_levels;
  uint32_t n_features;
  uint32_t log2_hashmap_size;
  uint32_t base_resolution;
  uint32_t total_rows;
  float per_level_scale;
  float scale[DNS_MAX_LEVELS];
  uint32_t resolution[DNS_MAX_LEVELS];
  uint32_t size[DNS_MAX_LEVELS];
  uint32_t offset[DNS_MAX_LEVELS];
  uint32_t hashed[DNS_MAX_LEVELS];
} DnsGridMeta;

int dns_abi_version(void);
const char* dns_last_error(void);

int dns_init(void);

int dns_kernel_timing(int enable);
int dns_kernel_timing_count(void);
int dns_kernel_timing_get(int i, char* name, int name_cap, float* ms);

int dns_grid_meta_init(DnsGridMeta* meta, uint32_t n_levels, uint32_t n_features,
                       uint32_t log2_hashmap_size, uint32_t base_resolution, double per_level_scale);

int dns_raygen_sample(const int64_t* pix_idx, const float* color, const float* depth, const float* label,
                      const float* quat, const float* trans, const double* cam, const double* bound,
                      int H, int W, int H0, int H1, int W0, int W1, int n_frames, int n_per_frame,
                      const float* t_uniform, const float* t_surf, const float* t_zero,
                      int n_uniform, int n_surface, int jitter_stride, uint32_t* depth_max_ws, int depth_max_given,
                      float* rays_o, float* rays_d, float* gt_color, float* gt_depth, int64_t* gt_label,
                      uint8_t* inside, float* z, float* pts ,
                      void* stream);

int dns_rays_from_pixels(const int64_t* pix_idx, const float* image, int C, const float* R, const float* T,
                         const double* cam, int H, int W, int H0, int H1, int W0, int W1, int n,
                         float* rays_o, float* rays_d, float* sample, float* ij, void* stream);

int dns_sample_along_rays(const float* gt_depth, const double* far_bb, int n_rays, const float* t_uniform,
                          const float* t_surf, const float* t_zero, int n_uniform, int n_surface,
                          uint32_t* depth_max_ws, float* z, void* stream);

int dns_raygen_bwd(const int64_t* pix_idx, const float* quat, const double* cam,
                   int H0, int H1, int W0, int W1, int n_frames, int n_per_frame, int S,
                   const float* z, const float* d_pts, const float* d_rays_o, const float* d_rays_d,
                   float* ws, float* d_quat, float* d_trans, void* stream);
uint64_t dns_raygen_bwd_ws_floats(int n_frames, int n_per_frame);

int dns_encode_fwd(const float* in, const double* bound, uint32_t P, uint32_t n_bins,
                   const float* table, const DnsGridMeta* meta,
                   float* x_out, float* pe_out, uint32_t ld_pe, float* grid_out, uint32_t ld_grid,
                   float* dy_dx, void* stream);

typedef struct DnsSplitRows {
  const void* rows;
  const int32_t* exps;
  uint32_t ld;
  uint32_t lo_off;
} DnsSplitRows;
#define DNS_SPLIT_HI_ONLY 1u
#define DNS_SPLIT_PLAIN 2u
int dns_encode_fwd_split(const float* in, const double* bound, uint32_t P, uint32_t n_bins, const float* table,
                         const DnsGridMeta* meta, float* x_out, float* f32_out, uint32_t ld32, void* xs_out, uint32_t ldxs,
                         int32_t* xexp, uint32_t flags, float* dy_dx, void* stream);

#define DNS_SCATTER_AUTO 0u
#define DNS_SCATTER_ATOMIC 1u
#define DNS_SCATTER_BINNED 2u
#define DNS_SCATTER_QUEUES 3u
#define DNS_SCATTER_MASK 3u
#define DNS_SCATTER_REPLAY 0x10u
#define DNS_SCATTER_LISTS 0x20u
int dns_encode_bwd(const float* x, const double* bound, uint32_t P, uint32_t n_bins,
                   const float* table, const DnsGridMeta* meta,
                   const float* d_pe, uint32_t ld_dpe, const float* d_grid, uint32_t ld_dgrid,
                   float* d_table, float* d_x, const float* dy_dx, float* ws, uint32_t flags, uint32_t queue_cap,
                   void* stream);
uint64_t dns_encode_bwd_ws_floats(uint32_t P, const DnsGridMeta* meta, uint32_t flags, uint32_t queue_cap);

int dns_hashgrid_indices(const float* x, uint32_t P, const DnsGridMeta* meta, uint32_t* rows, void* stream);

#define DNS_MLP_FP16 0x100u
#define DNS_MLP_PREPARED 0x200u
#define DNS_MLP_NO_DWIN 0x400u
#define DNS_MLP_DX_FIRST 0x800u
#define DNS_MLP_LIVE_IN(n) ((uint32_t)(n) << 16)
#define DNS_MLP_DX_FROM(c) ((uint32_t)(c) << 24)
int dns_mlp_dwin(const float* x, uint32_t ldx, const float* x2, uint32_t ldx2, uint32_t n_in1, uint32_t n_in, uint32_t n_neurons,
                 uint32_t n_hidden_layers, float* d_params, const float* ws, uint32_t n_slots, const int32_t* row_index,
                 const int32_t* tile_group, uint32_t param_stride, uint32_t flags, void* stream);
uint64_t dns_mlp_prepared_floats(uint32_t n_in, uint32_t n_out, uint32_t n_neurons, uint32_t n_hidden_layers);
int dns_mlp_prepare(const float* params, uint32_t n_in, uint32_t n_out, uint32_t n_neurons, uint32_t n_hidden_layers,
                    uint32_t n_sets, uint32_t param_stride, float* prepared, uint32_t flags, void* stream);
int dns_mlp_fwd(const float* x, uint32_t ldx, const float* x2, uint32_t ldx2, uint32_t n_in1,
                const float* params, uint32_t n_in, uint32_t n_out,
                uint32_t n_neurons, uint32_t n_hidden_layers, float* y, uint32_t ldy, uint32_t n_slots,
                const int32_t* row_index, const int32_t* tile_group, uint32_t param_stride,
                float* h_save ,
                uint32_t flags , void* stream);

int dns_mlp_bwd(const float* x, uint32_t ldx, const float* x2, uint32_t ldx2, uint32_t n_in1,
                const float* dy, uint32_t lddy, const float* params,
                uint32_t n_in, uint32_t n_out, uint32_t n_neurons, uint32_t n_hidden_layers,
                float* d_x, uint32_t lddx, float* d_x2, uint32_t lddx2, float* d_params, float* ws, uint32_t n_slots,
                const int32_t* row_index, const int32_t* tile_group, uint32_t param_stride, const float* h_saved,
                int accumulate_dx, void* stream);
uint64_t dns_mlp_bwd_ws_floats(uint32_t n_slots, uint32_t n_neurons, uint32_t n_hidden_layers);
int dns_mlp_fwd_split(const DnsSplitRows* x, const DnsSplitRows* x2, uint32_t n_in1, const float* params, uint32_t n_in,
                      uint32_t n_out, uint32_t n_neurons, uint32_t n_hidden_layers, float* y, uint32_t ldy, uint32_t n_slots,
                      const int32_t* row_index, const int32_t* tile_group, uint32_t param_stride, uint32_t flags, void* stream);
int dns_mlp_bwd_split(const DnsSplitRows* x, const DnsSplitRows* x2, uint32_t n_in1, const float* dy, uint32_t lddy,
                      const float* params, uint32_t n_in, uint32_t n_out, uint32_t n_neurons, uint32_t n_hidden_layers,
                      float* d_x, uint32_t lddx, float* d_x2, uint32_t lddx2, float* d_params, float* ws, uint32_t n_slots,
                      const int32_t* row_index, const int32_t* tile_group, uint32_t param_stride, int accumulate_dx,
                      void* stream);

int dns_mlp_fwd_half(const void* x, uint32_t ldx, const void* x2, uint32_t ldx2, uint32_t n_in1, const float* params, uint32_t n_in,
                     uint32_t n_out, uint32_t n_neurons, uint32_t n_hidden_layers, float* y, uint32_t ldy, uint32_t n_slots,
                     const int32_t* row_index, const int32_t* tile_group, uint32_t param_stride, uint32_t flags, void* stream);
int dns_mlp_bwd_half(const void* x, uint32_t ldx, const void* x2, uint32_t ldx2, uint32_t n_in1, const float* dy, uint32_t lddy,
                     const float* params, uint32_t n_in, uint32_t n_out, uint32_t n_neurons, uint32_t n_hidden_layers, float* d_x,
                     uint32_t lddx, float* d_x2, uint32_t lddx2, float* d_params, uint32_t n_slots, const int32_t* row_index,
                     const int32_t* tile_group, uint32_t param_stride, int accumulate_dx, float loss_scale, void* stream);

int dns_composite_fwd(const float* raw, const float* z, const float* logits, uint32_t N, uint32_t S, uint32_t C,
                      float* depth, float* var, float* rgb, float* weights, float* sem, void* stream);
int dns_composite_bwd(const float* raw, const float* z, const float* logits, uint32_t N, uint32_t S, uint32_t C,
                      const float* d_depth, const float* d_var, const float* d_rgb, const float* d_weights,
                      const float* d_sem, float* d_raw, float* d_logits, void* stream);

#define DNS_COMPOSITE_RGB_LOGITS 1u
int dns_composite_fwd_ex(const float* raw, const float* z, const float* logits, uint32_t N, uint32_t S, uint32_t C, float* depth,
                         float* var, float* rgb, float* weights, float* sem, uint32_t flags, void* stream);
int dns_composite_bwd_ex(const float* raw, const float* z, const float* logits, uint32_t N, uint32_t S, uint32_t C,
                         const float* d_depth, const float* d_var, const float* d_rgb, const float* d_weights, const float* d_sem,
                         float* d_raw, float* d_logits, uint32_t flags, void* stream);

#define DNS_LOSS_SUMS_FLOATS (32 + 5 * 1024)
int dns_loss_rays(const float* lambdas, uint32_t N, uint32_t S, uint32_t C, uint32_t L, int tracker,
                  const float* pred_color, const float* pred_depth, const float* pred_var, const float* pred_logits,
                  const float* gt_color, const float* gt_depth, const int64_t* gt_label, const uint8_t* valid,
                  const float* fine, const float* coarse, const float* z, float* sums, float* out, const float* g_total,
                  float* d_color, float* d_depth, float* d_var, float* d_logits, void* stream);
int dns_loss_finalize_bwd(const float* lambdas, uint32_t N, uint32_t S, uint32_t C, uint32_t L, int tracker,
                          const float* sums, float* out, const float* g_total, const float* pred_color,
                          const float* pred_depth, const float* pred_var, const float* pred_logits, const float* gt_color,
                          const float* gt_depth, const int64_t* gt_label, const uint8_t* valid, float* d_color,
                          float* d_depth, float* d_var, float* d_logits, void* stream);
int dns_loss_sums(const float* lambdas, uint32_t N, uint32_t S, uint32_t C, uint32_t L, int tracker,
                  const float* pred_color, const float* pred_depth, const float* pred_var, const float* pred_logits,
                  const float* gt_color, const float* gt_depth, const int64_t* gt_label, const uint8_t* valid,
                  const float* fine, const float* coarse, const float* z, float* sums, void* stream);
int dns_loss_finalize(const float* lambdas, uint32_t N, uint32_t S, uint32_t C, uint32_t L, int tracker,
                      const float* sums, float* out, void* stream);
int dns_loss_bwd(const float* lambdas, uint32_t N, uint32_t S, uint32_t C, uint32_t L, int tracker,
                 const float* out, const float* g_total, const float* pred_color, const float* pred_depth,
                 const float* pred_var, const float* pred_logits, const float* gt_color, const float* gt_depth,
                 const int64_t* gt_label, const uint8_t* valid, const float* fine, const float* coarse, const float* z,
                 float* d_color, float* d_depth, float* d_var, float* d_logits, float* d_fine, float* d_coarse,
                 uint32_t ldd_fine, void* stream);

int dns_loss_bwd_points(const float* lambdas, uint32_t N, uint32_t S, uint32_t C, uint32_t L, const float* out,
                        const float* g_total, const float* gt_depth, const uint8_t* valid, const float* fine, const float* coarse,
                        const float* z, float* d_fine, float* d_coarse, uint32_t ldd_fine, const float* d_occ, uint32_t ld_occ,
                        void* stream);

typedef struct DnsAdamTensor {
  float* p;
  const float* g;
  float* m;
  float* v;
  uint64_t n;
  float lr;
} DnsAdamTensor;
int dns_adam_step(const DnsAdamTensor* tensors, uint32_t n_tensors, float beta1, float beta2, float eps,
                  float* state, void* stream);

typedef struct DnsTrackFused {
  const float* color;
  const float* depth;
  const float* label;
  int32_t H, W, H0, H1, W0, W1;
  const double* cam;
  const double* bound;
  const int64_t* pix;
  const float* t_uniform;
  const float* t_surf;
  const float* t_zero;
  const uint32_t* dmax;
  uint32_t* iter;
  uint32_t n_iters;
  uint32_t n_uniform, n_surface, n_rays;
  float* quat;
  float* trans;
  const float* table;
  const DnsGridMeta* meta;
  uint32_t n_bins;
  const float* w_coarse;
  const float* w_color;
  const float* w_logit;
  uint32_t n_neurons, n_hidden_layers, hidden, n_feat, n_class;
  const float* code;
  uint32_t code_dim;
  float lambda_p, lambda_d, lambda_l;
  float* ws;
  float* adam_m;
  float* adam_v;
  float* adam_state;
  float lr_quat, lr_trans, beta1, beta2, eps;
  float* best_loss;
  float* best_cam;
  float* out;
  float* g_quat;
  float* g_trans;
} DnsTrackFused;
uint64_t dns_track_fused_ws_floats(const DnsTrackFused* a);
int dns_track_fused_begin(const int64_t* pix_all, uint32_t n_rays, uint32_t n_iters, const float* depth, int W, int H0, int W0,
                          int W1, float* t_surf_all, uint32_t n_surface, uint32_t* dmax_all, void* stream);
int dns_track_fused_iter(const DnsTrackFused* a, void* stream);

int dns_tv_fwd(const float* lat, uint32_t ld, uint32_t nx, uint32_t n, int halo, uint32_t sample_points, float* out,
               void* stream);
int dns_tv_bwd(const float* lat, uint32_t ld, uint32_t nx, uint32_t n, int halo, uint32_t sample_points, const float* g,
               float* d_lat, void* stream);

int dns_group_slots(const int64_t* slot_of_point, uint32_t P, uint32_t n_groups, uint32_t min_count, uint32_t n_slots,
                    uint32_t* ws, int32_t* row_index, int32_t* tile_group, void* stream);

int dns_device_error(int clear);
int dns_group_scatter(const int64_t* slot_of_point, uint32_t P, uint32_t n_groups, uint32_t* cursor, uint32_t n_slots,
                      int32_t* row_index, void* stream);

int dns_class_slots(const int64_t* labels, uint32_t N, uint32_t S, int tiled, const int64_t* lut, uint32_t n_lut,
                    int64_t* slot_of_point, void* stream);
int dns_feature_block(const float* fine, uint32_t ld_fine, uint32_t hidden, const float* code, uint32_t C, const float* z,
                      const float* gt_depth, uint32_t N, uint32_t S, float* feat, uint32_t ld_feat, float* raw, void* stream);
int dns_feature_block_split(const float* fine, uint32_t ld_fine, uint32_t hidden, const float* code, uint32_t C, uint32_t n_ref,
                            uint32_t pts_per_frame, const float* z, const float* gt_depth, uint32_t N, uint32_t S, float* feat,
                            uint32_t ld_feat, void* xs_out, uint32_t ldxs, int32_t* xexp, uint32_t flags, float* raw, void* stream);
int dns_rgb_sigmoid(float* raw, uint32_t P, void* stream);
int dns_raw_bwd(const float* d_raw, const float* raw, uint32_t P, float* d_col, float* d_occ, uint32_t ld_occ, int accumulate,
                void* stream);
int dns_lattice_points(const float* r6, const double* consts9, uint32_t n, const int32_t* order, uint32_t count, float* pts,
                       void* stream);
int dns_draw_finish(const int64_t* i1, const double* u, const double* count_f64, const int64_t* count_m1,
                    const int64_t* start_flat, const int64_t* sorted_flat, const float* depth, const float* label,
                    uint32_t n_frames, uint32_t n1, uint32_t n2, uint32_t HW, int64_t* pix, int64_t* labels, uint32_t* dmax,
                    void* stream);
int dns_track_mask(const float* gt_depth, const uint8_t* inside, uint32_t N, float min_depth, uint8_t* valid, void* stream);
int dns_keep_best(const float* loss, const float* quat, const float* trans, float* best_loss, float* best_cam, void* stream);
int dns_force_half(float* t, uint32_t n, uint32_t idx, void* stream);

int dns_feature_gather(const float* pts, const float* w2c, const float* K, const float* feat, uint32_t R, uint32_t P,
                       uint32_t C, int h, int w, int H, int W, float* code, uint8_t* mask, void* stream);

int dns_feature_gather_frames(const float* pts, const float* w2c, const float* origin, const float* K, const float* feat,
                              uint32_t n_frames, uint32_t R, uint32_t pts_per_frame, uint32_t C, int h, int w, int H, int W,
                              float* code, uint32_t ld_code, float* rel_out, void* stream);
int dns_refer_poses(const float* quat, const float* trans, const int32_t* src, const float* fixed_c2w, uint32_t n, float* w2c,
                    float* origin, void* stream);
int dns_merge_dy(float* d_code, uint32_t ld_dcode, uint32_t C, uint32_t R, uint32_t pts_per_frame, const float* z,
                 const float* gt_depth, uint32_t N, uint32_t S, float* d_lat, void* stream);
int dns_add_ref_sum(const float* d_rel, uint32_t R, uint32_t pts_per_frame, uint32_t P, float* d_pts, void* stream);

uint64_t dns_mc_ws_bytes(uint32_t nx, uint32_t ny, uint32_t nz);
int dns_mc_count(const float* vol, uint32_t nx, uint32_t ny, uint32_t nz, float level, void* ws, uint64_t* totals, void* stream);
int dns_mc_emit(const float* vol, uint32_t nx, uint32_t ny, uint32_t nz, float level, const double* origin, const double* spacing,
                const void* ws, float* verts, uint64_t v_cap, int32_t* faces, uint64_t f_cap, void* stream);

int dns_keyframe_project(const float* pts, uint32_t P, const float* w2c, uint32_t K, const float* labels, const float* max_depth,
                         int H, int W, const float* intr, float* label, uint8_t* seen, void* stream);

#ifdef __cplusplus
}
#endif
#endif
```

Measured before the change: 170.1 million.

## Fuse ray compositing, loss forward and backward into one per-ray kernel

```diff
diff --git a/dns_slam_amd/_lib.py b/dns_slam_amd/_lib.py
--- a/dns_slam_amd/_lib.py
+++ b/dns_slam_amd/_lib.py
@@ -6,7 +6,7 @@
 _HERE = os.path.dirname(os.path.abspath(__file__))
 LIB_PATH = os.environ.get("DNS_HIP_LIB") or os.path.join(_HERE, "libdns_hip.so")
 DNS_MAX_LEVELS = 32
-ABI_VERSION = 13
+ABI_VERSION = 14
 
 
 class DnsGridMeta(C.Structure):
@@ -88,6 +88,10 @@
     "dns_loss_bwd": (C.c_int, [_P, _U, _U, _U, _U, _I, _P, _P, _P, _P, _P, _P, _P, _P, _P, _P, _P, _P, _P, _P, _P, _P, _P,
                                 _P, _P, _U, _P]),
     "dns_loss_bwd_points": (C.c_int, [_P, _U, _U, _U, _U, _P, _P, _P, _P, _P, _P, _P, _P, _P, _U, _P, _U, _P]),
+    "dns_ray_losses_ws_floats": (C.c_uint64, [_U]),
+    "dns_loss_mask_counts": (C.c_int, [_P, _U, _U, _P, _P, _P, _P, _P]),
+    "dns_ray_losses": (C.c_int, [_P, _U, _U, _U, _U] + [_P] * 20 + [_U, _U, _P]),
+    "dns_ray_losses_finalize": (C.c_int, [_P, _U, _U, _U, _U, _P, _P, _P]),
     "dns_composite_fwd_ex": (C.c_int, [_P, _P, _P, _U, _U, _U, _P, _P, _P, _P, _P, _U, _P]),
     "dns_composite_bwd_ex": (C.c_int, [_P, _P, _P, _U, _U, _U, _P, _P, _P, _P, _P, _P, _P, _U, _P]),
     "dns_class_slots": (C.c_int, [_P, _U, _U, _I, _P, _U, _P, _P]),
diff --git a/dns_slam_amd/csrc/composite.hip b/dns_slam_amd/csrc/composite.hip
--- a/dns_slam_amd/csrc/composite.hip
+++ b/dns_slam_amd/csrc/composite.hip
@@ -16,26 +16,8 @@
   float* wl = lds + wave * (64 * E);
   RayState<E> st;
   ray_forward<E>(raw, zv, n, S, lane, st);
-  float sv = 0.f, sc[3] = {0.f, 0.f, 0.f};
-#pragma unroll
-  for (int e = 0; e < E; ++e) {
-    const uint32_t s = lane * E + e;
-    const float t = st.z[e] - st.depth;
-    sv += st.w[e] * t * t;
-    if (s < S) {
-      const float* r = raw + ((size_t)n * S + s) * 4;
-      const float c0 = rgbl ? sigmoid1c(r[0]) : r[0], c1 = rgbl ? sigmoid1c(r[1]) : r[1], c2 = rgbl ? sigmoid1c(r[2]) : r[2];
-      sc[0] += st.w[e] * c0;
-      sc[1] += st.w[e] * c1;
-      sc[2] += st.w[e] * c2;
-      if (weights) weights[(size_t)n * S + s] = st.w[e];
-    }
-    wl[s] = st.w[e];
-  }
-  sv = wave_sum(sv);
-  sc[0] = wave_sum(sc[0]);
-  sc[1] = wave_sum(sc[1]);
-  sc[2] = wave_sum(sc[2]);
+  float sv, sc[3];
+  ray_render<E>(st, raw + (size_t)n * S * 4, S, lane, rgbl, weights ? weights + (size_t)n * S : nullptr, wl, sv, sc);
   if (lane == 0) {
     depth[n] = st.depth;
     var[n] = sv;
@@ -43,14 +25,7 @@
     rgb[(size_t)n * 3 + 1] = sc[1];
     rgb[(size_t)n * 3 + 2] = sc[2];
   }
-  if (C) {
-    for (uint32_t c = lane; c < C; c += 64) {
-      float acc = 0.f;
-      const float* lp = logits + (size_t)n * S * C + c;
-      for (uint32_t s = 0; s < S; ++s) acc += wl[s] * lp[(size_t)s * C];
-      sem[(size_t)n * C + c] = acc;
-    }
-  }
+  if (C) ray_sem(logits + (size_t)n * S * C, S, C, lane, wl, sem + (size_t)n * C);
 }
 
 template <int E>
@@ -76,62 +51,9 @@
     gc[1] = d_rgb[(size_t)n * 3 + 1];
     gc[2] = d_rgb[(size_t)n * 3 + 2];
   }
-  float g[E];
-  float col[E][3];
-  float gbar = 0.f;
-#pragma unroll
-  for (int e = 0; e < E; ++e) {
-    const uint32_t s = lane * E + e;
-    g[e] = 0.f;
-    col[e][0] = col[e][1] = col[e][2] = 0.f;
-    if (s < S) {
-      const float* r = raw + ((size_t)n * S + s) * 4;
-      const float t = st.z[e] - st.depth;
-      col[e][0] = rgbl ? sigmoid1c(r[0]) : r[0];
-      col[e][1] = rgbl ? sigmoid1c(r[1]) : r[1];
-      col[e][2] = rgbl ? sigmoid1c(r[2]) : r[2];
-      float v = gc[0] * col[e][0] + gc[1] * col[e][1] + gc[2] * col[e][2] + gD * st.z[e] + gV * t * t;
-      if (d_weights) v += d_weights[(size_t)n * S + s];
-      if (C && d_sem) {
-        const float* lp = logits + ((size_t)n * S + s) * C;
-        const float* gs = d_sem + (size_t)n * C;
-        float dot = 0.f;
-        for (uint32_t c = 0; c < C; ++c) dot += gs[c] * lp[c];
-        v += dot;
-      }
-      g[e] = v;
-    }
-    gbar += st.w[e] * g[e];
-    wl[s] = st.w[e];
-  }
-  gbar = wave_sum(gbar);
-  float du[E], lsum = 0.f;
-#pragma unroll
-  for (int e = 0; e < E; ++e) {
-    du[e] = (g[e] - gbar) / st.sumu;
-    lsum += du[e] * st.u[e];
-  }
-  const float after = wave_suffix_excl_sum(lsum, lane);
-  float tail = after;
-#pragma unroll
-  for (int e = E - 1; e >= 0; --e) {
-    const uint32_t s = lane * E + e;
-    const float dalpha = du[e] * st.T[e] - tail / st.om[e];
-    tail += du[e] * st.u[e];
-    if (s < S) {
-      float* o = d_raw + ((size_t)n * S + s) * 4;
-      float o0 = st.w[e] * gc[0], o1 = st.w[e] * gc[1], o2 = st.w[e] * gc[2];
-      if (rgbl) {
-        o0 = o0 * (1.f - col[e][0]) * col[e][0];
-        o1 = o1 * (1.f - col[e][1]) * col[e][1];
-        o2 = o2 * (1.f - col[e][2]) * col[e][2];
-      }
-      o[0] = o0;
-      o[1] = o1;
-      o[2] = o2;
-      o[3] = 10.0f * st.alpha[e] * (1.0f - st.alpha[e]) * dalpha;
-    }
-  }
+  ray_backward<E>(st, raw + (size_t)n * S * 4, logits + (size_t)n * S * C, S, C, lane, gD, gV, gc,
+                  d_weights ? d_weights + (size_t)n * S : nullptr, d_sem ? d_sem + (size_t)n * C : nullptr, wl,
+                  d_raw + (size_t)n * S * 4, rgbl, nullptr);
   if (C && d_logits) {
     for (uint32_t c = lane; c < C; c += 64) {
       const float gs = d_sem ? d_sem[(size_t)n * C + c] : 0.f;
diff --git a/dns_slam_amd/csrc/dev_composite.hpp b/dns_slam_amd/csrc/dev_composite.hpp
--- a/dns_slam_amd/csrc/dev_composite.hpp
+++ b/dns_slam_amd/csrc/dev_composite.hpp
@@ -73,4 +73,104 @@
   st.depth = wave_sum(sd);
 }
 
+template <int E>
+__device__ __forceinline__ void ray_render(const RayState<E>& st, const float* __restrict__ raw_r, uint32_t S, uint32_t lane,
+                                           uint32_t rgbl, float* __restrict__ weights_r, float* wl, float& sv, float (&sc)[3]) {
+  sv = 0.f;
+  sc[0] = sc[1] = sc[2] = 0.f;
+#pragma unroll
+  for (int e = 0; e < E; ++e) {
+    const uint32_t s = lane * E + e;
+    const float t = st.z[e] - st.depth;
+    sv += st.w[e] * t * t;
+    if (s < S) {
+      const float* r = raw_r + (size_t)s * 4;
+      const float c0 = rgbl ? sigmoid1c(r[0]) : r[0], c1 = rgbl ? sigmoid1c(r[1]) : r[1], c2 = rgbl ? sigmoid1c(r[2]) : r[2];
+      sc[0] += st.w[e] * c0;
+      sc[1] += st.w[e] * c1;
+      sc[2] += st.w[e] * c2;
+      if (weights_r) weights_r[s] = st.w[e];
+    }
+    wl[s] = st.w[e];
+  }
+  sv = wave_sum(sv);
+  sc[0] = wave_sum(sc[0]);
+  sc[1] = wave_sum(sc[1]);
+  sc[2] = wave_sum(sc[2]);
 }
+
+__device__ __forceinline__ void ray_sem(const float* __restrict__ logits_r, uint32_t S, uint32_t C, uint32_t lane, const float* wl,
+                                        float* sem_r) {
+  for (uint32_t c = lane; c < C; c += 64) {
+    float acc = 0.f;
+    const float* lp = logits_r + c;
+    for (uint32_t s = 0; s < S; ++s) acc += wl[s] * lp[(size_t)s * C];
+    sem_r[c] = acc;
+  }
+}
+
+template <int E>
+__device__ __forceinline__ void ray_backward(const RayState<E>& st, const float* __restrict__ raw_r,
+                                             const float* __restrict__ logits_r, uint32_t S, uint32_t C, uint32_t lane, float gD,
+                                             float gV, const float (&gc)[3], const float* __restrict__ d_weights_r, const float* gs,
+                                             float* wl, float* __restrict__ d_raw_r, uint32_t rgbl, float* docc_l) {
+  float g[E];
+  float col[E][3];
+  float gbar = 0.f;
+#pragma unroll
+  for (int e = 0; e < E; ++e) {
+    const uint32_t s = lane * E + e;
+    g[e] = 0.f;
+    col[e][0] = col[e][1] = col[e][2] = 0.f;
+    if (s < S) {
+      const float* r = raw_r + (size_t)s * 4;
+      const float t = st.z[e] - st.depth;
+      col[e][0] = rgbl ? sigmoid1c(r[0]) : r[0];
+      col[e][1] = rgbl ? sigmoid1c(r[1]) : r[1];
+      col[e][2] = rgbl ? sigmoid1c(r[2]) : r[2];
+      float v = gc[0] * col[e][0] + gc[1] * col[e][1] + gc[2] * col[e][2] + gD * st.z[e] + gV * t * t;
+      if (d_weights_r) v += d_weights_r[s];
+      if (C && gs) {
+        const float* lp = logits_r + (size_t)s * C;
+        float dot = 0.f;
+        for (uint32_t c = 0; c < C; ++c) dot += gs[c] * lp[c];
+        v += dot;
+      }
+      g[e] = v;
+    }
+    gbar += st.w[e] * g[e];
+    wl[s] = st.w[e];
+  }
+  gbar = wave_sum(gbar);
+  float du[E], lsum = 0.f;
+#pragma unroll
+  for (int e = 0; e < E; ++e) {
+    du[e] = (g[e] - gbar) / st.sumu;
+    lsum += du[e] * st.u[e];
+  }
+  const float after = wave_suffix_excl_sum(lsum, lane);
+  float tail = after;
+#pragma unroll
+  for (int e = E - 1; e >= 0; --e) {
+    const uint32_t s = lane * E + e;
+    const float dalpha = du[e] * st.T[e] - tail / st.om[e];
+    tail += du[e] * st.u[e];
+    if (s < S) {
+      float* o = d_raw_r + (size_t)s * 4;
+      float o0 = st.w[e] * gc[0], o1 = st.w[e] * gc[1], o2 = st.w[e] * gc[2];
+      if (rgbl) {
+        o0 = o0 * (1.f - col[e][0]) * col[e][0];
+        o1 = o1 * (1.f - col[e][1]) * col[e][1];
+        o2 = o2 * (1.f - col[e][2]) * col[e][2];
+      }
+      const float o3 = 10.0f * st.alpha[e] * (1.0f - st.alpha[e]) * dalpha;
+      o[0] = o0;
+      o[1] = o1;
+      o[2] = o2;
+      o[3] = o3;
+      if (docc_l) docc_l[s] = o3;
+    }
+  }
+}
+
+}
diff --git a/dns_slam_amd/csrc/losses.hip b/dns_slam_amd/csrc/losses.hip
--- a/dns_slam_amd/csrc/losses.hip
+++ b/dns_slam_amd/csrc/losses.hip
@@ -1,5 +1,6 @@
 #include <stdlib.h>
 #include "common.hpp"
+#include "dev_composite.hpp"
 
 namespace dns {
 
@@ -33,39 +34,43 @@
 struct RayTerms {
   float sp, sd, sl, nv, nd;
 };
+__device__ __forceinline__ RayTerms ray_terms_vals(const LossCfg& c, bool ok, const float* pc, float pd, float pv, const float* lg,
+                                                   const float* gc, float gd, int64_t lab) {
+  RayTerms r = {0.f, 0.f, 0.f, 0.f, 0.f};
+  if (ok) {
+    r.nv = 1.f;
+#pragma unroll
+    for (int k = 0; k < 3; ++k) {
+      const float e = gc[k] - pc[k];
+      r.sp += e * e;
+    }
+    if (c.tracker) {
+      r.sd = fabsf(gd - pd) / sqrtf(pv + 1e-10f);
+      r.nd = 1.f;
+    } else if (gd > 0.f) {
+      r.sd = fabsf(gd - pd);
+      r.nd = 1.f;
+    }
+    if (c.C) {
+      float mx = -INFINITY;
+      for (uint32_t k = 0; k < c.C; ++k) mx = fmaxf(mx, lg[k]);
+      float se = 0.f;
+      for (uint32_t k = 0; k < c.C; ++k) se += expf(lg[k] - mx);
+      const float ll = (lab >= 0 && lab < (int64_t)c.C) ? lg[lab] : 0.f;
+      r.sl = (mx + logf(se)) - ll;
+    }
+  }
+  return r;
+}
+
 __device__ __forceinline__ RayTerms ray_terms(const LossCfg& c, uint32_t n, const float* __restrict__ pred_color,
                                               const float* __restrict__ pred_depth, const float* __restrict__ pred_var,
                                               const float* __restrict__ logits, const float* __restrict__ gt_color,
                                               const float* __restrict__ gt_depth, const int64_t* __restrict__ gt_label,
                                               const uint8_t* __restrict__ valid) {
-  RayTerms r = {0.f, 0.f, 0.f, 0.f, 0.f};
-  if (n < c.N && ray_valid(valid, n)) {
-    r.nv = 1.f;
-#pragma unroll
-    for (int k = 0; k < 3; ++k) {
-      const float e = gt_color[(size_t)n * 3 + k] - pred_color[(size_t)n * 3 + k];
-      r.sp += e * e;
-    }
-    const float gd = gt_depth[n];
-    if (c.tracker) {
-      r.sd = fabsf(gd - pred_depth[n]) / sqrtf(pred_var[n] + 1e-10f);
-      r.nd = 1.f;
-    } else if (gd > 0.f) {
-      r.sd = fabsf(gd - pred_depth[n]);
-      r.nd = 1.f;
-    }
-    if (c.C) {
-      const float* lg = logits + (size_t)n * c.C;
-      float mx = -INFINITY;
-      for (uint32_t k = 0; k < c.C; ++k) mx = fmaxf(mx, lg[k]);
-      float se = 0.f;
-      for (uint32_t k = 0; k < c.C; ++k) se += expf(lg[k] - mx);
-      const int64_t lab = gt_label[n];
-      const float ll = (lab >= 0 && lab < (int64_t)c.C) ? lg[lab] : 0.f;
-      r.sl = (mx + logf(se)) - ll;
-    }
-  }
-  return r;
+  if (!(n < c.N && ray_valid(valid, n))) return RayTerms{0.f, 0.f, 0.f, 0.f, 0.f};
+  return ray_terms_vals(c, true, pred_color + (size_t)n * 3, pred_depth[n], c.tracker ? pred_var[n] : 0.f,
+                        c.C ? logits + (size_t)n * c.C : nullptr, gt_color + (size_t)n * 3, gt_depth[n], c.C ? gt_label[n] : 0);
 }
 
 __global__ __launch_bounds__(256) void loss_ray_sums_kernel(LossCfg c, const float* __restrict__ pred_color,
@@ -237,6 +242,38 @@
   finalize_terms(c, sums, out);
 }
 
+__device__ __forceinline__ void ray_bwd_vals(const LossCfg& c, const float* out, float g, bool ok, const float* pc, float pd, float pv,
+                                             const float* lg, const float* gc, float gd, int64_t lab, float* dcol, float& dd, float& dv,
+                                             float* dl) {
+#pragma unroll
+  for (int k = 0; k < 3; ++k) dcol[k] = ok ? -g * out[O_CP] * (gc[k] - pc[k]) : 0.f;
+  dd = 0.f;
+  dv = 0.f;
+  if (ok) {
+    const float e = gd - pd;
+    const float sg = e > 0.f ? -1.f : (e < 0.f ? 1.f : 0.f);
+    if (c.tracker) {
+      const float sv = sqrtf(pv + 1e-10f);
+      dd = g * out[O_CD] * sg / sv;
+      dv = g * out[O_CD] * fabsf(e) * (-0.5f) / (sv * sv * sv);
+    } else if (gd > 0.f) {
+      dd = g * out[O_CD] * sg;
+    }
+  }
+  if (c.C) {
+    if (!ok) {
+      for (uint32_t k = 0; k < c.C; ++k) dl[k] = 0.f;
+    } else {
+      float mx = -INFINITY;
+      for (uint32_t k = 0; k < c.C; ++k) mx = fmaxf(mx, lg[k]);
+      float se = 0.f;
+      for (uint32_t k = 0; k < c.C; ++k) se += expf(lg[k] - mx);
+      const float cl = g * out[O_CL];
+      for (uint32_t k = 0; k < c.C; ++k) dl[k] = cl * (expf(lg[k] - mx) / se - ((int64_t)k == lab ? 1.f : 0.f));
+    }
+  }
+}
+
 __device__ __forceinline__ void ray_bwd_one(const LossCfg& c, const float* out, float g, uint32_t n,
                                             const float* __restrict__ pred_color, const float* __restrict__ pred_depth,
                                             const float* __restrict__ pred_var, const float* __restrict__ logits,
@@ -245,39 +282,12 @@
                                             float* __restrict__ d_color, float* __restrict__ d_depth, float* __restrict__ d_var,
                                             float* __restrict__ d_logits) {
   const bool ok = ray_valid(valid, n);
-#pragma unroll
-  for (int k = 0; k < 3; ++k)
-    d_color[(size_t)n * 3 + k] = ok ? -g * out[O_CP] * (gt_color[(size_t)n * 3 + k] - pred_color[(size_t)n * 3 + k]) : 0.f;
-  const float gd = gt_depth[n];
-  float dd = 0.f, dv = 0.f;
-  if (ok) {
-    const float e = gd - pred_depth[n];
-    const float sg = e > 0.f ? -1.f : (e < 0.f ? 1.f : 0.f);
-    if (c.tracker) {
-      const float sv = sqrtf(pred_var[n] + 1e-10f);
-      dd = g * out[O_CD] * sg / sv;
-      dv = g * out[O_CD] * fabsf(e) * (-0.5f) / (sv * sv * sv);
-    } else if (gd > 0.f) {
-      dd = g * out[O_CD] * sg;
-    }
-  }
+  float dd, dv;
+  ray_bwd_vals(c, out, g, ok, pred_color + (size_t)n * 3, ok ? pred_depth[n] : 0.f, (ok && c.tracker) ? pred_var[n] : 0.f,
+               c.C ? logits + (size_t)n * c.C : nullptr, gt_color + (size_t)n * 3, gt_depth[n], (ok && c.C) ? gt_label[n] : 0,
+               d_color + (size_t)n * 3, dd, dv, c.C ? d_logits + (size_t)n * c.C : nullptr);
   d_depth[n] = dd;
   if (d_var) d_var[n] = dv;
-  if (c.C) {
-    const float* lg = logits + (size_t)n * c.C;
-    float* dl = d_logits + (size_t)n * c.C;
-    if (!ok) {
-      for (uint32_t k = 0; k < c.C; ++k) dl[k] = 0.f;
-    } else {
-      float mx = -INFINITY;
-      for (uint32_t k = 0; k < c.C; ++k) mx = fmaxf(mx, lg[k]);
-      float se = 0.f;
-      for (uint32_t k = 0; k < c.C; ++k) se += expf(lg[k] - mx);
-      const int64_t lab = gt_label[n];
-      const float cl = g * out[O_CL];
-      for (uint32_t k = 0; k < c.C; ++k) dl[k] = cl * (expf(lg[k] - mx) / se - ((int64_t)k == lab ? 1.f : 0.f));
-    }
-  }
 }
 
 __global__ __launch_bounds__(256) void loss_ray_bwd_kernel(LossCfg c, const float* __restrict__ out,
@@ -362,6 +372,30 @@
                 d_logits);
 }
 
+__device__ __forceinline__ void loss_point_bwd_elem(const LossCfg& c, float clt, float cfs, float cop, uint32_t p, uint32_t k,
+                                                    uint32_t n, bool ok, float f, float co, float df0,
+                                                    const float* __restrict__ z, const float* __restrict__ gt_depth, float& df,
+                                                    float& dc) {
+  df = df0;
+  dc = 0.f;
+  if (!ok) return;
+  const float d0 = co - f;
+  dc = clt * d0;
+  df -= clt * d0;
+  if (k + 1 == c.L) {
+    const float d = gt_depth[n], zz = z[p];
+    const float occ = sigmoid10f(f);
+    const float front = zz < (d - c.truncation) ? 1.f : 0.f;
+    const float back = zz > (d + c.truncation) ? 1.f : 0.f;
+    const float dm = d > 0.f ? 1.f : 0.f;
+    const float om = (1.f - front) * (1.f - back) * dm;
+    const float r = (zz - d) / c.sigma;
+    const float pseudo = 0.5f * expf(-0.5f * r * r);
+    const float docc = cfs * (occ * front * dm) * (front * dm) + cop * (occ * om - pseudo * om) * om;
+    df += docc * 10.f * occ * (1.f - occ);
+  }
+}
+
 __global__ __launch_bounds__(256) void loss_point_bwd_kernel(LossCfg c, const float* __restrict__ out,
                                                              const float* __restrict__ g_total,
                                                              const float* __restrict__ fine,
@@ -375,24 +409,7 @@
   const float g = g_total[0];
   const float clt = g * out[O_CLT], cfs = g * out[O_CFS], cop = g * out[O_COP];
   auto elem = [&](uint32_t p, uint32_t k, uint32_t n, bool ok, float f, float co, float& df, float& dc) {
-    df = (k == 0 && d_occ) ? d_occ[(size_t)p * ld_occ] : 0.f;
-    dc = 0.f;
-    if (!ok) return;
-    const float d0 = co - f;
-    dc = clt * d0;
-    df -= clt * d0;
-    if (k + 1 == c.L) {
-      const float d = gt_depth[n], zz = z[p];
-      const float occ = sigmoid10f(f);
-      const float front = zz < (d - c.truncation) ? 1.f : 0.f;
-      const float back = zz > (d + c.truncation) ? 1.f : 0.f;
-      const float dm = d > 0.f ? 1.f : 0.f;
-      const float om = (1.f - front) * (1.f - back) * dm;
-      const float r = (zz - d) / c.sigma;
-      const float pseudo = 0.5f * expf(-0.5f * r * r);
-      const float docc = cfs * (occ * front * dm) * (front * dm) + cop * (occ * om - pseudo * om) * om;
-      df += docc * 10.f * occ * (1.f - occ);
-    }
+    loss_point_bwd_elem(c, clt, cfs, cop, p, k, n, ok, f, co, (k == 0 && d_occ) ? d_occ[(size_t)p * ld_occ] : 0.f, z, gt_depth, df, dc);
   };
   const uint32_t gtid = blockIdx.x * blockDim.x + threadIdx.x, stride = gridDim.x * blockDim.x;
   const bool vec = ((((uintptr_t)fine) | ((uintptr_t)coarse) | ((uintptr_t)d_coarse)) & 15u) == 0;
@@ -438,6 +455,250 @@
     elem(p, k, n, ray_valid(valid, n), fine[e], coarse[e], df, dc);
     d_fine[(size_t)p * ldd_fine + k] = df;
     d_coarse[e] = dc;
+  }
+}
+
+constexpr uint32_t CNT_BLOCKS = 256;
+constexpr uint32_t RW_CNT = 16, RW_RAYS = 16 + 4 * CNT_BLOCKS;
+
+__global__ __launch_bounds__(256) void loss_mask_counts_kernel(LossCfg c, const float* __restrict__ gt_depth,
+                                                               const uint8_t* __restrict__ valid, const float* __restrict__ z,
+                                                               float* __restrict__ cnt_part) {
+  __shared__ float sh[4];
+  const uint32_t P = c.N * c.S;
+  float nv = 0.f, nd = 0.f, nfr = 0.f, nom = 0.f;
+#pragma unroll 4
+  for (uint32_t e = blockIdx.x * blockDim.x + threadIdx.x; e < P; e += gridDim.x * blockDim.x) {
+    const uint32_t n = e / c.S;
+    const bool ok = ray_valid(valid, n);
+    const float d = gt_depth[n], zz = z[e];
+    const float front = zz < (d - c.truncation) ? 1.f : 0.f;
+    const float back = zz > (d + c.truncation) ? 1.f : 0.f;
+    const float dm = d > 0.f ? 1.f : 0.f;
+    const float om = (1.f - front) * (1.f - back) * dm;
+    nfr += ok ? front : 0.f;
+    nom += ok ? om : 0.f;
+    const bool first = ok && e == n * c.S;
+    nv += first ? 1.f : 0.f;
+    nd += first ? dm : 0.f;
+  }
+  const float vals[4] = {nv, nd, nfr, nom};
+#pragma unroll
+  for (int i = 0; i < 4; ++i) {
+    const float t = block_sum(vals[i], sh);
+    if (threadIdx.x == 0) cnt_part[i * CNT_BLOCKS + blockIdx.x] = t;
+  }
+}
+
+template <int E>
+__global__ __launch_bounds__(256) void ray_losses_kernel(LossCfg c, const float* __restrict__ raw, const float* __restrict__ zv,
+                                                         const float* __restrict__ logits, const float* __restrict__ gt_color,
+                                                         const float* __restrict__ gt_depth, const int64_t* __restrict__ gt_label,
+                                                         const uint8_t* __restrict__ valid, const float* __restrict__ fine,
+                                                         const float* __restrict__ coarse, const float* __restrict__ g_total,
+                                                         const float* __restrict__ cnt_part, float* __restrict__ ray_part,
+                                                         float* __restrict__ depth, float* __restrict__ var, float* __restrict__ rgb,
+                                                         float* __restrict__ weights, float* __restrict__ sem,
+                                                         float* __restrict__ d_raw, float* __restrict__ d_logits,
+                                                         float* __restrict__ d_fine, float* __restrict__ d_coarse, uint32_t ldd_fine,
+                                                         uint32_t rgbl, uint32_t stage_logits, uint32_t wstride) {
+  extern __shared__ float4 lds4[];
+  __shared__ float s_cnt[16];
+  constexpr uint32_t SE = 64 * E;
+  constexpr int U = 4;
+  const uint32_t lane = threadIdx.x & 63u, wave = threadIdx.x >> 6;
+  const uint32_t n = blockIdx.x * 4 + wave;
+  const bool live = n < c.N;
+  const uint32_t S = c.S, C = c.C, L = c.L;
+  const uint32_t LC = stage_logits ? ((S * C + 3u) & ~3u) : 0u;
+  float* raw_l = reinterpret_cast<float*>(lds4) + (size_t)wave * wstride;
+  float* lg_l = raw_l + 4 * SE;
+  float* z_l = lg_l + LC;
+  float* wl = z_l + SE;
+  float* docc_l = wl + SE;
+  float* sem_l = docc_l + SE;
+  float* gs_l = sem_l + C;
+
+  const uint32_t a0 = n * S * L, b0 = a0 + S * L;
+  const bool vec = ((((uintptr_t)fine) | ((uintptr_t)coarse) | ((uintptr_t)d_coarse)) & 15u) == 0;
+  const uint32_t qa = (a0 + 3u) / 4u, qb = b0 / 4u;
+  const bool hasq = live && vec && qa < qb;
+  const float4* __restrict__ f4p = reinterpret_cast<const float4*>(fine);
+  const float4* __restrict__ c4p = reinterpret_cast<const float4*>(coarse);
+  float4 fv[U], cv[U];
+  auto load_trip = [&](uint32_t qw) {
+#pragma unroll
+    for (int u = 0; u < U; ++u) {
+      const uint32_t q = qw + lane + 64u * (uint32_t)u;
+      const uint32_t qc = q < qb ? q : qb - 1u;
+      fv[u] = f4p[qc];
+      cv[u] = c4p[qc];
+    }
+  };
+  if (live) {
+    const float4* r4 = reinterpret_cast<const float4*>(raw) + (size_t)n * S;
+    float4 rr[E];
+    float zr[E];
+#pragma unroll
+    for (int e = 0; e < E; ++e) {
+      const uint32_t i = lane + 64u * (uint32_t)e;
+      const uint32_t ic = i < S ? i : S - 1u;
+      rr[e] = r4[ic];
+      zr[e] = zv[(size_t)n * S + ic];
+    }
+    if (hasq) load_trip(qa);
+    if (stage_logits) {
+      const uint32_t TL = S * C;
+      const float* lb = logits + (size_t)n * TL;
+      if ((((uintptr_t)lb) & 15u) == 0 && (TL & 3u) == 0) {
+#pragma unroll 2
+        for (uint32_t i = lane; i < TL / 4u; i += 64u) reinterpret_cast<float4*>(lg_l)[i] = reinterpret_cast<const float4*>(lb)[i];
+      } else {
+#pragma unroll 4
+        for (uint32_t i = lane; i < TL; i += 64u) lg_l[i] = lb[i];
+      }
+    }
+#pragma unroll
+    for (int e = 0; e < E; ++e) {
+      const uint32_t i = lane + 64u * (uint32_t)e;
+      if (i < S) {
+        reinterpret_cast<float4*>(raw_l)[i] = rr[e];
+        z_l[i] = zr[e];
+      }
+    }
+  }
+  {
+    float v[4];
+#pragma unroll
+    for (int i = 0; i < 4; ++i) v[i] = wave_sum(cnt_part[i * CNT_BLOCKS + threadIdx.x]);
+    if (lane == 0) {
+#pragma unroll
+      for (int i = 0; i < 4; ++i) s_cnt[wave * 4 + i] = v[i];
+    }
+  }
+  __syncthreads();
+  if (!live) return;
+  float sums16[S_COUNT], co[16];
+#pragma unroll
+  for (int i = 0; i < S_COUNT; ++i) sums16[i] = 0.f;
+  {
+    const int dst[4] = {S_NV, S_ND, S_NFRONT, S_NOMASK};
+#pragma unroll
+    for (int i = 0; i < 4; ++i) sums16[dst[i]] = (s_cnt[i] + s_cnt[4 + i]) + (s_cnt[8 + i] + s_cnt[12 + i]);
+  }
+  finalize_terms(c, sums16, co);
+  const float g = g_total[0];
+  const float clt = g * co[O_CLT], cfs = g * co[O_CFS], cop = g * co[O_COP];
+
+  RayState<E> st;
+  ray_forward<E>(raw_l, z_l, 0u, S, lane, st);
+  float sv, sc[3];
+  ray_render<E>(st, raw_l, S, lane, rgbl, weights ? weights + (size_t)n * S : nullptr, wl, sv, sc);
+  const float* lg_r = stage_logits ? lg_l : logits + (size_t)n * S * C;
+  if (C) ray_sem(lg_r, S, C, lane, wl, sem_l);
+  const bool ok = ray_valid(valid, n);
+  const float gd = gt_depth[n];
+  const float gcol[3] = {gt_color[(size_t)n * 3], gt_color[(size_t)n * 3 + 1], gt_color[(size_t)n * 3 + 2]};
+  const int64_t lab = C ? gt_label[n] : 0;
+  const RayTerms rt = ray_terms_vals(c, ok, sc, st.depth, 0.f, sem_l, gcol, gd, lab);
+  if (lane == 0) {
+    depth[n] = st.depth;
+    if (var) var[n] = sv;
+    rgb[(size_t)n * 3 + 0] = sc[0];
+    rgb[(size_t)n * 3 + 1] = sc[1];
+    rgb[(size_t)n * 3 + 2] = sc[2];
+  }
+  for (uint32_t k = lane; k < C; k += 64u) sem[(size_t)n * C + k] = sem_l[k];
+  float dcol[3], dd, dv;
+  ray_bwd_vals(c, co, g, ok, sc, st.depth, 0.f, sem_l, gcol, gd, lab, dcol, dd, dv, gs_l);
+  ray_backward<E>(st, raw_l, lg_r, S, C, lane, dd, 0.f, dcol, nullptr, C ? gs_l : nullptr, wl, d_raw + (size_t)n * S * 4, rgbl, docc_l);
+  if (C) {
+    float* dl = d_logits + (size_t)n * S * C;
+    for (uint32_t i = lane; i < S * C; i += 64u) {
+      const uint32_t s = i / C;
+      dl[i] = wl[s] * gs_l[i - s * C];
+    }
+  }
+  PointAcc acc = {0.f, 0.f, 0.f, 0.f, 0.f};
+  auto one = [&](uint32_t p, uint32_t k, float f, float cc, float& df, float& dc) {
+    loss_point_bwd_elem(c, clt, cfs, cop, p, k, n, ok, f, cc, k == 0 ? docc_l[p - n * S] : 0.f, zv, gt_depth, df, dc);
+    if (ok) loss_point_elem(c, f, cc, p, k, n, zv, gt_depth, nullptr, acc);
+  };
+  auto scalar = [&](uint32_t e) {
+    const uint32_t p = e / L, k = e - p * L;
+    float df, dc;
+    one(p, k, fine[e], coarse[e], df, dc);
+    d_fine[(size_t)p * ldd_fine + k] = df;
+    d_coarse[e] = dc;
+  };
+  const uint32_t head_end = hasq ? 4u * qa : b0, tail_beg = hasq ? 4u * qb : b0;
+#pragma unroll 4
+  for (uint32_t e = a0 + lane; e < head_end; e += 64u) scalar(e);
+  for (uint32_t e = tail_beg + lane; e < b0; e += 64u) scalar(e);
+  if (hasq) {
+    for (uint32_t qw = qa;;) {
+#pragma unroll
+      for (int u = 0; u < U; ++u) {
+        const uint32_t q = qw + lane + 64u * (uint32_t)u;
+        if (q < qb) {
+          const uint32_t e0 = 4u * q;
+          uint32_t p = e0 / L, k = e0 - p * L;
+          const float f4[4] = {fv[u].x, fv[u].y, fv[u].z, fv[u].w}, c4[4] = {cv[u].x, cv[u].y, cv[u].z, cv[u].w};
+          float dcv[4];
+#pragma unroll
+          for (int j = 0; j < 4; ++j) {
+            float df;
+            one(p, k, f4[j], c4[j], df, dcv[j]);
+            d_fine[(size_t)p * ldd_fine + k] = df;
+            if (++k == L) {
+              k = 0;
+              ++p;
+            }
+          }
+          *reinterpret_cast<float4*>(d_coarse + e0) = make_float4(dcv[0], dcv[1], dcv[2], dcv[3]);
+        }
+      }
+      qw += 64u * U;
+      if (qw >= qb) break;
+      load_trip(qw);
+    }
+  }
+  const float slt = wave_sum(acc.slt), sfs = wave_sum(acc.sfs), sop = wave_sum(acc.sop);
+  if (lane == 0) {
+    const float vals[6] = {rt.sp, rt.sd, rt.sl, slt, sfs, sop};
+#pragma unroll
+    for (int i = 0; i < 6; ++i) ray_part[(size_t)i * c.N + n] = vals[i];
+  }
+}
+
+__global__ __launch_bounds__(1024) void ray_losses_finalize_kernel(LossCfg c, const float* __restrict__ cnt_part,
+                                                                   const float* __restrict__ ray_part, float* __restrict__ sums,
+                                                                   float* __restrict__ out) {
+  __shared__ float sh[16];
+  __shared__ float s_sums[S_COUNT], s_out[16];
+  if (threadIdx.x < S_COUNT) s_sums[threadIdx.x] = 0.f;
+  const int dn[6] = {S_P, S_D, S_L, S_LT, S_FS, S_OP};
+#pragma unroll
+  for (int i = 0; i < 6; ++i) {
+    float v = 0.f;
+    for (uint32_t n = threadIdx.x; n < c.N; n += blockDim.x) v += ray_part[(size_t)i * c.N + n];
+    const float t = block_sum(v, sh);
+    if (threadIdx.x == 0) s_sums[dn[i]] = t;
+  }
+  const int dc[4] = {S_NV, S_ND, S_NFRONT, S_NOMASK};
+#pragma unroll
+  for (int i = 0; i < 4; ++i) {
+    const float t = block_sum(threadIdx.x < CNT_BLOCKS ? cnt_part[i * CNT_BLOCKS + threadIdx.x] : 0.f, sh);
+    if (threadIdx.x == 0) s_sums[dc[i]] = t;
+  }
+  if (threadIdx.x == 0) {
+    finalize_terms(c, s_sums, s_out);
+    s_out[7] = 0.f; s_out[14] = 0.f; s_out[15] = 0.f;
+  }
+  __syncthreads();
+  if (threadIdx.x < S_COUNT) {
+    sums[threadIdx.x] = s_sums[threadIdx.x];
+    out[threadIdx.x] = s_out[threadIdx.x];
   }
 }
 
@@ -576,3 +837,57 @@
              d_fine, d_coarse, ldd_fine ? ldd_fine : L, d_occ, ld_occ);
   return check_launch("dns_loss_bwd_points");
 }
+
+extern "C" uint64_t dns_ray_losses_ws_floats(uint32_t N) { return (uint64_t)RW_RAYS + 6ull * N; }
+
+extern "C" int dns_loss_mask_counts(const float* lambdas, uint32_t N, uint32_t S, const float* gt_depth, const uint8_t* valid,
+                                    const float* z, float* ws, void* stream) {
+  DNS_REQUIRE(lambdas && ws, "dns_loss_mask_counts: NULL argument");
+  DNS_REQUIRE(N == 0 || (gt_depth && z && S >= 1), "dns_loss_mask_counts: NULL ray tensor");
+  DNS_REQUIRE((uint64_t)N * S < (1ull << 32) - (1ull << 22), "dns_loss_mask_counts: N*S must stay below 2^32");
+  const LossCfg c = make_cfg(lambdas, N, S, 0, 1, 0);
+  DNS_LAUNCH(loss_mask_counts_kernel, dim3(CNT_BLOCKS), dim3(256), 0, (hipStream_t)stream, c, gt_depth, valid, z, ws + RW_CNT);
+  return check_launch("dns_loss_mask_counts");
+}
+
+extern "C" int dns_ray_losses(const float* lambdas, uint32_t N, uint32_t S, uint32_t C, uint32_t L, const float* raw, const float* z,
+                              const float* logits, const float* gt_color, const float* gt_depth, const int64_t* gt_label,
+                              const uint8_t* valid, const float* fine, const float* coarse, const float* g_total, float* ws,
+                              float* depth, float* var, float* rgb, float* weights, float* sem, float* d_raw, float* d_logits,
+                              float* d_fine, float* d_coarse, uint32_t ldd_fine, uint32_t flags, void* stream) {
+  if (N == 0) return DNS_OK;
+  DNS_REQUIRE((flags & ~DNS_COMPOSITE_RGB_LOGITS) == 0, "dns_ray_losses: unknown flags 0x%x", flags);
+  DNS_REQUIRE(lambdas && raw && z && gt_color && gt_depth && fine && coarse && g_total && ws, "dns_ray_losses: NULL input");
+  DNS_REQUIRE(depth && rgb && d_raw && d_fine && d_coarse, "dns_ray_losses: NULL output");
+  DNS_REQUIRE(C == 0 || (logits && gt_label && sem && d_logits), "dns_ray_losses: C > 0 needs logits, labels, sem and d_logits");
+  DNS_REQUIRE(S >= 1 && S <= 256 && L >= 1, "dns_ray_losses: S=%u out of range [1,256] or L=%u < 1", S, L);
+  DNS_REQUIRE(ldd_fine == 0 || ldd_fine >= L, "dns_ray_losses: ldd_fine %u < L %u", ldd_fine, L);
+  DNS_REQUIRE((uint64_t)N * S * L < (1ull << 32) - (1ull << 22), "dns_ray_losses: N*S*L must stay below 2^32");
+  DNS_REQUIRE(((((uintptr_t)raw) | ((uintptr_t)d_raw)) & 15u) == 0, "dns_ray_losses: raw and d_raw must be 16-byte aligned");
+  const LossCfg c = make_cfg(lambdas, N, S, C, L, 0);
+  const uint32_t E = S <= 64 ? 1 : (S <= 128 ? 2 : 4);
+  const uint64_t base = 7ull * 64 * E + 2ull * C, lc = ((uint64_t)S * C + 3) & ~3ull;
+  const uint32_t stage = C && 4 * ((base + lc + 3) & ~3ull) * sizeof(float) <= 48 * 1024 ? 1u : 0u;
+  const uint64_t wstride = (base + (stage ? lc : 0) + 3) & ~3ull;
+  const size_t ldsb = 4 * wstride * sizeof(float);
+  DNS_REQUIRE(ldsb <= 60 * 1024, "dns_ray_losses: C=%u classes need %zu bytes of LDS", C, ldsb);
+  hipStream_t st = (hipStream_t)stream;
+  const dim3 grid((N + 3) / 4), block(256);
+#define LAUNCH_RL(EE)                                                                                                          \
+  DNS_LAUNCH(ray_losses_kernel<EE>, grid, block, ldsb, st, c, raw, z, logits, gt_color, gt_depth, gt_label, valid, fine, coarse, \
+             g_total, ws + RW_CNT, ws + RW_RAYS, depth, var, rgb, weights, sem, d_raw, d_logits, d_fine, d_coarse,              \
+             ldd_fine ? ldd_fine : L, flags & DNS_COMPOSITE_RGB_LOGITS, stage, (uint32_t)wstride)
+  if (E == 1) LAUNCH_RL(1);
+  else if (E == 2) LAUNCH_RL(2);
+  else LAUNCH_RL(4);
+#undef LAUNCH_RL
+  return check_launch("dns_ray_losses");
+}
+
+extern "C" int dns_ray_losses_finalize(const float* lambdas, uint32_t N, uint32_t S, uint32_t C, uint32_t L, float* ws, float* out,
+                                       void* stream) {
+  DNS_REQUIRE(lambdas && ws && out, "dns_ray_losses_finalize: NULL argument");
+  const LossCfg c = make_cfg(lambdas, N, S, C, L, 0);
+  DNS_LAUNCH(ray_losses_finalize_kernel, dim3(1), dim3(1024), 0, (hipStream_t)stream, c, ws + RW_CNT, ws + RW_RAYS, ws, out);
+  return check_launch("dns_ray_losses_finalize");
+}
diff --git a/dns_slam_amd/fused_step.py b/dns_slam_amd/fused_step.py
--- a/dns_slam_amd/fused_step.py
+++ b/dns_slam_amd/fused_step.py
@@ -209,6 +209,9 @@
         self.depth, self.var, self.rgb, self.weights, self.sem = f(N), f(N), f(N, 3), f(N, S), f(N, self.n_class)
         self.sums_ws, self.out = f(ops.LOSS_SUMS_FLOATS), f(16)
         self.one = torch.ones(1, device=dev)
+        self.fused_rays = (bool(getattr(m, "fused_ray_losses", os.environ.get("DNS_FUSED_RAY_LOSSES", "1") != "0"))
+                           and not self.dist_on)
+        self.rl_ws = f(int(ops.lib._raw.dns_ray_losses_ws_floats(N)))
         self.d_color, self.d_depth, self.d_sem = f(N, 3), f(N), f(N, self.n_class)
         self.d_coarse = f(P, nf)
         self.d_raw, self.d_logit, self.d_col = f(P, 4), f(P, self.n_class), f(P, 4)
@@ -472,6 +475,10 @@
                                     ptr(t_zero), self.nu, self.ns, jstride, ptr(cur.dmax), 1, ptr(self.rays_o), ptr(self.rays_d),
                                     ptr(self.gt_color), ptr(self.gt_depth), ptr(self.gt_label), ptr(self.inside), ptr(self.z),
                                     ptr(self.pts), st), "dns_raygen_sample")
+        fused_rays = self.fused_rays
+        if fused_rays:
+            check(lib.dns_loss_mask_counts(self.lam, N, S, ptr(self.gt_depth), ptr(self.inside), ptr(self.z), ptr(self.rl_ws), st),
+                  "dns_loss_mask_counts")
         meta = C.byref(self.meta.c)
         grid = _V(self.buf.data_ptr() + 4 * pe)
         sr = self.sr
@@ -540,27 +547,41 @@
         fwd(self.feat, pe, self.p_color, self.shp_col, self.raw, None, None, P, 0, self.h_col)
         fwd(self.feat, pe, self.p_logit, self.shp_log, self.logit, None, None, P, 0, self.h_log)
         Cn, L = self.n_class, self.hid + 1
-        check(lib.dns_composite_fwd_ex(ptr(self.raw), ptr(self.z), ptr(self.logit), N, S, Cn, ptr(self.depth), ptr(self.var),
-                                       ptr(self.rgb), ptr(self.weights), ptr(self.sem), 1, st), "dns_composite_fwd_ex")
         lam = self.lam
-        check(lib.dns_loss_sums(lam, N, S, Cn, L, 0, ptr(self.rgb), ptr(self.depth), None, ptr(self.sem), ptr(self.gt_color),
-                                ptr(self.gt_depth), ptr(self.gt_label), ptr(self.inside), ptr(fine), ptr(self.coarse),
-                                ptr(self.z), ptr(self.sums_ws), st), "dns_loss_sums")
-        if self.dist_on:
-            m.dist.allreduce_sums(self.sums_ws[:16])
-
         ldf = 4 + self.n_feat
         d_fine_dst = _V(self.d_featx.data_ptr() + 4 * 3)
-        check(lib.dns_loss_finalize_bwd(lam, N, S, Cn, L, 0, ptr(self.sums_ws), ptr(self.out), ptr(self.one), ptr(self.rgb),
-                                        ptr(self.depth), None, ptr(self.sem), ptr(self.gt_color), ptr(self.gt_depth),
-                                        ptr(self.gt_label), ptr(self.inside), ptr(self.d_color), ptr(self.d_depth), None,
-                                        ptr(self.d_sem), st), "dns_loss_finalize_bwd")
-        check(lib.dns_composite_bwd_ex(ptr(self.raw), ptr(self.z), ptr(self.logit), N, S, Cn, ptr(self.d_depth), None,
-                                       ptr(self.d_color), None, ptr(self.d_sem), ptr(self.d_raw), ptr(self.d_logit), 1, st),
-              "dns_composite_bwd_ex")
-        check(lib.dns_loss_bwd_points(lam, N, S, Cn, L, ptr(self.out), ptr(self.one), ptr(self.gt_depth), ptr(self.inside), ptr(fine),
-                                      ptr(self.coarse), ptr(self.z), d_fine_dst, ptr(self.d_coarse), ldf,
-                                      _V(self.d_raw.data_ptr() + 12), 4, st), "dns_loss_bwd_points")
+        loss_ev = None
+        if fused_rays:
+            check(lib.dns_ray_losses(lam, N, S, Cn, L, ptr(self.raw), ptr(self.z), ptr(self.logit), ptr(self.gt_color),
+                                     ptr(self.gt_depth), ptr(self.gt_label), ptr(self.inside), ptr(fine), ptr(self.coarse),
+                                     ptr(self.one), ptr(self.rl_ws), ptr(self.depth), None, ptr(self.rgb), None, ptr(self.sem),
+                                     ptr(self.d_raw), ptr(self.d_logit), d_fine_dst, ptr(self.d_coarse), ldf, 1, st), "dns_ray_losses")
+            if on_side:
+                loss_ev = torch.cuda.Event()
+                loss_ev.record(main)
+                self.side.wait_event(loss_ev)
+                with torch.cuda.stream(self.side):
+                    check(lib.dns_ray_losses_finalize(lam, N, S, Cn, L, ptr(self.rl_ws), ptr(self.out), _V(self.side.cuda_stream)),
+                          "dns_ray_losses_finalize")
+        else:
+            check(lib.dns_composite_fwd_ex(ptr(self.raw), ptr(self.z), ptr(self.logit), N, S, Cn, ptr(self.depth), ptr(self.var),
+                                           ptr(self.rgb), ptr(self.weights), ptr(self.sem), 1, st), "dns_composite_fwd_ex")
+            check(lib.dns_loss_sums(lam, N, S, Cn, L, 0, ptr(self.rgb), ptr(self.depth), None, ptr(self.sem), ptr(self.gt_color),
+                                    ptr(self.gt_depth), ptr(self.gt_label), ptr(self.inside), ptr(fine), ptr(self.coarse),
+                                    ptr(self.z), ptr(self.sums_ws), st), "dns_loss_sums")
+            if self.dist_on:
+                m.dist.allreduce_sums(self.sums_ws[:16])
+
+            check(lib.dns_loss_finalize_bwd(lam, N, S, Cn, L, 0, ptr(self.sums_ws), ptr(self.out), ptr(self.one), ptr(self.rgb),
+                                            ptr(self.depth), None, ptr(self.sem), ptr(self.gt_color), ptr(self.gt_depth),
+                                            ptr(self.gt_label), ptr(self.inside), ptr(self.d_color), ptr(self.d_depth), None,
+                                            ptr(self.d_sem), st), "dns_loss_finalize_bwd")
+            check(lib.dns_composite_bwd_ex(ptr(self.raw), ptr(self.z), ptr(self.logit), N, S, Cn, ptr(self.d_depth), None,
+                                           ptr(self.d_color), None, ptr(self.d_sem), ptr(self.d_raw), ptr(self.d_logit), 1, st),
+                  "dns_composite_bwd_ex")
+            check(lib.dns_loss_bwd_points(lam, N, S, Cn, L, ptr(self.out), ptr(self.one), ptr(self.gt_depth), ptr(self.inside), ptr(fine),
+                                          ptr(self.coarse), ptr(self.z), d_fine_dst, ptr(self.d_coarse), ldf,
+                                          _V(self.d_raw.data_ptr() + 12), 4, st), "dns_loss_bwd_points")
 
         fork_dwin = on_side and not half
         side_st = _V(self.side.cuda_stream)
@@ -651,6 +672,8 @@
                 check(lib.dns_add_ref_sum(ptr(self.d_rel), self.R, self.Pf, P, ptr(self.d_x3), st), "dns_add_ref_sum")
             check(lib.dns_raygen_bwd(ptr(pix), ptr(self.Q), self.camv, 0, H, 0, W, K, npf, S, ptr(self.z), ptr(self.d_x3), None,
                                      None, ptr(self.ray_ws), ptr(cur.g_quat), ptr(cur.g_trans), st), "dns_raygen_bwd")
+        if fused_rays and loss_ev is None:
+            check(lib.dns_ray_losses_finalize(lam, N, S, Cn, L, ptr(self.rl_ws), ptr(self.out), st), "dns_ray_losses_finalize")
         if on_side:
             main.wait_stream(self.side)
         if self.dist_on:
diff --git a/dns_slam_amd/ops.py b/dns_slam_amd/ops.py
--- a/dns_slam_amd/ops.py
+++ b/dns_slam_amd/ops.py
@@ -67,7 +67,8 @@
                   "dns_loss_bwd": (1, 2), "dns_loss_rays": (1, 2), "dns_loss_finalize_bwd": (1, 2), "dns_raw_bwd": 2, "dns_rgb_sigmoid": 1, "dns_class_slots": (1, 2),
                   "dns_hashgrid_indices": 1, "dns_sample_along_rays": 2, "dns_feature_gather": (4, 5),
                   "dns_encode_fwd_split": 2, "dns_mlp_fwd_half": 12, "dns_mlp_bwd_half": 17, "dns_mlp_fwd_split": 10, "dns_mlp_bwd_split": 16, "dns_feature_block_split": (9, 10),
-                  "dns_composite_fwd_ex": 3, "dns_composite_bwd_ex": 3, "dns_loss_bwd_points": (1, 2)}
+                  "dns_composite_fwd_ex": 3, "dns_composite_bwd_ex": 3, "dns_loss_bwd_points": (1, 2),
+                  "dns_loss_mask_counts": (1, 2), "dns_ray_losses": (1, 2)}
 
     def arm(self, kernels=False):
         self.kernels = bool(kernels)
diff --git a/include/dns_hip.h b/include/dns_hip.h
--- a/include/dns_hip.h
+++ b/include/dns_hip.h
@@ -7,7 +7,7 @@
 extern "C" {
 #endif
 
-#define DNS_ABI_VERSION 13
+#define DNS_ABI_VERSION 14
 #define DNS_MAX_LEVELS 32
 
 #define DNS_OK 0
@@ -181,6 +181,17 @@
                         const float* g_total, const float* gt_depth, const uint8_t* valid, const float* fine, const float* coarse,
                         const float* z, float* d_fine, float* d_coarse, uint32_t ldd_fine, const float* d_occ, uint32_t ld_occ,
                         void* stream);
+
+uint64_t dns_ray_losses_ws_floats(uint32_t N);
+int dns_loss_mask_counts(const float* lambdas, uint32_t N, uint32_t S, const float* gt_depth, const uint8_t* valid, const float* z,
+                         float* ws, void* stream);
+int dns_ray_losses(const float* lambdas, uint32_t N, uint32_t S, uint32_t C, uint32_t L, const float* raw, const float* z,
+                   const float* logits, const float* gt_color, const float* gt_depth, const int64_t* gt_label, const uint8_t* valid,
+                   const float* fine, const float* coarse, const float* g_total, float* ws, float* depth, float* var, float* rgb,
+                   float* weights, float* sem, float* d_raw, float* d_logits, float* d_fine, float* d_coarse, uint32_t ldd_fine,
+                   uint32_t flags, void* stream);
+int dns_ray_losses_finalize(const float* lambdas, uint32_t N, uint32_t S, uint32_t C, uint32_t L, float* ws, float* out,
+                            void* stream);
 
 typedef struct DnsAdamTensor {
   float* p;
```

New measurement: 164.5 million. -3.3%, worse.
